# samkoesnadi/fpn-MT-image-captioning

Hardware: AMD Instinct MI355X
Metric: training images/sec (FPN+transformer step) at 1/2/4/8 MI355X; CPU-ref logit Δ (higher is better)
Workload: dtype bf16; 1 GPU; C2: ResNet-50 FPN + 6-layer transformer, 224x224, per-GPU batch 32, T=31, V=10000, full training step (fwd+bwd+clip+AMSGrad), dropout 0.1, hipGraph replay; per_gpu_batch=32, global_batch=32, seq_len=31, parallelism=dp1

## Files before the change

### fpn-mt-image-captioning_amd/csrc/elementwise.hip

```cpp
#include "common.h"
#include <initializer_list>

namespace fpnmt {

template <typename T> struct V16;
template <> struct V16<bf16> { typedef bf16x8 type; static constexpr int n = 8; };
template <> struct V16<float> { typedef f32x4 type; static constexpr int n = 4; };

static inline int grid_for(long long work, int block, int cap = 4096) {
  long long g = (work + block - 1) / block;
  if (g > cap) g = cap;
  if (g < 1) g = 1;
  return (int)g;
}

static inline __host__ __device__ int pow2_floor(int v) {
  int r = 1;
  while (r * 2 <= v) r *= 2;
  return r;
}
template <typename T, bool VEC>
__device__ __forceinline__ void act_bwd_block(int bx, int by, long long rows, int c, int act, float a,
                                              const T* __restrict__ dy, const T* __restrict__ y, T* dz, float* db,
                                              float* __restrict__ ws, int rows_per_chunk, bool write, float dp,
// ... 422 lines not shown
    Ld8<T, VN>::store(dx + (((long long)nn * h + ih) * w + iw) * c + ch, g);
  }
}

template <typename T>
__global__ __launch_bounds__(256) void maxpool3s2_bwd_kernel(int n, int h, int w, int c, int pt, int pl, int ho,
                                                             int wo, const uint8_t* __restrict__ argmax,
                                                             const T* __restrict__ dy, T* __restrict__ dx,
                                                             const T* __restrict__ xact, int act, float alpha) {
  const int cg = c / 8;
  const long long total = (long long)n * ho * wo * cg;
  for (long long i = blockIdx.x * (long long)blockDim.x + threadIdx.x; i < total;
       i += (long long)gridDim.x * blockDim.x) {
    const int ch = (int)(i % cg) * 8;
    long long t = i / cg;
    const int ow = (int)(t % wo);
    t /= wo;
    const int oh = (int)(t % ho);
    const int nn = (int)(t / ho);
    float g[4][8];
#pragma unroll
    for (int q = 0; q < 4; ++q)
#pragma unroll
      for (int j = 0; j < 8; ++j) g[q][j] = 0.f;
#pragma unroll
    for (int dy_ = -1; dy_ <= 0; ++dy_) {
#pragma unroll
      for (int dx_ = -1; dx_ <= 0; ++dx_) {
        const int wy = oh + dy_, wx = ow + dx_;
        if (wy < 0 || wx < 0) continue;
        const long long o = (((long long)nn * ho + wy) * wo + wx) * c + ch;
        const uint2 a = *(const uint2*)(argmax + o);
        int slot[8];
        bool any = false;
#pragma unroll
        for (int j = 0; j < 8; ++j) {
          const int am = (int)(((j < 4 ? a.x : a.y) >> (8 * (j & 3))) & 255);
          const int r = am / 3, q = am - 3 * r;
          const int dr = 2 * dy_ + r, dc = 2 * dx_ + q;
          slot[j] = ((unsigned)dr < 2u && (unsigned)dc < 2u) ? dr * 2 + dc : -1;
          any |= slot[j] >= 0;
        }
        if (!any) continue;
        float d[8];
        Ld8<T, 8>::load(dy + o, d);
#pragma unroll
        for (int j = 0; j < 8; ++j)
#pragma unroll
          for (int q = 0; q < 4; ++q)
            if (slot[j] == q) g[q][j] += d[j];
      }
    }
#pragma unroll
    for (int q = 0; q < 4; ++q) {
      const int ih = 2 * oh - pt + (q >> 1), iw = 2 * ow - pl + (q & 1);
      if (ih < 0 || ih >= h || iw < 0 || iw >= w) continue;
      T* dst = dx + (((long long)nn * h + ih) * w + iw) * c + ch;
      if (xact) {
        float v[8];
        Ld8<T, 8>::load(xact + (dst - dx), v);
#pragma unroll
        for (int j = 0; j < 8; ++j) g[q][j] *= act_mask_from_y(v[j], act, alpha);
      }
      Ld8<T, 8>::store(dst, g[q]);
    }
  }
}

template <typename T>
static void maxpool_launch(bool fwd, int n, int h, int w, int c, int kh, int kw, int sh, int sw, int pt, int pl,
                           int ho, int wo, const void* x, void* y, uint8_t* am, const void* dy, void* dx,
                           hipStream_t s, const void* xact = nullptr, int act = 0, float alpha = 0.f) {
  const bool vec = c % 8 == 0 && (uintptr_t)x % 16 == 0 && (uintptr_t)(fwd ? y : dy) % 16 == 0 &&
                   (uintptr_t)(fwd ? y : dx) % 16 == 0 && (uintptr_t)am % 8 == 0 && (uintptr_t)xact % 16 == 0;
  const long long total = (long long)n * (fwd ? (long long)ho * wo : (long long)h * w) * (vec ? c / 8 : c);
  const int g = grid_for(total, 256, 8192);
  if (fwd) {
    if (vec)
      hipLaunchKernelGGL((maxpool_fwd_kernel<T, 8>), dim3(g), dim3(256), 0, s, n, h, w, c, kh, kw, sh, sw, pt, pl,
                         ho, wo, (const T*)x, (T*)y, am);
    else
      hipLaunchKernelGGL((maxpool_fwd_kernel<T, 1>), dim3(g), dim3(256), 0, s, n, h, w, c, kh, kw, sh, sw, pt, pl,
                         ho, wo, (const T*)x, (T*)y, am);
  } else if (vec && am && kh == 3 && kw == 3 && sh == 2 && sw == 2 && (unsigned)pt < 2u && (unsigned)pl < 2u &&
             2 * ho - pt >= h && 2 * wo - pl >= w) {
    const int g2 = grid_for((long long)n * ho * wo * (c / 8), 256, 8192);
    hipLaunchKernelGGL((maxpool3s2_bwd_kernel<T>), dim3(g2), dim3(256), 0, s, n, h, w, c, pt, pl, ho, wo,
                       (const uint8_t*)am, (const T*)dy, (T*)dx, (const T*)xact, act, alpha);
  } else {
    if (vec)
      hipLaunchKernelGGL((maxpool_bwd_kernel<T, 8>), dim3(g), dim3(256), 0, s, n, h, w, c, kh, kw, sh, sw, pt, pl,
                         ho, wo, (const T*)x, (const uint8_t*)am, (const T*)dy, (T*)dx, (const T*)xact, act, alpha);
    else
      hipLaunchKernelGGL((maxpool_bwd_kernel<T, 1>), dim3(g), dim3(256), 0, s, n, h, w, c, kh, kw, sh, sw, pt, pl,
                         ho, wo, (const T*)x, (const uint8_t*)am, (const T*)dy, (T*)dx, (const T*)xact, act, alpha);
  }
}

__device__ __forceinline__ int nn_src(int d, int in, int out) {
  int s = (int)floorf(((float)d + 0.5f) * ((float)in / (float)out));
  return s < in - 1 ? s : in - 1;
}

template <typename T>
__global__ void fpn_fwd_kernel(int n, int cg, int h5, int w5, int h4, int w4, int h3, int w3,
                               const T* __restrict__ l5, const T* __restrict__ l4,
                               const T* __restrict__ l3, T* __restrict__ p4m,
                               T* __restrict__ p3m) {
  typedef typename V16<T>::type VT;
  constexpr int VN = V16<T>::n;
  const int c = cg * VN;
  const long long tot3 = (long long)n * h3 * w3 * cg, tot4 = (long long)n * h4 * w4 * cg;
  for (long long i = blockIdx.x * (long long)blockDim.x + threadIdx.x; i < tot3 + tot4;
       i += (long long)gridDim.x * blockDim.x) {
    const bool is3 = i < tot3;
    long long j = is3 ? i : i - tot3;
    const int g = (int)(j % cg);
    long long t = j / cg;
    const int W = is3 ? w3 : w4, H = is3 ? h3 : h4;
    const int x = (int)(t % W);
    t /= W;
    const int y = (int)(t % H);
    const int b = (int)(t / H);
    const int y4 = is3 ? nn_src(y, h4, h3) : y, x4 = is3 ? nn_src(x, w4, w3) : x;
    const int y5 = nn_src(y4, h5, h4), x5 = nn_src(x4, w5, w4);
    VT a4 = *(const VT*)(l4 + (((long long)b * h4 + y4) * w4 + x4) * c + g * VN);
    VT a5 = *(const VT*)(l5 + (((long long)b * h5 + y5) * w5 + x5) * c + g * VN);
    VT o;
    if (is3) {
      VT a3 = *(const VT*)(l3 + (((long long)b * h3 + y) * w3 + x) * c + g * VN);
#pragma unroll
      for (int k = 0; k < VN; ++k) {
        const float p4 = to_f32(from_f32<T>(to_f32(a4[k]) + to_f32(a5[k])));
        o[k] = from_f32<T>(to_f32(a3[k]) + p4);
      }
      *(VT*)(p3m + (((long long)b * h3 + y) * w3 + x) * c + g * VN) = o;
    } else {
#pragma unroll
      for (int k = 0; k < VN; ++k) o[k] = from_f32<T>(to_f32(a4[k]) + to_f32(a5[k]));
      *(VT*)(p4m + (((long long)b * h4 + y) * w4 + x) * c + g * VN) = o;
    }
  }
}

__device__ __forceinline__ void nn_children(int s, int in, int out, int& lo, int& hi) {
  int d0 = (int)(((long long)s * out) / in) - 2;
  if (d0 < 0) d0 = 0;
  lo = -1;
  hi = -1;
  for (int d = d0; d < out; ++d) {
    const int src = nn_src(d, in, out);
    if (src == s && lo < 0) lo = d;
    if (src > s) { hi = d; break; }
  }
  if (lo < 0) { lo = 0; hi = 0; return; }
  if (hi < 0) hi = out;
}

template <typename T>
__global__ void fpn_bwd_kernel(int n, int cg, int h5, int w5, int h4, int w4, int h3, int w3,
                               const T* __restrict__ dp4, const T* __restrict__ dp3,
                               T* __restrict__ dl4, T* __restrict__ dl5, int acc5) {
  typedef typename V16<T>::type VT;
  constexpr int VN = V16<T>::n;
  const int c = cg * VN;
  const long long tot4 = (long long)n * h4 * w4 * cg, tot5 = (long long)n * h5 * w5 * cg;
  for (long long i = blockIdx.x * (long long)blockDim.x + threadIdx.x; i < tot4 + tot5;
       i += (long long)gridDim.x * blockDim.x) {
    const bool is4 = i < tot4;
    long long j = is4 ? i : i - tot4;
    const int g = (int)(j % cg);
    long long t = j / cg;
    const int W = is4 ? w4 : w5, H = is4 ? h4 : h5;
    const int x = (int)(t % W);
    t /= W;
    const int y = (int)(t % H);
    const int b = (int)(t / H);
    float acc[VN];
#pragma unroll
    for (int k = 0; k < VN; ++k) acc[k] = 0.f;
    int y4lo, y4hi, x4lo, x4hi;
    if (is4) { y4lo = y; y4hi = y + 1; x4lo = x; x4hi = x + 1; }
    else { nn_children(y, h5, h4, y4lo, y4hi); nn_children(x, w5, w4, x4lo, x4hi); }
    for (int yy = y4lo; yy < y4hi; ++yy)
      for (int xx = x4lo; xx < x4hi; ++xx) {
        VT d4 = *(const VT*)(dp4 + (((long long)b * h4 + yy) * w4 + xx) * c + g * VN);
        float s4[VN];
#pragma unroll
        for (int k = 0; k < VN; ++k) s4[k] = to_f32(d4[k]);
        int y3lo, y3hi, x3lo, x3hi;
        nn_children(yy, h4, h3, y3lo, y3hi);
        nn_children(xx, w4, w3, x3lo, x3hi);
        for (int y3 = y3lo; y3 < y3hi; ++y3)
          for (int x3 = x3lo; x3 < x3hi; ++x3) {
            VT d3 = *(const VT*)(dp3 + (((long long)b * h3 + y3) * w3 + x3) * c + g * VN);
#pragma unroll
            for (int k = 0; k < VN; ++k) s4[k] += to_f32(d3[k]);
          }
        if (is4) {
#pragma unroll
          for (int k = 0; k < VN; ++k) acc[k] = s4[k];
        } else {
#pragma unroll
          for (int k = 0; k < VN; ++k) acc[k] += to_f32(from_f32<T>(s4[k]));
        }
      }
    VT o;
    if (is4) {
#pragma unroll
      for (int k = 0; k < VN; ++k) o[k] = from_f32<T>(acc[k]);
      *(VT*)(dl4 + (((long long)b * h4 + y) * w4 + x) * c + g * VN) = o;
    } else {
      T* dst = dl5 + (((long long)b * h5 + y) * w5 + x) * c + g * VN;
      if (acc5) {
        VT old = *(const VT*)dst;
#pragma unroll
        for (int k = 0; k < VN; ++k) o[k] = from_f32<T>(acc[k] + to_f32(old[k]));
      } else {
#pragma unroll
        for (int k = 0; k < VN; ++k) o[k] = from_f32<T>(acc[k]);
      }
      *(VT*)dst = o;
    }
  }
}

template <typename T>
__global__ __launch_bounds__(256) void ssm_fwd_kernel(int hw, int c, int chunk,
                                                      const T* __restrict__ score,
                                                      const T* __restrict__ hs,
                                                      T* __restrict__ ctx, float* __restrict__ a_out) {
  __shared__ float red[8];
  const int b = blockIdx.x;
  const T* sc = score + (long long)b * hw;
  float m = -INFINITY;
  for (int p = threadIdx.x; p < hw; p += 256) m = fmaxf(m, to_f32(sc[p]));
  m = wave_max(m);
  if ((threadIdx.x & 63) == 0) red[threadIdx.x >> 6] = m;
  __syncthreads();
  m = fmaxf(fmaxf(red[0], red[1]), fmaxf(red[2], red[3]));
  __syncthreads();
  float s = 0.f;
  for (int p = threadIdx.x; p < hw; p += 256) s += expf(to_f32(sc[p]) - m);
  s = wave_sum(s);
  if ((threadIdx.x & 63) == 0) red[threadIdx.x >> 6] = s;
  __syncthreads();
  s = red[0] + red[1] + red[2] + red[3];
  const int p0 = blockIdx.y * chunk, p1 = min(hw, p0 + chunk);
  for (int p = p0 + threadIdx.x; p < p1; p += 256)
    a_out[(long long)b * hw + p] = expf(to_f32(sc[p]) - m) / s;
  const long long e0 = (long long)p0 * c, e1 = (long long)p1 * c;
  const T* h = hs + (long long)b * hw * c;
  T* o = ctx + (long long)b * hw * c;
  for (long long e = e0 + threadIdx.x; e < e1; e += 256) {
    const int p = (int)(e / c);
    const float a = expf(to_f32(sc[p]) - m) / s;
    o[e] = from_f32<T>(a * to_f32(h[e]));
  }
}

template <typename T>
__global__ __launch_bounds__(256) void ssm_bwd1_kernel(long long npos, int c, const float* __restrict__ a,
                                                       const T* __restrict__ hs,
                                                       const T* __restrict__ dctx, T* __restrict__ dhs,
                                                       double* __restrict__ da) {
  const long long wid = (blockIdx.x * 256LL + threadIdx.x) >> 6;
  const int lane = threadIdx.x & 63;
  for (long long p = wid; p < npos; p += (long long)gridDim.x * 4) {
    const float ap = a[p];
    double dot = 0.0;
    for (int ch = lane; ch < c; ch += 64) {
      const long long e = p * c + ch;
      const float g = to_f32(dctx[e]);
      dot += (double)g * (double)to_f32(hs[e]);
      dhs[e] = from_f32<T>(ap * g);
    }
    dot = wave_sum(dot);
    if (lane == 0) da[p] = dot;
  }
}
template <typename T>
__global__ __launch_bounds__(256) void ssm_bwd2_kernel(int hw, const float* __restrict__ a,
                                                       const double* __restrict__ da,
                                                       T* __restrict__ dscore) {
  __shared__ double red[4];
  const long long base = (long long)blockIdx.x * hw;
  double s = 0.0;
  for (int p = threadIdx.x; p < hw; p += 256) s += (double)a[base + p] * da[base + p];
  s = wave_sum(s);
  if ((threadIdx.x & 63) == 0) red[threadIdx.x >> 6] = s;
  __syncthreads();
  s = red[0] + red[1] + red[2] + red[3];
  for (int p = threadIdx.x; p < hw; p += 256)
    dscore[base + p] = from_f32<T>((float)((double)a[base + p] * (da[base + p] - s)));
}

constexpr int LN_MAXE = 16;
template <bool VEC>
__device__ __forceinline__ int ln_col(int lane, int k) {
  if constexpr (VEC) return (lane + 64 * (k >> 3)) * 8 + (k & 7);
  else return lane + 64 * k;
}

template <typename T, bool VEC>
__device__ __forceinline__ void ln_fwd_rows(long long blk, long long nblk, long long rows, int d, float eps,
                                            const T* __restrict__ x, const T* __restrict__ res,
                                            const float* __restrict__ gamma, const float* __restrict__ beta,
                                            const float* __restrict__ pe, int pe_rows, T* __restrict__ y,
                                            float* __restrict__ mean_out, float* __restrict__ rstd_out, float op,
                                            unsigned long long okey) {
  const int lane = threadIdx.x & 63;
  const long long wid = (blk * 256LL + threadIdx.x) >> 6;
  const long long nw = nblk * 4;
  const float osc = op > 0.f ? 1.f / (1.f - op) : 1.f;
  float gm[LN_MAXE], bt[LN_MAXE];
#pragma unroll
  for (int i = 0; i < LN_MAXE; ++i) {
    const int col = ln_col<VEC>(lane, i);
    gm[i] = col < d ? gamma[col] : 0.f;
    bt[i] = col < d ? beta[col] : 0.f;
  }
  for (long long r = wid; r < rows; r += nw) {
    float v[LN_MAXE], pv[LN_MAXE];
    float s = 0.f;
    {
      const long long prow = pe ? (r % pe_rows) : 0;
#pragma unroll
      for (int i = 0; i < LN_MAXE; ++i) {
        const int col = ln_col<VEC>(lane, i);
        pv[i] = pe && col < d ? pe[prow * d + col] : 0.f;
      }
    }
    if constexpr (VEC) {
#pragma unroll
      for (int i = 0; i < LN_MAXE / 8; ++i) {
        const int c0 = (lane + 64 * i) * 8;
        bf16x8 xv = {}, rv = {};
        if (c0 < d) {
          xv = *(const bf16x8*)(x + r * d + c0);
          if (res) rv = *(const bf16x8*)(res + r * d + c0);
        }
#pragma unroll
        for (int e = 0; e < 8; ++e) {
          float t = 0.f;
          if (c0 < d) {
            t = to_f32(xv[e]);
            if (res) t = to_f32(from_f32<T>(t + to_f32(rv[e])));
          }
          v[i * 8 + e] = t;
          s += t;
        }
      }
    } else {
#pragma unroll
      for (int i = 0; i < LN_MAXE; ++i) {
        const int col = lane + 64 * i;
        v[i] = 0.f;
        if (col < d) {
          float t = to_f32(x[r * d + col]);
          if (res) t = to_f32(from_f32<T>(t + to_f32(res[r * d + col])));
          v[i] = t;
          s += t;
        }
      }
    }
    const float mu = wave_sum(s) / (float)d;
    float q = 0.f;
#pragma unroll
    for (int i = 0; i < LN_MAXE; ++i) {
      const int col = ln_col<VEC>(lane, i);
      if (col < d) { const float t = v[i] - mu; q += t * t; }
    }
    const float var = wave_sum(q) / (float)d;
    const float rs = rsqrtf(var + eps);
    if constexpr (VEC) {
#pragma unroll
      for (int i = 0; i < LN_MAXE / 8; ++i) {
        const int c0 = (lane + 64 * i) * 8;
        if (c0 < d) {
          bf16x8 ov;
#pragma unroll
          for (int e = 0; e < 8; ++e) {
            float o = (v[i * 8 + e] - mu) * rs * gm[i * 8 + e] + bt[i * 8 + e];
            if (pe) o += pv[i * 8 + e];
            ov[e] = from_f32<T>(o);
            if (op > 0.f)
              ov[e] = from_f32<T>(uniform01(okey, (uint64_t)r * (uint64_t)d + (uint64_t)(c0 + e)) >= op
                                      ? to_f32(ov[e]) * osc : 0.f);
          }
          *(bf16x8*)(y + r * d + c0) = ov;
        }
      }
    } else {
#pragma unroll
      for (int i = 0; i < LN_MAXE; ++i) {
        const int col = lane + 64 * i;
        if (col < d) {
          float o = (v[i] - mu) * rs * gm[i] + bt[i];
          if (pe) o += pv[i];
          T ot = from_f32<T>(o);
          if (op > 0.f)
            ot = from_f32<T>(uniform01(okey, (uint64_t)r * (uint64_t)d + (uint64_t)col) >= op ? to_f32(ot) * osc
                                                                                                 : 0.f);
          y[r * d + col] = ot;
        }
      }
    }
    if (lane == 0) { mean_out[r] = mu; rstd_out[r] = rs; }
  }
}

template <typename T, bool VEC = false>
__global__ __launch_bounds__(256) void ln_fwd_kernel(long long rows, int d, float eps,
                                                     const T* __restrict__ x, const T* __restrict__ res,
                                                     const float* __restrict__ gamma,
                                                     const float* __restrict__ beta,
                                                     const float* __restrict__ pe, int pe_rows,
                                                     T* __restrict__ y, float* __restrict__ mean_out,
                                                     float* __restrict__ rstd_out) {
  ln_fwd_rows<T, VEC>(blockIdx.x, gridDim.x, rows, d, eps, x, res, gamma, beta, pe, pe_rows, y, mean_out, rstd_out,
                      0.f, 0ull);
}

template <typename T, bool VEC>
__device__ __forceinline__ void ln_bwd_rows(long long blk, long long nblk, long long rows, int d,
                                            const T* __restrict__ x, const T* __restrict__ res,
                                            const float* __restrict__ gamma, const float* __restrict__ mean,
                                            const float* __restrict__ rstd, const T* __restrict__ dy,
                                            T* __restrict__ dx, float* __restrict__ part, float dp,
                                            unsigned long long dkey, T* __restrict__ dz, float ip,
                                            unsigned long long ikey) {
  const int lane = threadIdx.x & 63;
  const float dsc = dz ? 1.f / (1.f - dp) : 1.f;
  const float isc = ip > 0.f ? 1.f / (1.f - ip) : 1.f;
  const long long wid = (blk * 256LL + threadIdx.x) >> 6;
  const long long nw = nblk * 4;
  float pg[LN_MAXE], pb[LN_MAXE];
#pragma unroll
  for (int i = 0; i < LN_MAXE; ++i) pg[i] = pb[i] = 0.f;
  for (long long r = wid; r < rows; r += nw) {
    const float mu = mean[r], rs = rstd[r];
    float xh[LN_MAXE], g[LN_MAXE];
    float s1 = 0.f, s2 = 0.f;
    if constexpr (VEC) {
#pragma unroll
      for (int i = 0; i < LN_MAXE / 8; ++i) {
        const int c0 = (lane + 64 * i) * 8;
        bf16x8 xv = {}, rv = {}, dv = {};
        if (c0 < d) {
          xv = *(const bf16x8*)(x + r * d + c0);
          if (res) rv = *(const bf16x8*)(res + r * d + c0);
          dv = *(const bf16x8*)(dy + r * d + c0);
        }
#pragma unroll
        for (int e = 0; e < 8; ++e) {
          const int k = i * 8 + e;
          xh[k] = 0.f;
          g[k] = 0.f;
          if (c0 < d) {
            float t = to_f32(xv[e]);
            if (res) t = to_f32(from_f32<T>(t + to_f32(rv[e])));
            xh[k] = (t - mu) * rs;
            float dyf = to_f32(dv[e]);
            if (ip > 0.f)
              dyf = to_f32(from_f32<T>(uniform01(ikey, (uint64_t)r * (uint64_t)d + (uint64_t)(c0 + e)) >= ip
                                           ? dyf * isc : 0.f));
            g[k] = dyf * gamma[c0 + e];
            pg[k] += dyf * xh[k];
            pb[k] += dyf;
            s1 += g[k];
            s2 += g[k] * xh[k];
          }
        }
      }
    } else {
#pragma unroll
      for (int i = 0; i < LN_MAXE; ++i) {
        const int col = lane + 64 * i;
        xh[i] = 0.f;
        g[i] = 0.f;
        if (col < d) {
          float t = to_f32(x[r * d + col]);
          if (res) t = to_f32(from_f32<T>(t + to_f32(res[r * d + col])));
          xh[i] = (t - mu) * rs;
          float dyf = to_f32(dy[r * d + col]);
          if (ip > 0.f)
            dyf = to_f32(from_f32<T>(uniform01(ikey, (uint64_t)r * (uint64_t)d + (uint64_t)col) >= ip ? dyf * isc
                                                                                                       : 0.f));
          g[i] = dyf * gamma[col];
          pg[i] += dyf * xh[i];
          pb[i] += dyf;
          s1 += g[i];
          s2 += g[i] * xh[i];
        }
      }
    }
    s1 = wave_sum(s1) / (float)d;
    s2 = wave_sum(s2) / (float)d;
    if constexpr (VEC) {
#pragma unroll
      for (int i = 0; i < LN_MAXE / 8; ++i) {
        const int c0 = (lane + 64 * i) * 8;
        if (c0 < d) {
          bf16x8 ov;
#pragma unroll
          for (int e = 0; e < 8; ++e) ov[e] = from_f32<T>(rs * (g[i * 8 + e] - s1 - xh[i * 8 + e] * s2));
          *(bf16x8*)(dx + r * d + c0) = ov;
          if (dz) {
#pragma unroll
            for (int e = 0; e < 8; ++e) {
              const float t = to_f32(ov[e]);
              ov[e] = from_f32<T>(uniform01(dkey, (uint64_t)r * (uint64_t)d + (uint64_t)(c0 + e)) >= dp ? t * dsc
                                                                                                         : 0.f);
            }
            *(bf16x8*)(dz + r * d + c0) = ov;
          }
        }
      }
    } else {
#pragma unroll
      for (int i = 0; i < LN_MAXE; ++i) {
        const int col = lane + 64 * i;
        if (col < d) {
          const T v = from_f32<T>(rs * (g[i] - s1 - xh[i] * s2));
          dx[r * d + col] = v;
          if (dz) {
            const float t = to_f32(v);
            dz[r * d + col] =
                from_f32<T>(uniform01(dkey, (uint64_t)r * (uint64_t)d + (uint64_t)col) >= dp ? t * dsc : 0.f);
          }
        }
      }
    }
  }
  if (part) {
    __shared__ float red[4][2 * 64 * LN_MAXE];
    const int w = threadIdx.x >> 6;
#pragma unroll
    for (int i = 0; i < LN_MAXE; ++i) {
      const int col = ln_col<VEC>(lane, i);
      if (col < d) {
        red[w][col] = pg[i];
        red[w][d + col] = pb[i];
      }
    }
    __syncthreads();
    float* dst = part + blk * 2 * d;
    for (int e = threadIdx.x; e < 2 * d; e += 256) dst[e] = ((red[0][e] + red[1][e]) + red[2][e]) + red[3][e];
  }
}

__device__ __forceinline__ unsigned long long drop_key_of(unsigned long long seed, const long long* seed_dev) {
  return seed + (seed_dev ? (unsigned long long)(*seed_dev) * 0x9E3779B97F4A7C15ull : 0ull);
}

template <typename T, bool VEC = false>
__global__ __launch_bounds__(256) void ln_bwd_kernel(long long rows, int d, const T* __restrict__ x,
                                                     const T* __restrict__ res,
                                                     const float* __restrict__ gamma,
                                                     const float* __restrict__ mean,
                                                     const float* __restrict__ rstd,
                                                     const T* __restrict__ dy, T* __restrict__ dx,
                                                     float* __restrict__ part, float dp,
                                                     unsigned long long dseed,
                                                     const long long* __restrict__ dseed_dev,
                                                     T* __restrict__ dz) {
  ln_bwd_rows<T, VEC>(blockIdx.x, gridDim.x, rows, d, x, res, gamma, mean, rstd, dy, dx, part, dp,
                      dz ? drop_key_of(dseed, dseed_dev) : 0ull, dz, 0.f, 0ull);
}

struct LnView {
  const void* x;
  void* y;
  const void* dy;
  float* mean;
  float* rstd;
  float* part;
  long long rows;
  unsigned long long seed;
  int blk0, nblk, pe_rows;
};
struct LnViews {
  LnView v[FPNMT_MAX_LN_VIEWS];
  int n;
};

__device__ __forceinline__ int ln_view_of(const LnViews& A, int b) {
  int k = 0;
#pragma unroll
  for (int i = 1; i < FPNMT_MAX_LN_VIEWS; ++i)
    if (i < A.n && b >= A.v[i].blk0) k = i;
  return k;
}

template <typename T, bool VEC>
__global__ __launch_bounds__(256) void ln_views_fwd_kernel(const LnViews A, int d, float eps,
                                                           const float* __restrict__ gamma,
                                                           const float* __restrict__ beta,
                                                           const float* __restrict__ pe, float p,
                                                           const long long* __restrict__ seed_dev) {
  const LnView& a = A.v[ln_view_of(A, blockIdx.x)];
  ln_fwd_rows<T, VEC>(blockIdx.x - a.blk0, a.nblk, a.rows, d, eps, (const T*)a.x, nullptr, gamma, beta, pe, a.pe_rows,
                      (T*)a.y, a.mean, a.rstd, p, p > 0.f ? drop_key_of(a.seed, seed_dev) : 0ull);
}

template <typename T, bool VEC>
__global__ __launch_bounds__(256) void ln_views_bwd_kernel(const LnViews A, int d, const float* __restrict__ gamma,
                                                           float p, const long long* __restrict__ seed_dev) {
  const LnView& a = A.v[ln_view_of(A, blockIdx.x)];
  ln_bwd_rows<T, VEC>(blockIdx.x - a.blk0, a.nblk, a.rows, d, (const T*)a.x, nullptr, gamma, a.mean, a.rstd,
                      (const T*)a.dy, (T*)a.y, a.part, 0.f, 0ull, nullptr, p,
                      p > 0.f ? drop_key_of(a.seed, seed_dev) : 0ull);
}

template <typename T>
__global__ void embed_fwd_kernel(int b, int t, int d, const int32_t* __restrict__ tok,
                                 const float* __restrict__ emb, const float* __restrict__ pe,
                                 T* __restrict__ y, float p, unsigned long long seed,
                                 const long long* __restrict__ seed_dev) {
  const long long total = (long long)b * t * d;
  const float sc = p > 0.f ? 1.f / (1.f - p) : 1.f;
  const unsigned long long key = p > 0.f ? drop_key_of(seed, seed_dev) : 0ull;
  for (long long i = blockIdx.x * (long long)blockDim.x + threadIdx.x; i < total;
       i += (long long)gridDim.x * blockDim.x) {
    const int col = (int)(i % d);
    const long long row = i / d;
    const int pos = (int)(row % t);
    const int id = tok[row];
    T v = from_f32<T>(emb[(long long)id * d + col] + pe[(long long)pos * d + col]);
    if (p > 0.f) v = from_f32<T>(uniform01(key, (uint64_t)i) >= p ? to_f32(v) * sc : 0.f);
    y[i] = v;
  }
}

template <typename T>
__device__ __forceinline__ float drop_grad(T g, float p, float sc, unsigned long long key, long long i) {
  if (p <= 0.f) return to_f32(g);
  return to_f32(from_f32<T>(uniform01(key, (uint64_t)i) >= p ? to_f32(g) * sc : 0.f));
}
template <typename I>
__global__ void decoder_targets_kernel(int b, int t, const I* __restrict__ tok, long long ld,
                                       int32_t* __restrict__ tin, int32_t* __restrict__ tout,
                                       float* __restrict__ mask) {
  const long long total = (long long)b * t * t;
  for (long long e = blockIdx.x * (long long)blockDim.x + threadIdx.x; e < total;
       e += (long long)gridDim.x * blockDim.x) {
    const int j = (int)(e % t);
    const long long bi = e / t;
    const int i = (int)(bi % t);
    const int bb = (int)(bi / t);
    const long long tj = (long long)tok[(long long)bb * ld + j];
    mask[e] = (tj == 0 || j > i) ? 1.f : 0.f;
    if (i == 0) {
      tin[(long long)bb * t + j] = (int32_t)tj;
      tout[(long long)bb * t + j] = (int32_t)tok[(long long)bb * ld + j + 1];
    }
  }
}

constexpr int EMB_CHUNK = 64, EMB_COLS = 512;
template <typename T>
__global__ __launch_bounds__(256) void embed_chunk_kernel(long long rows, int d, const int32_t* __restrict__ tok,
                                                          const T* __restrict__ dy, float* __restrict__ part,
                                                          float p, unsigned long long seed,
                                                          const long long* __restrict__ seed_dev) {
  const float sc = p > 0.f ? 1.f / (1.f - p) : 1.f;
  const unsigned long long key = p > 0.f ? drop_key_of(seed, seed_dev) : 0ull;
  __shared__ int s_tok[EMB_CHUNK], s_lead[EMB_CHUNK];
  __shared__ float acc[EMB_CHUNK][EMB_COLS];
  const int tid = threadIdx.x;
  const long long p0 = (long long)blockIdx.x * EMB_CHUNK;
  const int n = (int)min((long long)EMB_CHUNK, rows - p0);
  if (tid < EMB_CHUNK) s_tok[tid] = tid < n ? tok[p0 + tid] : -1;
  __syncthreads();
  if (tid < n) {
    int l = tid;
    for (int j = 0; j < tid; ++j)
      if (s_tok[j] == s_tok[tid]) { l = j; break; }
    s_lead[tid] = l;
  }
  __syncthreads();
  for (int c0 = 0; c0 < d; c0 += EMB_COLS) {
    const int w = min(EMB_COLS, d - c0);
    for (int e = tid; e < EMB_CHUNK * EMB_COLS; e += 256) (&acc[0][0])[e] = 0.f;
    __syncthreads();
    for (int col = tid; col < w; col += 256) {
#pragma unroll 8
      for (int i = 0; i < n; ++i)
        acc[s_lead[i]][col] += drop_grad(dy[(p0 + i) * d + c0 + col], p, sc, key, (p0 + i) * d + c0 + col);
    }
    __syncthreads();
    for (int i = 0; i < n; ++i) {
      if (s_lead[i] != i) continue;
      for (int col = tid; col < w; col += 256) part[(p0 + i) * d + c0 + col] = acc[i][col];
    }
    __syncthreads();
  }
}

template <typename T>
__global__ __launch_bounds__(64) void embed_leader_kernel(long long rows, int d, const int32_t* __restrict__ tok,
                                                          const T* __restrict__ dy, const float* __restrict__ part,
                                                          float* __restrict__ demb, float* __restrict__ rowsq,
                                                          int tok_in_lds, float dp, unsigned long long seed,
                                                          const long long* __restrict__ seed_dev) {
  const float dsc = dp > 0.f ? 1.f / (1.f - dp) : 1.f;
  const unsigned long long key = dp > 0.f ? drop_key_of(seed, seed_dev) : 0ull;
  extern __shared__ int s_tok[];
  __shared__ int s_lead[EMB_CHUNK];
  const int lane = threadIdx.x;
  const long long p = blockIdx.x;
  if (tok_in_lds) {
    for (long long q = lane; q < rows; q += 64) s_tok[q] = tok[q];
    __syncthreads();
  }
  const int32_t* tk = tok_in_lds ? (const int32_t*)s_tok : tok;
  const int id = tk[p];
  float sq = 0.f;
  for (int col = lane; col < d; col += 64) {
    const float g = drop_grad(dy[p * d + col], dp, dsc, key, p * d + col);
    sq += g * g;
  }
  sq = wave_sum(sq);
  if (lane == 0 && rowsq) rowsq[p] = sq;
  bool seen = false;
  for (long long q = lane; q < p; q += 64) seen |= tk[q] == id;
  if (__any(seen)) return;
  const long long nch = (rows + EMB_CHUNK - 1) / EMB_CHUNK;
  for (int c0 = 0; c0 < d; c0 += 64 * 8) {
    float a[8];
#pragma unroll
    for (int j = 0; j < 8; ++j) a[j] = 0.f;
    for (long long cb = p / EMB_CHUNK; cb < nch; cb += EMB_CHUNK) {
      int nl = 0;
      for (int l = 0; l < EMB_CHUNK && cb + l < nch; ++l) {
        const long long q = (cb + l) * EMB_CHUNK + lane;
        const unsigned long long m = __ballot(q < rows && tk[q] == id);
        if (m) {
          if (lane == 0) s_lead[nl] = (int)((cb + l) * EMB_CHUNK + __ffsll((long long)m) - 1);
          ++nl;
        }
      }
      __syncthreads();
      for (int i = 0; i < nl; i += 4) {
        float v[4][8];
#pragma unroll
        for (int u = 0; u < 4; ++u)
#pragma unroll
          for (int j = 0; j < 8; ++j) {
            const int col = c0 + lane + 64 * j;
            v[u][j] = (i + u < nl && col < d) ? part[(long long)s_lead[i + u] * d + col] : 0.f;
          }
#pragma unroll
        for (int u = 0; u < 4; ++u)
#pragma unroll
          for (int j = 0; j < 8; ++j) a[j] += v[u][j];
      }
      __syncthreads();
    }
#pragma unroll
    for (int j = 0; j < 8; ++j) {
      const int col = c0 + lane + 64 * j;
      if (col < d) demb[(long long)id * d + col] += a[j];
    }
  }
}

__global__ __launch_bounds__(256) void ordered_sum_kernel(long long n, const float* __restrict__ v, float scale,
                                                          float* __restrict__ out, int accumulate) {
  __shared__ float red[4];
  float s = 0.f;
  for (long long i = threadIdx.x; i < n; i += 256) s += v[i];
  s = wave_sum(s);
  if ((threadIdx.x & 63) == 0) red[threadIdx.x >> 6] = s;
  __syncthreads();
  if (threadIdx.x == 0) {
    const float t = ((red[0] + red[1]) + (red[2] + red[3])) * scale;
    out[0] = accumulate ? out[0] + t : t;
  }
}

template <typename T>
__global__ __launch_bounds__(256) void xent_kernel(long long rows, int v, const float* __restrict__ logits,
                                                   long long ld, const int32_t* __restrict__ labels,
                                                   float* __restrict__ loss, T* __restrict__ dlog,
                                                   long long ldd, float gscale) {
  __shared__ float red[4];
  const long long r = blockIdx.x;
  const float* x = logits + r * ld;
  float m = -INFINITY;
  for (int j = threadIdx.x; j < v; j += 256) m = fmaxf(m, x[j]);
  m = wave_max(m);
  if ((threadIdx.x & 63) == 0) red[threadIdx.x >> 6] = m;
  __syncthreads();
  m = fmaxf(fmaxf(red[0], red[1]), fmaxf(red[2], red[3]));
  __syncthreads();
  float s = 0.f;
  for (int j = threadIdx.x; j < v; j += 256) s += expf(x[j] - m);
  s = wave_sum(s);
  if ((threadIdx.x & 63) == 0) red[threadIdx.x >> 6] = s;
  __syncthreads();
  s = red[0] + red[1] + red[2] + red[3];
  const int lab = labels[r];
  const float mask = lab != 0 ? 1.f : 0.f;
  if (threadIdx.x == 0) loss[r] = mask != 0.f ? (m + logf(s)) - x[lab] : 0.f;
  if (dlog) {
    const float coef = mask * gscale / (float)rows;
    T* dr = dlog + r * ldd;
    for (int j = threadIdx.x; j < v; j += 256) {
      float p = expf(x[j] - m) / s;
      if (j == lab) p -= 1.f;
      dr[j] = from_f32<T>(p * coef);
    }
  }
}

}

using namespace fpnmt;

#define DT_DISPATCH(dtype, FN, ...)                                         \
  ((dtype) == FPNMT_BF16 ? FN<bf16>(__VA_ARGS__)                            \
   : (dtype) == FPNMT_F32 ? FN<float>(__VA_ARGS__)                          \
                          : fail(FPNMT_E_ARG, "unknown dtype"))

extern "C" {

long long fpnmt_act_bwd_ws_bytes(int dtype, long long rows, int c) {
  if (rows <= 0 || c <= 0) return 0;
  const ActBwdGrid a = dtype == FPNMT_BF16 ? act_bwd_grid<bf16>(rows, c, true, true)
                                           : act_bwd_grid<float>(rows, c, true, true);
  const ActBwdGrid b = dtype == FPNMT_BF16 ? act_bwd_grid<bf16>(rows, c, false, true)
                                           : act_bwd_grid<float>(rows, c, false, true);
  return (long long)std::max(a.gy, b.gy) * c * (long long)sizeof(float);
}

int fpnmt_act_bwd(int dtype, long long rows, int c, int act, float act_alpha, const void* dy,
                  const void* y, void* dz, float* db, float* ws, float drop_p, unsigned long long drop_seed,
                  const long long* drop_seed_dev, fpnmt_stream_t stream) {
  if (rows <= 0 || c <= 0) return 0;
  if (!dy || !dz || (act != FPNMT_ACT_NONE && !y)) return fail(FPNMT_E_ARG, "act_bwd: null pointer");
  if (drop_p >= 1.f) return fail(FPNMT_E_ARG, "act_bwd: drop_p must be < 1");
  return DT_DISPATCH(dtype, act_bwd_t, rows, c, act, act_alpha, dy, y, dz, db, ws, drop_p, drop_seed,
                     drop_seed_dev, S(stream));
}

int fpnmt_bias_grad(int dtype, long long rows, int c, const void* dy, float* db, fpnmt_stream_t stream) {
  if (rows <= 0 || c <= 0 || !db) return 0;
  if (!dy) return fail(FPNMT_E_ARG, "bias_grad: null pointer");
  if (dtype != FPNMT_BF16 && dtype != FPNMT_F32) return fail(FPNMT_E_ARG, "bias_grad: bad dtype");
  hipStream_t s = S(stream);
  if (!defer_active())
    return dtype == FPNMT_BF16
               ? act_bwd_t<bf16>(rows, c, FPNMT_ACT_NONE, 0.f, dy, nullptr, (void*)dy, db, nullptr, 0.f, 0ull, nullptr, s)
               : act_bwd_t<float>(rows, c, FPNMT_ACT_NONE, 0.f, dy, nullptr, (void*)dy, db, nullptr, 0.f, 0ull, nullptr, s);
  const bool aligned = ((uintptr_t)dy % 16) == 0;
  const ActBwdGrid G = dtype == FPNMT_BF16 ? act_bwd_grid<bf16>(rows, c, aligned, true)
                                           : act_bwd_grid<float>(rows, c, aligned, true);
  DefDirect J{};
  J.dy = dy;
  J.db = db;
  J.rows = rows;
  J.c = c;
  J.rpc = G.rpc;
  J.gt = G.gt;
  J.gx = G.gx;
  J.gy = G.gy;
  J.vec = G.vec ? 1 : 0;
  J.dtype = dtype;
  {
    J.ws = defer_alloc((long long)G.gy * c);
    if (!J.ws)
      return dtype == FPNMT_BF16 ? act_bwd_t<bf16>(rows, c, FPNMT_ACT_NONE, 0.f, dy, nullptr, (void*)dy, db, nullptr,
                                                   0.f, 0ull, nullptr, s)
                                 : act_bwd_t<float>(rows, c, FPNMT_ACT_NONE, 0.f, dy, nullptr, (void*)dy, db, nullptr,
                                                    0.f, 0ull, nullptr, s);
  }
  int st = defer_direct(J, s);
  if (!st) colsum_launch(G.gy, c, J.ws, db, s);
  return st;
}

int fpnmt_cast(int in_dtype, int out_dtype, long long n, const void* in, void* out,
               fpnmt_stream_t stream) {
  if (n <= 0) return 0;
  const int g = grid_for(n, 256);
  hipStream_t s = S(stream);
  if (in_dtype == FPNMT_F32 && out_dtype == FPNMT_BF16)
    hipLaunchKernelGGL((cast_kernel<float, bf16>), dim3(g), dim3(256), 0, s, n, (const float*)in, (bf16*)out);
  else if (in_dtype == FPNMT_BF16 && out_dtype == FPNMT_F32)
    hipLaunchKernelGGL((cast_kernel<bf16, float>), dim3(g), dim3(256), 0, s, n, (const bf16*)in, (float*)out);
  else if (in_dtype == FPNMT_F32 && out_dtype == FPNMT_F32)
    hipLaunchKernelGGL((cast_kernel<float, float>), dim3(g), dim3(256), 0, s, n, (const float*)in, (float*)out);
  else if (in_dtype == FPNMT_BF16 && out_dtype == FPNMT_BF16)
    hipLaunchKernelGGL((cast_kernel<bf16, bf16>), dim3(g), dim3(256), 0, s, n, (const bf16*)in, (bf16*)out);
  else
    return fail(FPNMT_E_ARG, "cast: bad dtype");
  return check_launch("cast");
}

int fpnmt_dropout(int dtype, long long n, float p, unsigned long long seed, const long long* seed_dev,
                  const void* x, void* y, fpnmt_stream_t stream) {
  if (n <= 0) return 0;
  if (!(p >= 0.f && p < 1.f)) return fail(FPNMT_E_ARG, "dropout: p must be in [0,1)");
  const int g = grid_for(n, 256);
  if (dtype == FPNMT_BF16)
    hipLaunchKernelGGL((dropout_kernel<bf16>), dim3(g), dim3(256), 0, S(stream), n, p, seed, seed_dev,
                       (const bf16*)x, (bf16*)y);
  else
    hipLaunchKernelGGL((dropout_kernel<float>), dim3(g), dim3(256), 0, S(stream), n, p, seed, seed_dev,
                       (const float*)x, (float*)y);
  return check_launch("dropout");
}

int fpnmt_add(int dtype, long long n, const void* a, const void* b, void* out, fpnmt_stream_t stream) {
  if (n <= 0) return 0;
  const int g = grid_for(n, 256);
  if (dtype == FPNMT_BF16)
    hipLaunchKernelGGL((add_kernel<bf16>), dim3(g), dim3(256), 0, S(stream), n, (const bf16*)a,
                       (const bf16*)b, (bf16*)out);
  else
    hipLaunchKernelGGL((add_kernel<float>), dim3(g), dim3(256), 0, S(stream), n, (const float*)a,
                       (const float*)b, (float*)out);
  return check_launch("add");
}

int fpnmt_maxpool2d_fwd(int dtype, int n, int h, int w, int c, int kh, int kw, int sh, int sw, int pt,
                        int pl, int ho, int wo, const void* x, void* y, uint8_t* argmax, fpnmt_stream_t stream) {
  const long long total = (long long)n * ho * wo * c;
  if (total <= 0) return 0;
  if (argmax && kh * kw > 255) return fail(FPNMT_E_UNSUPPORTED, "maxpool: argmax needs kh*kw <= 255");
  if (dtype == FPNMT_BF16)
    maxpool_launch<bf16>(true, n, h, w, c, kh, kw, sh, sw, pt, pl, ho, wo, x, y, argmax, nullptr, nullptr, S(stream));
  else
    maxpool_launch<float>(true, n, h, w, c, kh, kw, sh, sw, pt, pl, ho, wo, x, y, argmax, nullptr, nullptr, S(stream));
  return check_launch("maxpool_fwd");
}

int fpnmt_maxpool2d_bwd(int dtype, int n, int h, int w, int c, int kh, int kw, int sh, int sw, int pt,
                        int pl, int ho, int wo, const void* x, const uint8_t* argmax, const void* dy, void* dx,
                        fpnmt_stream_t stream) {
  const long long total = (long long)n * h * w * c;
  if (total <= 0) return 0;
  if (ho <= 0 || wo <= 0) return zero_fill(dx, total * (dtype == FPNMT_BF16 ? 2 : 4), S(stream));
  if (!argmax && !x) return fail(FPNMT_E_ARG, "maxpool_bwd: need x or argmax");
  if (dtype == FPNMT_BF16)
    maxpool_launch<bf16>(false, n, h, w, c, kh, kw, sh, sw, pt, pl, ho, wo, x, nullptr, (uint8_t*)argmax, dy, dx, S(stream));
  else
    maxpool_launch<float>(false, n, h, w, c, kh, kw, sh, sw, pt, pl, ho, wo, x, nullptr, (uint8_t*)argmax, dy, dx, S(stream));
  return check_launch("maxpool_bwd");
}

int fpnmt_maxpool2d_bwd_act(int dtype, int n, int h, int w, int c, int kh, int kw, int sh, int sw, int pt, int pl,
                            int ho, int wo, const uint8_t* argmax, const void* dy, const void* x, int act,
                            float alpha, void* dx, fpnmt_stream_t stream) {
  const long long total = (long long)n * h * w * c;
  if (total <= 0) return 0;
  if (ho <= 0 || wo <= 0) return zero_fill(dx, total * (dtype == FPNMT_BF16 ? 2 : 4), S(stream));
  if (!argmax || !x || !dy || !dx) return fail(FPNMT_E_ARG, "maxpool_bwd_act: null argmax / x / dy / dx");
  if (act != FPNMT_ACT_RELU && act != FPNMT_ACT_RELU6 && act != FPNMT_ACT_LEAKY)
    return fail(FPNMT_E_ARG, "maxpool_bwd_act: act must be relu / relu6 / leaky");
  if (act == FPNMT_ACT_LEAKY && (kh > sh || kw > sw))
    return fail(FPNMT_E_UNSUPPORTED, "maxpool_bwd_act: leaky needs non-overlapping windows");
  if (dtype == FPNMT_BF16)
    maxpool_launch<bf16>(false, n, h, w, c, kh, kw, sh, sw, pt, pl, ho, wo, nullptr, nullptr, (uint8_t*)argmax, dy,
                         dx, S(stream), x, act, alpha);
  else
    maxpool_launch<float>(false, n, h, w, c, kh, kw, sh, sw, pt, pl, ho, wo, nullptr, nullptr, (uint8_t*)argmax, dy,
                          dx, S(stream), x, act, alpha);
  return check_launch("maxpool_bwd_act");
}

int fpnmt_fpn_topdown_fwd(int dtype, int n, int c, int h5, int w5, int h4, int w4, int h3, int w3,
                          const void* lat5, const void* lat4, const void* lat3, void* p4m, void* p3m,
                          fpnmt_stream_t stream) {
  const int vn = dtype == FPNMT_BF16 ? 8 : 4;
  if (c % vn) return fail(FPNMT_E_UNSUPPORTED, "fpn_topdown: channels must be a multiple of 8 (bf16) / 4 (f32)");
  const long long total = (long long)n * (h3 * w3 + h4 * w4) * (c / vn);
  if (total <= 0) return 0;
  const int g = grid_for(total, 256);
  if (dtype == FPNMT_BF16)
    hipLaunchKernelGGL((fpn_fwd_kernel<bf16>), dim3(g), dim3(256), 0, S(stream), n, c / vn, h5, w5, h4, w4,
                       h3, w3, (const bf16*)lat5, (const bf16*)lat4, (const bf16*)lat3, (bf16*)p4m, (bf16*)p3m);
  else
    hipLaunchKernelGGL((fpn_fwd_kernel<float>), dim3(g), dim3(256), 0, S(stream), n, c / vn, h5, w5, h4, w4,
                       h3, w3, (const float*)lat5, (const float*)lat4, (const float*)lat3, (float*)p4m,
                       (float*)p3m);
  return check_launch("fpn_topdown_fwd");
}

int fpnmt_fpn_topdown_bwd(int dtype, int n, int c, int h5, int w5, int h4, int w4, int h3, int w3,
                          const void* d_p4m, const void* d_p3m, void* d_lat4, void* d_lat5,
                          int accumulate_lat5, fpnmt_stream_t stream) {
  const int vn = dtype == FPNMT_BF16 ? 8 : 4;
  if (c % vn) return fail(FPNMT_E_UNSUPPORTED, "fpn_topdown: channels must be a multiple of 8 (bf16) / 4 (f32)");
  const long long total = (long long)n * (h4 * w4 + h5 * w5) * (c / vn);
  if (total <= 0) return 0;
  const int g = grid_for(total, 256);
  if (dtype == FPNMT_BF16)
    hipLaunchKernelGGL((fpn_bwd_kernel<bf16>), dim3(g), dim3(256), 0, S(stream), n, c / vn, h5, w5, h4, w4,
                       h3, w3, (const bf16*)d_p4m, (const bf16*)d_p3m, (bf16*)d_lat4, (bf16*)d_lat5,
                       accumulate_lat5);
  else
    hipLaunchKernelGGL((fpn_bwd_kernel<float>), dim3(g), dim3(256), 0, S(stream), n, c / vn, h5, w5, h4, w4,
                       h3, w3, (const float*)d_p4m, (const float*)d_p3m, (float*)d_lat4, (float*)d_lat5,
                       accumulate_lat5);
  return check_launch("fpn_topdown_bwd");
}

int fpnmt_spatial_softmax_fwd(int dtype, int n, int hw, int c, const void* score, const void* hs,
                              void* ctx, float* a_out, fpnmt_stream_t stream) {
  if (n <= 0 || hw <= 0) return 0;
  int chunks = (int)((long long)hw * c / 8192);
  if (chunks < 1) chunks = 1;
  if (chunks > hw) chunks = hw;
  const int chunk = cdiv(hw, chunks);
  chunks = cdiv(hw, chunk);
  dim3 grid(n, chunks);
  if (dtype == FPNMT_BF16)
    hipLaunchKernelGGL((ssm_fwd_kernel<bf16>), grid, dim3(256), 0, S(stream), hw, c, chunk,
                       (const bf16*)score, (const bf16*)hs, (bf16*)ctx, a_out);
  else
    hipLaunchKernelGGL((ssm_fwd_kernel<float>), grid, dim3(256), 0, S(stream), hw, c, chunk,
                       (const float*)score, (const float*)hs, (float*)ctx, a_out);
  return check_launch("spatial_softmax_fwd");
}

int fpnmt_spatial_softmax_bwd(int dtype, int n, int hw, int c, const float* a, const void* hs,
                              const void* d_ctx, void* d_score, void* d_hs, double* ws,
                              fpnmt_stream_t stream) {
  if (n <= 0 || hw <= 0) return 0;
  const long long npos = (long long)n * hw;
  const int g = grid_for(npos, 4, 8192);
  if (dtype == FPNMT_BF16) {
    hipLaunchKernelGGL((ssm_bwd1_kernel<bf16>), dim3(g), dim3(256), 0, S(stream), npos, c, a,
                       (const bf16*)hs, (const bf16*)d_ctx, (bf16*)d_hs, ws);
    hipLaunchKernelGGL((ssm_bwd2_kernel<bf16>), dim3(n), dim3(256), 0, S(stream), hw, a, ws, (bf16*)d_score);
  } else {
    hipLaunchKernelGGL((ssm_bwd1_kernel<float>), dim3(g), dim3(256), 0, S(stream), npos, c, a,
                       (const float*)hs, (const float*)d_ctx, (float*)d_hs, ws);
    hipLaunchKernelGGL((ssm_bwd2_kernel<float>), dim3(n), dim3(256), 0, S(stream), hw, a, ws, (float*)d_score);
  }
  return check_launch("spatial_softmax_bwd");
}

static bool ln_vec(int d, std::initializer_list<const void*> ptrs) {
  if (d % 8) return false;
  for (const void* p : ptrs)
    if ((uintptr_t)p & 15) return false;
  return true;
}

int fpnmt_layernorm_fwd(int dtype, long long rows, int d, float eps, const void* x, const void* res,
                        const float* gamma, const float* beta, const float* pe, int pe_rows, void* y,
                        float* mean, float* rstd, fpnmt_stream_t stream) {
  if (rows <= 0) return 0;
  if (d > 64 * LN_MAXE) return fail(FPNMT_E_UNSUPPORTED, "layernorm: d > 1024");
  if (pe && pe_rows <= 0) return fail(FPNMT_E_ARG, "layernorm: pe_rows");
  const int g = grid_for(rows, 4, 8192);
  if (dtype == FPNMT_BF16) {
    if (ln_vec(d, {x, res, y}))
      hipLaunchKernelGGL((ln_fwd_kernel<bf16, true>), dim3(g), dim3(256), 0, S(stream), rows, d, eps, (const bf16*)x,
                       (const bf16*)res, gamma, beta, pe, pe_rows, (bf16*)y, mean, rstd);
    else
      hipLaunchKernelGGL((ln_fwd_kernel<bf16>), dim3(g), dim3(256), 0, S(stream), rows, d, eps, (const bf16*)x,
                       (const bf16*)res, gamma, beta, pe, pe_rows, (bf16*)y, mean, rstd);
  } else {
    hipLaunchKernelGGL((ln_fwd_kernel<float>), dim3(g), dim3(256), 0, S(stream), rows, d, eps, (const float*)x,
                       (const float*)res, gamma, beta, pe, pe_rows, (float*)y, mean, rstd);
  }
  return check_launch("layernorm_fwd");
}

static int layernorm_bwd_impl(int dtype, long long rows, int d, const void* x, const void* res, const float* gamma,
                              const float* mean, const float* rstd, const void* dy, void* dx, float* dgamma,
                              float* dbeta, float dp, unsigned long long dseed, const long long* dseed_dev, void* dz,
                              hipStream_t s) {
  if (rows <= 0) return 0;
  if (d > 64 * LN_MAXE) return fail(FPNMT_E_UNSUPPORTED, "layernorm: d > 1024");
  if (dz && !(dp > 0.f && dp < 1.f)) return fail(FPNMT_E_ARG, "layernorm_bwd_drop: drop_p outside (0, 1)");
  const int g = grid_for(rows, 4, 1024);
  float* part = nullptr;
  if (dgamma || dbeta) {
    part = partial_f32((long long)g * 2 * d);
    if (!part) return fail(FPNMT_E_ARG, "layernorm_bwd: dgamma / dbeta need the fpnmt workspace");
  }
  if (dtype == FPNMT_BF16) {
    if (ln_vec(d, {x, res, dy, dx, dz}))
      hipLaunchKernelGGL((ln_bwd_kernel<bf16, true>), dim3(g), dim3(256), 0, s, rows, d, (const bf16*)x,
                         (const bf16*)res, gamma, mean, rstd, (const bf16*)dy, (bf16*)dx, part, dp, dseed, dseed_dev,
                         (bf16*)dz);
    else
      hipLaunchKernelGGL((ln_bwd_kernel<bf16>), dim3(g), dim3(256), 0, s, rows, d, (const bf16*)x,
                         (const bf16*)res, gamma, mean, rstd, (const bf16*)dy, (bf16*)dx, part, dp, dseed, dseed_dev,
                         (bf16*)dz);
  } else {
    hipLaunchKernelGGL((ln_bwd_kernel<float>), dim3(g), dim3(256), 0, s, rows, d, (const float*)x,
                       (const float*)res, gamma, mean, rstd, (const float*)dy, (float*)dx, part, dp, dseed, dseed_dev,
                       (float*)dz);
  }
  if (part) colsum_launch(g, 2 * d, part, dgamma, s, d, dbeta);
  return check_launch("layernorm_bwd");
}

int fpnmt_layernorm_bwd(int dtype, long long rows, int d, const void* x, const void* res,
                        const float* gamma, const float* mean, const float* rstd, const void* dy, void* dx,
                        float* dgamma, float* dbeta, fpnmt_stream_t stream) {
  return layernorm_bwd_impl(dtype, rows, d, x, res, gamma, mean, rstd, dy, dx, dgamma, dbeta, 0.f, 0ull, nullptr,
                            nullptr, S(stream));
}

int fpnmt_layernorm_bwd_drop(int dtype, long long rows, int d, const void* x, const void* res, const float* gamma,
                             const float* mean, const float* rstd, const void* dy, void* dx, float* dgamma,
                             float* dbeta, float drop_p, unsigned long long drop_seed,
                             const long long* drop_seed_dev, void* dz, fpnmt_stream_t stream) {
  if (!dz) return fail(FPNMT_E_ARG, "layernorm_bwd_drop: null dz");
  return layernorm_bwd_impl(dtype, rows, d, x, res, gamma, mean, rstd, dy, dx, dgamma, dbeta, drop_p, drop_seed,
                            drop_seed_dev, dz, S(stream));
}

static bool ln_views_vec(int n, int d, const fpnmt_ln_view* v, bool bwd) {
  for (int i = 0; i < n; ++i)
    if (!(bwd ? ln_vec(d, {v[i].x, v[i].dy, v[i].y}) : ln_vec(d, {v[i].x, v[i].y}))) return false;
  return true;
}

int fpnmt_layernorm_views_fwd(int dtype, int n, int d, float eps, const fpnmt_ln_view* views, const float* gamma,
                              const float* beta, const float* pe, float drop_p, const long long* seed_dev,
                              fpnmt_stream_t stream) {
  if (n < 0 || n > FPNMT_MAX_LN_VIEWS) return fail(FPNMT_E_ARG, "layernorm_views_fwd: 0 <= n <= FPNMT_MAX_LN_VIEWS");
  if (d > 64 * LN_MAXE) return fail(FPNMT_E_UNSUPPORTED, "layernorm: d > 1024");
  if (!(drop_p >= 0.f && drop_p < 1.f)) return fail(FPNMT_E_ARG, "layernorm_views_fwd: drop_p outside [0, 1)");
  LnViews A{};
  int blocks = 0;
  for (int i = 0; i < n; ++i) {
    const fpnmt_ln_view& v = views[i];
    if (v.rows <= 0) continue;
    if (!v.x || !v.y || !v.mean || !v.rstd || (pe && v.pe_rows <= 0))
      return fail(FPNMT_E_ARG, "layernorm_views_fwd: null pointer / pe_rows");
    LnView& a = A.v[A.n++];
    a.x = v.x; a.y = v.y; a.mean = v.mean; a.rstd = v.rstd; a.rows = v.rows; a.seed = v.seed;
    a.pe_rows = pe ? v.pe_rows : 1;
    a.blk0 = blocks;
    a.nblk = grid_for(v.rows, 4, 8192);
    blocks += a.nblk;
  }
  if (!A.n) return 0;
  hipStream_t s = S(stream);
  if (dtype == FPNMT_BF16) {
    if (ln_views_vec(n, d, views, false))
      hipLaunchKernelGGL((ln_views_fwd_kernel<bf16, true>), dim3(blocks), dim3(256), 0, s, A, d, eps, gamma, beta, pe,
                         drop_p, seed_dev);
    else
      hipLaunchKernelGGL((ln_views_fwd_kernel<bf16, false>), dim3(blocks), dim3(256), 0, s, A, d, eps, gamma, beta,
                         pe, drop_p, seed_dev);
  } else {
    hipLaunchKernelGGL((ln_views_fwd_kernel<float, false>), dim3(blocks), dim3(256), 0, s, A, d, eps, gamma, beta, pe,
                       drop_p, seed_dev);
  }
  return check_launch("layernorm_views_fwd");
}

int fpnmt_layernorm_views_bwd(int dtype, int n, int d, const fpnmt_ln_view* views, const float* gamma, float drop_p,
                              const long long* seed_dev, float* dgamma, float* dbeta, fpnmt_stream_t stream) {
  if (n < 0 || n > FPNMT_MAX_LN_VIEWS) return fail(FPNMT_E_ARG, "layernorm_views_bwd: 0 <= n <= FPNMT_MAX_LN_VIEWS");
  if (d > 64 * LN_MAXE) return fail(FPNMT_E_UNSUPPORTED, "layernorm: d > 1024");
  if (!(drop_p >= 0.f && drop_p < 1.f)) return fail(FPNMT_E_ARG, "layernorm_views_bwd: drop_p outside [0, 1)");
  LnViews A{};
  int blocks = 0;
  for (int i = 0; i < n; ++i) {
    const fpnmt_ln_view& v = views[i];
    if (v.rows <= 0) continue;
    if (!v.x || !v.y || !v.dy || !v.mean || !v.rstd) return fail(FPNMT_E_ARG, "layernorm_views_bwd: null pointer");
    LnView& a = A.v[A.n++];
    a.x = v.x; a.y = v.y; a.dy = v.dy; a.mean = v.mean; a.rstd = v.rstd; a.rows = v.rows; a.seed = v.seed;
    a.blk0 = blocks;
    a.nblk = grid_for(v.rows, 4, 1024);
    blocks += a.nblk;
    a.part = nullptr;
  }
  if (!A.n) return 0;
  if (dgamma || dbeta) {
    float* part = partial_f32((long long)blocks * 2 * d);
    if (!part) return fail(FPNMT_E_ARG, "layernorm_views_bwd: dgamma / dbeta need the fpnmt workspace");
    for (int i = 0; i < A.n; ++i) A.v[i].part = part + (long long)A.v[i].blk0 * 2 * d;
  }
  hipStream_t s = S(stream);
  if (dtype == FPNMT_BF16) {
    if (ln_views_vec(n, d, views, true))
      hipLaunchKernelGGL((ln_views_bwd_kernel<bf16, true>), dim3(blocks), dim3(256), 0, s, A, d, gamma, drop_p,
                         seed_dev);
    else
      hipLaunchKernelGGL((ln_views_bwd_kernel<bf16, false>), dim3(blocks), dim3(256), 0, s, A, d, gamma, drop_p,
                         seed_dev);
  } else {
    hipLaunchKernelGGL((ln_views_bwd_kernel<float, false>), dim3(blocks), dim3(256), 0, s, A, d, gamma, drop_p,
                       seed_dev);
  }
  const int st = check_launch("layernorm_views_bwd");
  if (st) return st;
  for (int i = 0; i < A.n; ++i)
    if (A.v[i].part) colsum_launch(A.v[i].nblk, 2 * d, A.v[i].part, dgamma, s, d, dbeta);
  return check_launch("layernorm_views_bwd colsum");
}

static int embed_fwd_impl(int dtype, int b, int t, int d, const int32_t* tok, const float* emb, const float* pe,
                          void* y, float p, unsigned long long seed, const long long* seed_dev, hipStream_t s) {
  const long long total = (long long)b * t * d;
  if (total <= 0) return 0;
  const int g = grid_for(total, 256);
  if (dtype == FPNMT_BF16)
    hipLaunchKernelGGL((embed_fwd_kernel<bf16>), dim3(g), dim3(256), 0, s, b, t, d, tok, emb, pe, (bf16*)y, p, seed,
                       seed_dev);
  else
    hipLaunchKernelGGL((embed_fwd_kernel<float>), dim3(g), dim3(256), 0, s, b, t, d, tok, emb, pe, (float*)y, p,
                       seed, seed_dev);
  return check_launch("embed_fwd");
}

static int embed_bwd_impl(int dtype, int b, int t, int d, const int32_t* tok, const void* dy, float* d_emb,
                          float* sumsq, float p, unsigned long long seed, const long long* seed_dev,
                          hipStream_t s) {
  const long long rows = (long long)b * t;
  if (rows <= 0) return 0;
  if (rows >= (1LL << 31)) return fail(FPNMT_E_UNSUPPORTED, "embed_bwd: too many positions");
  float* part = scratch_f32(rows * d + rows);
  if (!part) return fail(FPNMT_E_ARG, "embed_bwd: needs the fpnmt workspace");
  float* rowsq = sumsq ? part + rows * d : nullptr;
  const unsigned nch = (unsigned)((rows + EMB_CHUNK - 1) / EMB_CHUNK);
  const unsigned lds = rows <= 8192 ? (unsigned)(rows * 4) : 0u;
  if (dtype == FPNMT_BF16) {
    hipLaunchKernelGGL((embed_chunk_kernel<bf16>), dim3(nch), dim3(256), 0, s, rows, d, tok, (const bf16*)dy, part,
                       p, seed, seed_dev);
    hipLaunchKernelGGL((embed_leader_kernel<bf16>), dim3((unsigned)rows), dim3(64), lds, s, rows, d, tok,
                       (const bf16*)dy, (const float*)part, d_emb, rowsq, lds > 0, p, seed, seed_dev);
  } else {
    hipLaunchKernelGGL((embed_chunk_kernel<float>), dim3(nch), dim3(256), 0, s, rows, d, tok, (const float*)dy, part,
                       p, seed, seed_dev);
    hipLaunchKernelGGL((embed_leader_kernel<float>), dim3((unsigned)rows), dim3(64), lds, s, rows, d, tok,
                       (const float*)dy, (const float*)part, d_emb, rowsq, lds > 0, p, seed, seed_dev);
  }
  if (sumsq) hipLaunchKernelGGL(ordered_sum_kernel, dim3(1), dim3(256), 0, s, rows, rowsq, 1.f, sumsq, 1);
  return check_launch("embed_bwd");
}

int fpnmt_embed_posenc_fwd(int dtype, int b, int t, int d, const int32_t* tok, const float* emb,
                           const float* pe, void* y, fpnmt_stream_t stream) {
  return embed_fwd_impl(dtype, b, t, d, tok, emb, pe, y, 0.f, 0ull, nullptr, S(stream));
}

int fpnmt_embed_posenc_bwd(int dtype, int b, int t, int d, const int32_t* tok, const void* dy, float* d_emb,
                           float* sumsq, fpnmt_stream_t stream) {
  return embed_bwd_impl(dtype, b, t, d, tok, dy, d_emb, sumsq, 0.f, 0ull, nullptr, S(stream));
}

int fpnmt_embed_posenc_fwd_drop(int dtype, int b, int t, int d, const int32_t* tok, const float* emb,
                                const float* pe, void* y, float drop_p, unsigned long long seed,
                                const long long* seed_dev, fpnmt_stream_t stream) {
  if (!(drop_p >= 0.f && drop_p < 1.f)) return fail(FPNMT_E_ARG, "embed_posenc_fwd_drop: drop_p outside [0, 1)");
  return embed_fwd_impl(dtype, b, t, d, tok, emb, pe, y, drop_p, seed, seed_dev, S(stream));
}

int fpnmt_embed_posenc_bwd_drop(int dtype, int b, int t, int d, const int32_t* tok, const void* dy, float* d_emb,
                                float* sumsq, float drop_p, unsigned long long seed, const long long* seed_dev,
                                fpnmt_stream_t stream) {
  if (!(drop_p >= 0.f && drop_p < 1.f)) return fail(FPNMT_E_ARG, "embed_posenc_bwd_drop: drop_p outside [0, 1)");
  return embed_bwd_impl(dtype, b, t, d, tok, dy, d_emb, sumsq, drop_p, seed, seed_dev, S(stream));
}
int fpnmt_decoder_targets(int b, int t_full, const void* tok, int tok_bytes, long long ld_tok, int32_t* tar_inp,
                          int32_t* tar_real, float* mask, fpnmt_stream_t stream) {
  const int t = t_full - 1;
  if (b <= 0 || t <= 0) return 0;
  if (!tok || !tar_inp || !tar_real || !mask || ld_tok < t_full || (tok_bytes != 4 && tok_bytes != 8))
    return fail(FPNMT_E_ARG, "decoder_targets: null pointer / ld_tok < t_full / tok_bytes not 4 or 8");
  const long long total = (long long)b * t * t;
  if (tok_bytes == 8)
    hipLaunchKernelGGL(decoder_targets_kernel<long long>, dim3(grid_for(total, 256)), dim3(256), 0, S(stream), b, t,
                       (const long long*)tok, ld_tok, tar_inp, tar_real, mask);
  else
    hipLaunchKernelGGL(decoder_targets_kernel<int32_t>, dim3(grid_for(total, 256)), dim3(256), 0, S(stream), b, t,
                       (const int32_t*)tok, ld_tok, tar_inp, tar_real, mask);
  return check_launch("decoder_targets");
}

int fpnmt_xent_fwd_bwd(int dtype, long long rows, int v, const float* logits, long long ld,
                       const int32_t* labels, float* loss, void* dlogits, long long ldd, float dloss_scale,
                       fpnmt_stream_t stream) {
  if (!loss || !logits || !labels) return fail(FPNMT_E_ARG, "xent: null pointer");
  if (rows <= 0) return zero_fill(loss, sizeof(float), S(stream));
  float* row_loss = scratch_f32(rows);
  if (!row_loss) return fail(FPNMT_E_ARG, "xent: needs the fpnmt workspace");
  if (dtype == FPNMT_BF16)
    hipLaunchKernelGGL((xent_kernel<bf16>), dim3((unsigned)rows), dim3(256), 0, S(stream), rows, v, logits, ld,
                       labels, row_loss, (bf16*)dlogits, ldd, dloss_scale);
  else
    hipLaunchKernelGGL((xent_kernel<float>), dim3((unsigned)rows), dim3(256), 0, S(stream), rows, v, logits, ld,
                       labels, row_loss, (float*)dlogits, ldd, dloss_scale);
  hipLaunchKernelGGL(ordered_sum_kernel, dim3(1), dim3(256), 0, S(stream), rows, (const float*)row_loss,
                     1.f / (float)rows, loss, 0);
  return check_launch("xent");
}

}
```

### fpn-mt-image-captioning_amd/fpnmt/__init__.py

```python
import torch

from . import _lib
from . import ops, layers

_DTYPES = {"bf16": torch.bfloat16, "fp32": torch.float32, "f32": torch.float32,
           torch.bfloat16: torch.bfloat16, torch.float32: torch.float32}


class _Config:
    dtype = torch.bfloat16
    fuse_projections = True
    fuse_conv_chains = True
    fuse_bottleneck = True
    side_wgrad = False
    defer_reductions = True
    defer_conv_wgrads = True
    early_update = False
    early_update_grid = 64
    fuse_residual_grads = True
    fuse_optimizer_prep = True
    fuse_identity_residual = True
    fuse_block_act = True
    fuse_bias_wgrad = True
    fuse_drop_ln = True
    fuse_grad_sums = True
    fuse_view_norms = True
    fuse_ffn_act = True
    fuse_input_act = True
    zero_grad_overlap_grid = 0


config = _Config()


def set_precision(p):
    config.dtype = _DTYPES[p]


def compute_dtype():
    return config.dtype
```

### fpn-mt-image-captioning_amd/fpnmt/_lib.py

```python
from __future__ import annotations

import ctypes as C
import os

import torch

_HERE = os.path.dirname(os.path.abspath(__file__))
IN_TREE_PATH = os.path.join(_HERE, "libfpnmt.so")
LIB_PATH = os.environ.get("FPNMT_LIBRARY") or IN_TREE_PATH


CSRC_DIR = os.path.join(os.path.dirname(_HERE), "csrc")
HEADER_PATH = os.path.join(os.path.dirname(os.path.dirname(_HERE)), "include", "fpnmt.h")


def tree_build_id(csrc_dir: str = CSRC_DIR, header: str = HEADER_PATH) -> str:
    import hashlib
    names = sorted(f for f in os.listdir(csrc_dir) if f.endswith((".hip", ".h")))
    h = hashlib.sha256()
    for p in [os.path.join(csrc_dir, f) for f in names] + [os.path.join(csrc_dir, "Makefile"), header]:
        with open(p, "rb") as fh:
            h.update(fh.read())
    return h.hexdigest()[:16]


def library_build_id() -> str:
    return lib.fpnmt_build_id().decode()


def assert_in_tree():
    if os.path.realpath(LIB_PATH) != os.path.realpath(IN_TREE_PATH):
        raise RuntimeError(f"fpnmt: FPNMT_LIBRARY={LIB_PATH} is not the in-tree build {IN_TREE_PATH}; "
                           "unset it for benchmarks, smoke and tests")
    built, tree = library_build_id(), tree_build_id()
    if built != tree:
        raise RuntimeError(f"fpnmt: {LIB_PATH} was built from other sources (build id {built}) than the "
                           f"tree's csrc/ ({tree}); rebuild it with `make -C fpn-mt-image-captioning_amd/csrc`")
    knobs = sorted(k for k in os.environ if k.startswith(("FPNMT_TUNE_", "FPNMT_DBG_")))
    if knobs:
        raise RuntimeError(f"fpnmt: tuning / debug variables set ({', '.join(knobs)}); "
                           "unset them for benchmarks, smoke and tests")

F32, BF16 = 0, 1
ACT_NONE, ACT_RELU, ACT_LEAKY, ACT_RELU6 = 0, 1, 2, 3


class GemmDesc(C.Structure):
    _fields_ = [
        ("m", C.c_int), ("n", C.c_int), ("k", C.c_int),
        ("batch", C.c_int), ("batch_inner", C.c_int),
        ("dtype", C.c_int), ("a_trans", C.c_int), ("b_trans", C.c_int),
        ("lda", C.c_longlong), ("ldb", C.c_longlong), ("ldc", C.c_longlong), ("ldr", C.c_longlong),
        ("a_so", C.c_longlong), ("a_si", C.c_longlong), ("b_so", C.c_longlong), ("b_si", C.c_longlong),
        ("c_so", C.c_longlong), ("c_si", C.c_longlong), ("r_so", C.c_longlong), ("r_si", C.c_longlong),
        ("alpha", C.c_float), ("act", C.c_int), ("act_alpha", C.c_float),
        ("accumulate", C.c_int), ("c_f32", C.c_int), ("split_k", C.c_int),
        ("drop_p", C.c_float), ("drop_seed", C.c_ulonglong), ("drop_seed_dev", C.c_void_p),
    ]


class ConvDesc(C.Structure):
    _fields_ = [
        ("n", C.c_int), ("h", C.c_int), ("w", C.c_int), ("c", C.c_int),
        ("k", C.c_int), ("r", C.c_int), ("s", C.c_int),
        ("stride_h", C.c_int), ("stride_w", C.c_int),
        ("pad_t", C.c_int), ("pad_b", C.c_int), ("pad_l", C.c_int), ("pad_r", C.c_int),
        ("dtype", C.c_int), ("act", C.c_int), ("act_alpha", C.c_float),
    ]


class ConvLevel(C.Structure):
    _fields_ = [
        ("n", C.c_int), ("h", C.c_int), ("w", C.c_int),
        ("x", C.c_void_p), ("dz", C.c_void_p), ("residual", C.c_void_p), ("y", C.c_void_p),
    ]


class LnView(C.Structure):
    _fields_ = [
        ("x", C.c_void_p), ("y", C.c_void_p), ("dy", C.c_void_p), ("mean", C.c_void_p), ("rstd", C.c_void_p),
        ("rows", C.c_longlong), ("pe_rows", C.c_int), ("seed", C.c_ulonglong),
    ]


class AttnDesc(C.Structure):
    _fields_ = [
        ("b", C.c_int), ("h", C.c_int), ("lq", C.c_int), ("lk", C.c_int), ("d", C.c_int),
        ("dtype", C.c_int),
        ("ldq", C.c_longlong), ("ldk", C.c_longlong), ("ldv", C.c_longlong),
        ("ldo", C.c_longlong), ("ldw", C.c_longlong),
        ("scale", C.c_float),
        ("m_sb", C.c_longlong), ("m_sh", C.c_longlong), ("m_si", C.c_longlong), ("m_sj", C.c_longlong),
    ]


class AdamDesc(C.Structure):
    _fields_ = [
        ("beta1", C.c_float), ("beta2", C.c_float), ("eps", C.c_float), ("clipnorm", C.c_float),
        ("sched_d_model", C.c_float), ("sched_warmup", C.c_float), ("sched_mult", C.c_float),
        ("sched_warm_pow", C.c_float), ("const_lr", C.c_float), ("grad_scale", C.c_float),
    ]


class WPrepItem(C.Structure):
    _fields_ = [
        ("w_hwio", C.c_void_p), ("scale", C.c_void_p), ("w_ohwi", C.c_void_p), ("w_flip", C.c_void_p),
        ("r", C.c_int), ("s", C.c_int), ("c", C.c_int), ("k", C.c_int),
        ("tile_start", C.c_longlong), ("ld_flip", C.c_longlong),
    ]


class SegPrep(C.Structure):
    _fields_ = [
        ("ohwi", C.c_void_p), ("flip", C.c_void_p), ("scale", C.c_void_p),
        ("r", C.c_int), ("s", C.c_int), ("c", C.c_int), ("k", C.c_int),
        ("ld_flip", C.c_longlong), ("c_magic", C.c_uint32), ("c_shift", C.c_uint32),
    ]


P = C.c_void_p
I = C.c_int
LL = C.c_longlong
F = C.c_float
ULL = C.c_ulonglong
PP = C.POINTER(C.c_void_p)

SIGNATURES = {
    "fpnmt_version": [],
    "fpnmt_set_workspace": [P, LL],
    "fpnmt_fill_zero": [P, LL, P],
    "fpnmt_fill_zero_grid": [P, LL, I, P],
    "fpnmt_defer_begin": [P, LL],
    "fpnmt_defer_flush": [P],
    "fpnmt_gemm": [C.POINTER(GemmDesc), P, P, P, P, P, P, P],
    "fpnmt_gemm_act_in": [C.POINTER(GemmDesc), P, P, P, P, I, F, P],
    "fpnmt_gemm_wgrad": [C.POINTER(GemmDesc), P, P, P, P],
    "fpnmt_bottleneck_fwd": [I, I, I, I, I, P, P, P, P, P, P, P, P, P],
    "fpnmt_conv2d_fwd": [C.POINTER(ConvDesc), P, P, P, P, P, P, P],
    "fpnmt_conv2d_bwd_data": [C.POINTER(ConvDesc), P, P, P, I, P],
    "fpnmt_conv2d_bwd_data_act": [C.POINTER(ConvDesc), P, P, P, P, I, P],
    "fpnmt_conv2d_bwd_data_mask": [C.POINTER(ConvDesc), P, P, P, I, P, I, P],
    "fpnmt_conv2d_bwd_data_res": [C.POINTER(ConvDesc), P, P, P, P, P],
    "fpnmt_conv2d_bwd_data_res_act": [C.POINTER(ConvDesc), P, P, P, P, P, I, P],
    "fpnmt_set_defer_conv_wgrads": [I],
    "fpnmt_conv2d_bwd_filter": [C.POINTER(ConvDesc), P, P, P, P, P],
    "fpnmt_conv2d_bwd_filter_bias": [C.POINTER(ConvDesc), P, P, P, P, P, P],
    "fpnmt_conv2d_fwd_grouped": [C.POINTER(ConvDesc), I, C.POINTER(ConvLevel), P, P, P, P],
    "fpnmt_conv2d_bwd_data_grouped": [C.POINTER(ConvDesc), I, C.POINTER(ConvLevel), P, I, P],
    "fpnmt_conv2d_bwd_data_grouped_act": [C.POINTER(ConvDesc), I, C.POINTER(ConvLevel), P, I, P],
    "fpnmt_conv2d_bwd_data_grouped_mask": [C.POINTER(ConvDesc), I, C.POINTER(ConvLevel), P, I, I, P],
    "fpnmt_conv2d_bwd_filter_grouped": [C.POINTER(ConvDesc), I, C.POINTER(ConvLevel), P, P, P],
    "fpnmt_conv2d_bwd_filter_grouped_bias": [C.POINTER(ConvDesc), I, C.POINTER(ConvLevel), P, P, P, P],
    "fpnmt_weight_prep": [P, I, I, I, I, P, I, P, P, LL, P],
    "fpnmt_weight_prep_batched": [P, I, LL, I, P],
    "fpnmt_act_bwd": [I, LL, I, I, F, P, P, P, P, P, F, ULL, P, P],
    "fpnmt_bias_grad": [I, LL, I, P, P, P],
    "fpnmt_cast": [I, I, LL, P, P, P],
    "fpnmt_dropout": [I, LL, F, ULL, P, P, P, P],
    "fpnmt_add": [I, LL, P, P, P, P],
    "fpnmt_maxpool2d_fwd": [I, I, I, I, I, I, I, I, I, I, I, I, I, P, P, P, P],
    "fpnmt_maxpool2d_bwd": [I, I, I, I, I, I, I, I, I, I, I, I, I, P, P, P, P, P],
    "fpnmt_maxpool2d_bwd_act": [I, I, I, I, I, I, I, I, I, I, I, I, I, P, P, P, I, F, P, P],
    "fpnmt_fpn_topdown_fwd": [I, I, I, I, I, I, I, I, I, P, P, P, P, P, P],
    "fpnmt_fpn_topdown_bwd": [I, I, I, I, I, I, I, I, I, P, P, P, P, I, P],
    "fpnmt_spatial_softmax_fwd": [I, I, I, I, P, P, P, P, P],
    "fpnmt_spatial_softmax_bwd": [I, I, I, I, P, P, P, P, P, P, P],
    "fpnmt_attention_fwd": [C.POINTER(AttnDesc), P, P, P, P, P, P, P, P],
    "fpnmt_attention_bwd": [C.POINTER(AttnDesc), P, P, P, P, P, P, P, P, P, P],
    "fpnmt_attention_fwd_views": [I, C.POINTER(AttnDesc), PP, PP, PP, PP, PP, PP, PP, P],
    "fpnmt_attention_bwd_views": [I, C.POINTER(AttnDesc), PP, PP, PP, PP, PP, PP, PP, PP, PP, P],
    "fpnmt_view_proj_fwd": [I, I, I, I, I, P, LL, P, P, P, LL, P, LL, F, ULL, P, P],
    "fpnmt_view_proj_bwd_dz": [I, I, I, I, P, LL, P, P, F, ULL, P, P],
    "fpnmt_layernorm_fwd": [I, LL, I, F, P, P, P, P, P, I, P, P, P, P],
    "fpnmt_layernorm_bwd": [I, LL, I, P, P, P, P, P, P, P, P, P, P],
    "fpnmt_layernorm_bwd_drop": [I, LL, I, P, P, P, P, P, P, P, P, P, F, ULL, P, P, P],
    "fpnmt_decoder_targets": [I, I, P, I, LL, P, P, P, P],
    "fpnmt_layernorm_views_fwd": [I, I, I, F, C.POINTER(LnView), P, P, P, F, P, P],
    "fpnmt_layernorm_views_bwd": [I, I, I, C.POINTER(LnView), P, F, P, P, P, P],
    "fpnmt_embed_posenc_fwd": [I, I, I, I, P, P, P, P, P],
    "fpnmt_embed_posenc_bwd": [I, I, I, I, P, P, P, P, P],
    "fpnmt_embed_posenc_fwd_drop": [I, I, I, I, P, P, P, P, F, ULL, P, P],
    "fpnmt_embed_posenc_bwd_drop": [I, I, I, I, P, P, P, P, F, ULL, P, P],
    "fpnmt_xent_fwd_bwd": [I, LL, I, P, LL, P, P, P, LL, F, P],
    "fpnmt_grad_sumsq": [I, P, P, I, P, P, P, F, P, P],
    "fpnmt_amsgrad_step": [C.POINTER(AdamDesc), I, P, P, I, P, P, P, P, P, P, P, P, P, P, P, P],
    "fpnmt_amsgrad_step_prep": [C.POINTER(AdamDesc), I, P, P, I, P, P, P, P, P, P, P, P, P, P, P, P, P],
    "fpnmt_grad_sumsq_part": [I, I, I, P, P, I, P, P, P, F, P, P],
    "fpnmt_amsgrad_step_part": [C.POINTER(AdamDesc), I, I, I, I, P, P, I, P, P, P, P, P, P, P, P, P, P, P, P, P],
    "fpnmt_decode_attention": [I, I, I, I, I, F, P, LL, P, LL, LL, LL, LL, P, I, I, P, LL, P],
    "fpnmt_beam_step": [I, I, I, P, LL, P, P, P, I, I, P, P, I, I, P, P, I, P, P, P],
    "fpnmt_beam_step_log": [I, I, I, P, LL, P, P, P, P, P, I, I, P, P, I, I, P, P, P],
    "fpnmt_beam_finalize": [I, I, P, I, P, P, P, F, P, I, P, P, P],
    "fpnmt_sample_step": [I, I, P, LL, F, I, F, ULL, P, P, P, P, P, I, I, I, P, P, P],
    "fpnmt_sample_uniform": [I, I, ULL, P, P, P],
    "fpnmt_bn_stats": [I, LL, I, P, P, P, P, P, F, P],
    "fpnmt_bn_apply": [I, LL, I, P, P, P, P, P, F, I, P, P, P],
    "fpnmt_bn_bwd": [I, LL, I, P, P, P, P, F, I, P, P, P, P, P, P],
    "fpnmt_bn_stats_sums": [I, LL, I, P, P, P],
    "fpnmt_bn_stats_finalize": [I, P, P, P, P, P, F, P],
    "fpnmt_bn_bwd_sums": [I, LL, I, P, P, P, F, I, P, P, P, P, P, P],
    "fpnmt_bn_bwd_dx": [I, LL, I, P, P, P, P, F, I, P, P, P, P, P],
    "fpnmt_depthwise_fwd": [I, I, I, I, I, I, I, I, I, I, I, I, P, P, P, P],
    "fpnmt_depthwise_bwd_data": [I, I, I, I, I, I, I, I, I, I, I, I, P, P, P, P],
    "fpnmt_depthwise_bwd_filter": [I, I, I, I, I, I, I, I, I, I, I, I, P, P, P, P],
    "fpnmt_image_resize_normalize": [P, I, P, LL, I, I, I, F, F, I, P, P],
}
SIZE_T_FUNCS = {"fpnmt_attention_ws_bytes": [C.POINTER(AttnDesc)]}
LL_FUNCS = {"fpnmt_act_bwd_ws_bytes": [I, LL, I], "fpnmt_defer_peak_bytes": []}
STR_FUNCS = {"fpnmt_last_error": [], "fpnmt_build_id": []}
ALL_SYMBOLS = sorted(list(SIGNATURES) + list(SIZE_T_FUNCS) + list(LL_FUNCS) + list(STR_FUNCS))


def _load():
    if not os.path.exists(LIB_PATH):
        raise ImportError(
            f"libfpnmt.so not found at {LIB_PATH}; build it with "
            "`make -C fpn-mt-image-captioning_amd/csrc` (or __graft_entry__.build()). "
            "There is no fallback path.")
    lib = C.CDLL(LIB_PATH)
    for name, args in SIGNATURES.items():
        fn = getattr(lib, name)
        fn.argtypes = args
        fn.restype = C.c_int
    for name, args in SIZE_T_FUNCS.items():
        fn = getattr(lib, name)
        fn.argtypes = args
        fn.restype = C.c_size_t
    for name, args in LL_FUNCS.items():
        fn = getattr(lib, name)
        fn.argtypes = args
        fn.restype = C.c_longlong
    for name, args in STR_FUNCS.items():
        fn = getattr(lib, name)
        fn.argtypes = args
        fn.restype = C.c_char_p
    return lib


lib = _load()


E_ARG, E_UNSUPPORTED, E_HIP = -1, -2, -3
SAMPLE_FILTER_MAX_VOCAB = 16384


def check(status: int, what: str = ""):
    if status != 0:
        msg = lib.fpnmt_last_error().decode(errors="replace")
        raise RuntimeError(f"fpnmt {what} failed ({status}): {msg}")


def call(name: str, *args):
    check(getattr(lib, name)(*args), name)


def ptr(t):
    if t is None:
        return None
    return t.data_ptr()


WORKSPACE_BYTES = 256 << 20
_ws = {}
_ws_dev = [None]


def _ensure_workspace():
    dev = torch.cuda.current_device()
    if _ws_dev[0] == dev:
        return
    buf = _ws.get(dev)
    if buf is None:
        buf = torch.zeros(WORKSPACE_BYTES, dtype=torch.uint8, device=f"cuda:{dev}")
        _ws[dev] = buf
    check(lib.fpnmt_set_workspace(buf.data_ptr(), buf.numel()), "fpnmt_set_workspace")
    _ws_dev[0] = dev


_ws_side = {}


class side_workspace:

    def __enter__(self):
        _ensure_workspace()
        dev = torch.cuda.current_device()
        buf = _ws_side.get(dev)
        if buf is None:
            buf = torch.zeros(WORKSPACE_BYTES, dtype=torch.uint8, device=f"cuda:{dev}")
            _ws_side[dev] = buf
        check(lib.fpnmt_set_workspace(buf.data_ptr(), buf.numel()), "fpnmt_set_workspace")
        return self

    def __exit__(self, *exc):
        dev = torch.cuda.current_device()
        buf = _ws[dev]
        check(lib.fpnmt_set_workspace(buf.data_ptr(), buf.numel()), "fpnmt_set_workspace")
        return False


DEFER_BYTES = 3 << 30
_defer = {}


class deferred_reductions:

    def __init__(self, enabled=True):
        self.enabled = enabled

    def __enter__(self):
        self.on = False
        if self.enabled and torch.cuda.is_available():
            dev = torch.cuda.current_device()
            buf = _defer.get(dev)
            if buf is None:
                buf = torch.empty(DEFER_BYTES, dtype=torch.uint8, device=f"cuda:{dev}")
                _defer[dev] = buf
            _ensure_workspace()
            from . import config
            classes = conv_wgrad_classes(config.defer_conv_wgrads)
            check(lib.fpnmt_set_defer_conv_wgrads(classes), "fpnmt_set_defer_conv_wgrads")
            check(lib.fpnmt_defer_begin(buf.data_ptr(), buf.numel()), "fpnmt_defer_begin")
            self.on = True
            _defer_active[0] = True
            _defer_conv[0] = classes != 0
        return self

    def __exit__(self, *exc):
        if self.on:
            _defer_active[0] = False
            check(lib.fpnmt_defer_flush(torch.cuda.current_stream().cuda_stream), "fpnmt_defer_flush")
            _defer_keep.clear()
        return False


_defer_active = [False]
_defer_conv = [False]

CONV_WGRAD_CLASSES_DEFAULT = 0b01111


def conv_wgrad_classes(setting):
    if setting is True:
        return CONV_WGRAD_CLASSES_DEFAULT
    return int(setting or 0)


def defer_conv_wgrads():
    return _defer_active[0] and _defer_conv[0]
_defer_keep = []


def defer_checkpoint():
    if not _defer_active[0]:
        return
    dev = torch.cuda.current_device()
    buf = _defer[dev]
    check(lib.fpnmt_defer_flush(torch.cuda.current_stream().cuda_stream), "fpnmt_defer_flush")
    _defer_keep.clear()
    check(lib.fpnmt_defer_begin(buf.data_ptr(), buf.numel()), "fpnmt_defer_begin")


def defer_keep(t):
    if _defer_active[0]:
        _defer_keep.append(t)


def defer_active():
    return _defer_active[0]


def stream_ptr():
    _ensure_workspace()
    return torch.cuda.current_stream().cuda_stream


def dtype_code(dt: torch.dtype) -> int:
    if dt == torch.bfloat16:
        return BF16
    if dt == torch.float32:
        return F32
    raise TypeError(f"fpnmt kernels run in float32 or bfloat16, got {dt}")


ACT_CODES = {None: ACT_NONE, "linear": ACT_NONE, "relu": ACT_RELU, "leaky_relu": ACT_LEAKY, "relu6": ACT_RELU6}
```

### fpn-mt-image-captioning_amd/fpnmt/layers.py

```python
from __future__ import annotations

import math

import torch
from torch import nn

from . import _lib as L
from . import ops
from ._lib import call, ptr, stream_ptr, dtype_code

_GEN = [0]


def invalidate_weights():
    _GEN[0] += 1


class Init:

    def __init__(self, gen=None):
        self.gen = gen

    def _g(self):
        return self.gen

    def glorot_uniform(self, shape, fan_in, fan_out):
        lim = math.sqrt(6.0 / (fan_in + fan_out))
        return (torch.rand(shape, generator=self._g()) * 2 - 1) * lim

    def he_normal(self, shape, fan_in):
        std = math.sqrt(2.0 / fan_in) / 0.87962566103423978
        t = torch.randn(shape, generator=self._g())
        bad = t.abs() > 2
        while bad.any():
            t[bad] = torch.randn(int(bad.sum()), generator=self._g())
            bad = t.abs() > 2
        return t * std

    def normal(self, shape, std):
        return torch.randn(shape, generator=self._g()) * std

    def uniform(self, shape, lim):
        return (torch.rand(shape, generator=self._g()) * 2 - 1) * lim


DEFAULT_INIT = Init(None)


def _make_kernel(init, kind, shape, fan_in, fan_out, std=0.01):
    if kind == "he_normal":
        return init.he_normal(shape, fan_in)
    if kind == "normal":
        return init.normal(shape, std)
    return init.glorot_uniform(shape, fan_in, fan_out)


class _WeightLayer(nn.Module):

    def _init_copies(self):
        self._copies = {}
        self._gen = -1

    def _rsck(self):
        raise NotImplementedError

    def ensure_copies(self, dt):
        grp = self.__dict__.get("_group")
        if grp is not None and dt not in self._copies:
            grp[0].ensure(dt)
        if dt not in self._copies:
            r, s, c, k = self._rsck()
            dev = self.kernel.device
            self._copies[dt] = (torch.empty(r * s * c * k, dtype=dt, device=dev),
                                torch.empty(r * s * c * k, dtype=dt, device=dev))
        return self._copies[dt]

    def prepare(self, dtype=None):
        dts = [dtype] if dtype is not None else (list(self._copies) or [])
        r, s, c, k = self._rsck()
        for dt in dts:
            wf, wb = self.ensure_copies(dt)
            call("fpnmt_weight_prep", ptr(self.kernel), r, s, c, k, ptr(self.bn_scale), dtype_code(dt),
                 ptr(wf), ptr(wb), self.flip_ld(), stream_ptr())
        self._gen = _GEN[0]

    def flip_ld(self):
        grp = self.__dict__.get("_group")
        if grp is not None:
            return grp[0].n * grp[0].fout
        r, s, c, k = self._rsck()
        return r * s * k

    def compute_weights(self, dtype):
        if dtype not in self._copies or self._gen != _GEN[0]:
            self.prepare(dtype)
            if len(self._copies) > 1:
                self.prepare()
        return self._copies[dtype]


class Conv2D(_WeightLayer):

    def __init__(self, in_channels, filters, kernel_size, strides=1, padding="same", activation=None,
                 use_bias=True, kernel_initializer="glorot_uniform", std=0.01, frozen_bn=False,
                 bn_epsilon=1e-5, act_alpha=0.2, init=None, name=None):
        super().__init__()
        ks = kernel_size if isinstance(kernel_size, (tuple, list)) else (kernel_size, kernel_size)
        st = strides if isinstance(strides, (tuple, list)) else (strides, strides)
        self.kh, self.kw = ks
        self.sh, self.sw = st
        self.in_channels, self.filters = in_channels, filters
        self.padding = padding
        self.activation = activation
        self.act_alpha = act_alpha
        self.lname = name
        init = init or DEFAULT_INIT
        fan_in = self.kh * self.kw * in_channels
        fan_out = self.kh * self.kw * filters
        self.kernel = nn.Parameter(_make_kernel(init, kernel_initializer, (self.kh, self.kw, in_channels, filters),
                                                fan_in, fan_out, std))
        self.bias = nn.Parameter(torch.zeros(filters)) if use_bias else None
        if frozen_bn:
            self.register_buffer("bn_gamma", torch.ones(filters))
            self.register_buffer("bn_beta", torch.zeros(filters))
            self.register_buffer("bn_mean", torch.zeros(filters))
            self.register_buffer("bn_var", torch.ones(filters))
            self.bn_epsilon = bn_epsilon
            self.register_buffer("bn_scale", torch.empty(filters))
            self.register_buffer("bn_shift", torch.empty(filters))
            self.refresh_bn()
        else:
            self.bn_scale = None
            self.bn_shift = None
        self._init_copies()

    def refresh_bn(self):
        with torch.no_grad():
            sc = self.bn_gamma / torch.sqrt(self.bn_var + self.bn_epsilon)
            self.bn_scale.copy_(sc)
            self.bn_shift.copy_(self.bn_beta - self.bn_mean * sc)

    def _rsck(self):
        return self.kh, self.kw, self.in_channels, self.filters

    def pads_for(self, h, w):
        if isinstance(self.padding, (tuple, list)):
            return tuple(self.padding)
        if self.padding == "valid":
            return 0, 0, 0, 0
        ho, wo = -(-h // self.sh), -(-w // self.sw)
        th = max((ho - 1) * self.sh + self.kh - h, 0)
        tw = max((wo - 1) * self.sw + self.kw - w, 0)
        return th // 2, th - th // 2, tw // 2, tw - tw // 2

    def desc(self, n, h, w, c, dtype):
        key = (n, h, w, c, dtype)
        cache = self.__dict__.setdefault("_desc_cache", {})
        d = cache.get(key)
        if d is None:
            d = L.ConvDesc()
            d.n, d.h, d.w, d.c = n, h, w, c
            d.k, d.r, d.s = self.filters, self.kh, self.kw
            d.stride_h, d.stride_w = self.sh, self.sw
            d.pad_t, d.pad_b, d.pad_l, d.pad_r = self.pads_for(h, w)
            d.dtype = dtype_code(dtype)
            d.act = L.ACT_CODES[self.activation]
            d.act_alpha = self.act_alpha
            cache[key] = d
        return d

    def epilogue_bias(self):
        if self.bn_shift is not None:
            if self.bias is not None:
                raise NotImplementedError("conv bias + frozen BN")
            return self.bn_shift
        return self.bias

    def groupable(self, xs):
        return self.sh == 1 and self.sw == 1 and len({self.pads_for(*t.shape[1:3]) for t in xs}) == 1 and \
            len({t.dtype for t in xs}) == 1

    def check_input(self, x):
        if x is not None and x.shape[-1] != self.in_channels:
            raise ValueError(f"Conv2D {self.lname}: expected {self.in_channels} channels, got {x.shape[-1]}")

    def forward(self, x, residual=None):
        if isinstance(x, (list, tuple)):
            for t in x:
                self.check_input(t)
            if residual is None and len(x) > 1 and self.groupable(x):
                return list(ops.ConvGroupedFn.apply(self, *x))
            res = residual if residual is not None else [None] * len(x)
            return [self.forward(t, r) for t, r in zip(x, res)]
        self.check_input(x)
        return ops.Conv2dFn.apply(x, self.kernel, self.bias, residual, self)


class Dense(_WeightLayer):

    def __init__(self, in_features, units, activation=None, use_bias=True, kernel_initializer="glorot_uniform",
                 act_alpha=0.2, out_f32=False, init=None, name=None):
        super().__init__()
        init = init or DEFAULT_INIT
        self.kernel = nn.Parameter(_make_kernel(init, kernel_initializer, (in_features, units), in_features, units))
        self.bias = nn.Parameter(torch.zeros(units)) if use_bias else None
        self.activation = activation
        self.act_alpha = act_alpha
        self.out_f32 = out_f32
        self.bn_scale = None
        self.lname = name
        self._init_copies()

    def _rsck(self):
        fin, fout = self.kernel.shape
        return 1, 1, fin, fout

    def forward(self, x, dropout=0.0, residual=None):
        return ops.LinearFn.apply(x, self.kernel, self.bias, self, float(dropout), residual)


class BatchNormalization(nn.Module):

    def __init__(self, channels, epsilon=1e-3, momentum=0.999):
        super().__init__()
        self.gamma = nn.Parameter(torch.ones(channels))
        self.beta = nn.Parameter(torch.zeros(channels))
        self.register_buffer("moving_mean", torch.zeros(channels))
        self.register_buffer("moving_variance", torch.ones(channels))
        self.epsilon, self.momentum = epsilon, momentum
        self.sync_group = None

    def forward(self, x, training=True, activation=None, residual=None):
        act = L.ACT_CODES[activation]
        if training:
            return ops.BatchNormFn.apply(x, self.gamma, self.beta, self, act, residual)
        return ops.batch_norm_inference(x, self, act, residual)


class DepthwiseConv2D(nn.Module):

    def __init__(self, channels, kernel_size=3, strides=1, pads=(1, 1, 1, 1), init=None, name=None):
        super().__init__()
        init = init or DEFAULT_INIT
        self.kh = self.kw = kernel_size
        self.stride = strides
        self.pads = tuple(pads)
        self.lname = name
        k = kernel_size * kernel_size
        self.kernel = nn.Parameter(init.glorot_uniform((kernel_size, kernel_size, channels, 1), k * channels, k))

    def forward(self, x):
        return ops.DepthwiseConvFn.apply(x, self.kernel, self)


class LayerNormalization(nn.Module):
    def __init__(self, d, epsilon=1e-6):
        super().__init__()
        self.gamma = nn.Parameter(torch.ones(d))
        self.beta = nn.Parameter(torch.zeros(d))
        self.epsilon = epsilon

    def forward(self, x, residual=None, pe=None):
        return ops.LayerNormFn.apply(x, self.gamma, self.beta, residual, pe, self.epsilon, self)


class Embedding(nn.Module):

    def __init__(self, vocab, d, init=None):
        super().__init__()
        init = init or DEFAULT_INIT
        self.embeddings = nn.Parameter(init.uniform((vocab, d), 0.05))
        self.sumsq_slot = None

    def forward(self, tok, pe, dtype, dropout=0.0):
        slot = self.sumsq_slot
        if slot is None:
            slot = torch.zeros(1, dtype=torch.float32, device=self.embeddings.device)
        return ops.EmbedPosencFn.apply(tok, self.embeddings, pe, dtype, self, slot, dropout)


class DenseGroup:

    def __init__(self, layers):
        self.layers = list(layers)
        fin, fout = self.layers[0].kernel.shape
        for m in self.layers:
            if tuple(m.kernel.shape) != (fin, fout) or m.activation not in (None, "linear") or m.out_f32 \
                    or m.bias is None:
                raise ValueError("DenseGroup: members need equal shapes, linear activation, a bias")
        self.fin, self.fout, self.n = fin, fout, len(self.layers)
        for i, m in enumerate(self.layers):
            if m.__dict__.get("_group") is not None or m._copies:
                raise ValueError("DenseGroup: layer already grouped or already holds compute copies")
            m.__dict__["_group"] = (self, i)
        self._stack = {}

    def ensure(self, dt):
        if dt in self._stack:
            return
        n, fin, fout = self.n, self.fin, self.fout
        dev = self.layers[0].kernel.device
        stack = torch.empty(n * fout * fin, dtype=dt, device=dev)
        flip = torch.empty(fin, n * fout, dtype=dt, device=dev)
        self._stack[dt] = (stack, flip)
        for i, m in enumerate(self.layers):
            m._copies[dt] = (stack[i * fout * fin:(i + 1) * fout * fin], flip[:, i * fout:(i + 1) * fout])
            m._gen = -1

    def to_device_moved(self):
        self._stack = {}
        for m in self.layers:
            m._copies = {}

    def stacked(self, dt):
        for m in self.layers:
            m.compute_weights(dt)
        return self._stack[dt]

    def params(self):
        return [m.kernel for m in self.layers] + [m.bias for m in self.layers]

    @staticmethod
    def _contig(ts, per):
        base = ts[0]
        es = base.element_size()
        sp = base.untyped_storage().data_ptr()
        for i, t in enumerate(ts):
            if t is None or t.untyped_storage().data_ptr() != sp or t.data_ptr() != base.data_ptr() + i * per * es:
                return False
        return True

    def bias_cat(self):
        bs = [m.bias for m in self.layers]
        if self._contig(bs, self.fout):
            return bs[0].detach().view(-1).as_strided((self.n * self.fout,), (1,))
        return torch.cat([b.detach() for b in bs])

    def grad_views(self):
        from .ops import _grad_of
        kg = [_grad_of(m.kernel) for m in self.layers]
        bg = [_grad_of(m.bias) for m in self.layers]
        k = kg[0].as_strided((self.n, self.fin, self.fout), (self.fin * self.fout, self.fout, 1)) \
            if self._contig(kg, self.fin * self.fout) else None
        b = bg[0].as_strided((self.n * self.fout,), (1,)) if self._contig(bg, self.fout) else None
        return k, b

    def __call__(self, x):
        return ops.ProjectionGroupFn.apply(x, self, self.layers[0].kernel)


def group_param_order(model, named):
    groups = []
    seen = set()
    for m in model.modules():
        g = m.__dict__.get("_group")
        if g is not None and id(g[0]) not in seen:
            seen.add(id(g[0]))
            groups.append(g[0])
    name_of = {id(p): n for n, p in named}
    first = {}
    for g in groups:
        ps = [p for p in g.params() if id(p) in name_of]
        if len(ps) != len(g.params()):
            continue
        for p in ps:
            first[id(p)] = g
    out, done = [], set()
    for n, p in named:
        if id(p) in done:
            continue
        g = first.get(id(p))
        if g is None:
            out.append((n, p))
            done.add(id(p))
            continue
        for q in g.params():
            if id(q) not in done:
                out.append((name_of[id(q)], q))
                done.add(id(q))
    return out


def weight_layers(model):
    return [m for m in model.modules() if isinstance(m, _WeightLayer)]


class WeightPrepPlan:

    def __init__(self, model, dtypes, skip=()):
        self.layers = [m for m in weight_layers(model) if id(m) not in skip]
        self.tables = []
        for dt in dtypes:
            items = (L.WPrepItem * max(1, len(self.layers)))()
            tiles = 0
            for i, m in enumerate(self.layers):
                r, s, c, k = m._rsck()
                wf, wb = m.ensure_copies(dt)
                it = items[i]
                it.w_hwio = m.kernel.data_ptr()
                it.scale = m.bn_scale.data_ptr() if m.bn_scale is not None else None
                it.w_ohwi, it.w_flip = wf.data_ptr(), wb.data_ptr()
                it.r, it.s, it.c, it.k = r, s, c, k
                it.tile_start = tiles
                it.ld_flip = m.flip_ld()
                tiles += r * s * ((c + 31) // 32) * ((k + 31) // 32)
            raw = torch.frombuffer(bytearray(bytes(items)), dtype=torch.uint8)
            dev = self.layers[0].kernel.device if self.layers else torch.device("cpu")
            self.tables.append((dt, raw.to(dev), len(self.layers), tiles))

    def run(self):
        for dt, table, n, tiles in self.tables:
            call("fpnmt_weight_prep_batched", table.data_ptr(), n, tiles, dtype_code(dt), stream_ptr())
        for m in self.layers:
            m._gen = _GEN[0]


def _fastdiv(d):
    d = max(int(d), 1)
    sh = 0
    while (1 << sh) < d:
        sh += 1
    return (((1 << 32) * ((1 << sh) - d)) // d + 1) & 0xFFFFFFFF, sh


class FusedPrep:

    def __init__(self, model, arena):
        self.layers = set()
        self._mods = []
        n = len(arena.params)
        tab = (L.SegPrep * max(1, n))()
        for m in weight_layers(model):
            seg = arena.index.get(id(m.kernel))
            if seg is None or set(m._copies) != {torch.bfloat16}:
                continue
            r, s, c, k = m._rsck()
            wf, wb = m._copies[torch.bfloat16]
            scale_ok = m.bn_scale is None or m.bn_scale.data_ptr() % 16 == 0
            if (k & (k - 1)) or not 16 <= k <= 4096 or not scale_ok or m.flip_ld() % 4 \
                    or wf.data_ptr() % 8 or wb.data_ptr() % 8:
                continue
            e = tab[seg]
            e.ohwi, e.flip = wf.data_ptr(), wb.data_ptr()
            e.scale = m.bn_scale.data_ptr() if m.bn_scale is not None else None
            e.r, e.s, e.c, e.k = r, s, c, k
            e.ld_flip = m.flip_ld()
            e.c_magic, e.c_shift = _fastdiv(c)
            self.layers.add(id(m))
            self._mods.append(m)
        raw = torch.frombuffer(bytearray(bytes(tab)), dtype=torch.uint8)
        self.table = raw.to(arena.flat.device) if self.layers else None

    def mark_fresh(self):
        for m in self._mods:
            m._gen = _GEN[0]


def fused_prep(model, arena):
    import fpnmt
    if not fpnmt.config.fuse_optimizer_prep or not arena.flat.is_cuda:
        return None
    wl = weight_layers(model)
    key = (arena.flat.data_ptr(), tuple((tuple(sorted(str(d) for d in m._copies)),
                                         tuple(t.data_ptr() for c in m._copies.values() for t in c)) for m in wl))
    tabs = model.__dict__.setdefault("_fpnmt_fused_preps", {})
    if key not in tabs:
        tabs[key] = FusedPrep(model, arena)
    return tabs[key]


def prepare_all(model, dtype=None, skip=()):
    dts = set()
    wl = [m for m in weight_layers(model) if id(m) not in skip]
    for m in wl:
        dts.update(m._copies.keys())
    if dtype is not None:
        dts.add(dtype)
    ptrs = tuple((m.kernel.data_ptr(), m.bn_scale.data_ptr() if m.bn_scale is not None else 0) for m in wl)
    key = (tuple(sorted(str(d) for d in dts)), ptrs)
    plans = model.__dict__.setdefault("_fpnmt_wprep_plans", {})
    if key not in plans:
        plans[key] = WeightPrepPlan(model, sorted(dts, key=str), skip)
    plans[key].run()
```

### fpn-mt-image-captioning_amd/fpnmt/ops.py

```python
from __future__ import annotations

import math

import torch

from . import _lib as L
from ._lib import call, ptr, stream_ptr, dtype_code

class Runtime:
    seed_tensor = None
    base_seed = 0x5EED
    site = 0
    on_transformer_grads = None

    def reset_sites(self):
        self.site = 0

    def next_seed(self):
        self.site += 1
        return (self.base_seed * 1000003 + self.site) & 0xFFFFFFFFFFFF


runtime = Runtime()

# ... 1231 lines not shown


class MultiViewAttnProjFn(torch.autograd.Function):

    @staticmethod
    def forward(ctx, baseline, group, drop_p, num_heads, scale, mask, *qkv):
        nseg, fin, fout = group.n, group.fin, group.fout
        if len(qkv) != 3 * nseg:
            raise ValueError("MultiViewAttnProjFn: one (q, k, v) per view")
        B, Lq, HD = qkv[0].shape
        if HD != fin or baseline.shape[-1] != fout:
            raise ValueError("MultiViewAttnProjFn: view width / output width mismatch")
        rows = B * Lq
        cdt = baseline.dtype
        dt = dtype_code(cdt)
        dev = baseline.device
        O = _empty((rows, nseg * fin), cdt, dev)
        outs = [O[:, i * fin:(i + 1) * fin].view(B, Lq, fin) for i in range(nseg)]
        states = _attn_fwd_views([qkv[3 * i:3 * i + 3] for i in range(nseg)], mask, num_heads, scale, outs)
        stack, _ = group.stacked(cdt)
        bias = group.bias_cat()
        seed, st_dev = 0, None
        if drop_p > 0.0:
            seed = runtime.next_seed()
            st_dev = runtime.seed_tensor
        res = baseline.contiguous()
        ctx.rsink_res = _sink_for_res(baseline)
        y = _empty(tuple(baseline.shape), cdt, dev)
        call("fpnmt_view_proj_fwd", dt, rows, fout, fin, nseg, ptr(O), nseg * fin, ptr(stack), ptr(bias), ptr(res),
             fout, ptr(y), fout, float(drop_p), seed, ptr(st_dev), stream_ptr())
        ctx.group, ctx.drop = group, (float(drop_p), seed, st_dev)
        ctx.descs = [st[0] for st in states]
        ctx.slots = [st[6] for st in states]
        ctx.mask_keep = [st[5] for st in states]
        ctx.view_shape = (B, Lq, fin)
        ctx.set_materialize_grads(False)
        ctx.save_for_backward(O, *[t for st in states for t in (st[1], st[2], st[3], st[4])])
        return y

    @staticmethod
    def backward(ctx, dy):
        O, *saved = ctx.saved_tensors
        group = ctx.group
        nseg, fin, fout = group.n, group.fin, group.fout
        if dy is None:
            return (None,) * (6 + 3 * nseg)
        cdt = O.dtype
        dt = dtype_code(cdt)
        s = stream_ptr()
        rows = O.shape[0]
        dy = dy.contiguous()
        if dy.dtype != cdt:
            dyc = torch.empty(dy.shape, dtype=cdt, device=dy.device)
            call("fpnmt_cast", dtype_code(dy.dtype), dt, dy.numel(), ptr(dy), ptr(dyc), s)
            dy = dyc
        p, seed, st_dev = ctx.drop
        kg, bg = group.grad_views()
        dz = _empty((rows, nseg * fout), cdt, O.device)
        tmp = None
        if bg is None:
            tmp = torch.zeros(nseg * fout, dtype=torch.float32, device=O.device)
        call("fpnmt_view_proj_bwd_dz", dt, rows, fout, nseg, ptr(dy), fout, ptr(dz),
             (bg if bg is not None else tmp).data_ptr(), p, seed, ptr(st_dev), s)
        if tmp is not None:
            for i, m in enumerate(group.layers):
                _grad_of(m.bias).add_(tmp[i * fout:(i + 1) * fout])
        _, flip = group.stacked(cdt)
        dO = _empty((rows, nseg * fin), cdt, O.device)
        g = _gemm_desc(rows, fin, fout, dt, nseg * fout, nseg * fout, nseg * fin)
        g.batch = nseg
        g.a_so, g.b_so, g.c_so = fout, fout, fin
        call("fpnmt_gemm", g, ptr(dz), ptr(flip), ptr(dO), None, None, None, s)
        if kg is not None:
            g = _gemm_desc(fin, fout, rows, dt, nseg * fin, nseg * fout, fout, a_trans=1, b_trans=1,
                           accumulate=2, c_f32=1)
            g.batch = nseg
            g.a_so, g.b_so, g.c_so = fin, fout, fin * fout
            _wgrad(lambda: call("fpnmt_gemm_wgrad", g, ptr(O), ptr(dz), ptr(kg), stream_ptr()), O, dz)
        else:
            for i, m in enumerate(group.layers):
                g = _gemm_desc(fin, fout, rows, dt, nseg * fin, nseg * fout, fout, a_trans=1, b_trans=1,
                               accumulate=2, c_f32=1)
                gk = _grad_of(m.kernel)
                _wgrad(lambda g=g, i=i, gk=gk: call("fpnmt_gemm_wgrad", g, O[:, i * fin:].data_ptr(),
                                                    dz[:, i * fout:].data_ptr(), ptr(gk),
                                                    stream_ptr()), O, dz)
        B, Lq, _ = ctx.view_shape
        grads = _attn_bwd_views([(ctx.descs[i], *saved[4 * i:4 * i + 4], ctx.slots[i]) for i in range(nseg)],
                                [dO[:, i * fin:(i + 1) * fin].view(B, Lq, fin) for i in range(nseg)])
        dres = _sink_put(ctx.rsink_res, dy)
        return (dres, None, None, None, None, None, *grads)


class _GradSlot:

    def __init__(self, rows, cols, dtype, device):
        self.rows, self.cols, self.dtype, self.device = rows, cols, dtype, device
        self.buf = None
        self.claimed = set()

    def claim(self, off):
        if off in self.claimed:
            return False
        self.claimed.add(off)
        return True

    def get(self):
        if self.buf is None:
            self.buf = torch.empty((self.rows, self.cols), dtype=self.dtype, device=self.device)
        return self.buf

    def view(self, off, shape):
        w = shape[-1]
        return self.get()[:, off:off + w].view(shape)


def _slot_of(t):
    s = t.__dict__.get("_fpnmt_gslot") if hasattr(t, "__dict__") else None
    return s


class ProjectionGroupFn(torch.autograd.Function):

    @staticmethod
    def forward(ctx, x, group, _anchor):
        fin, fout, n = group.fin, group.fout, group.n
        ctx.rsink_gemm = _sink_for_gemm(x)
        if x.stride(-1) != 1 or not x.is_contiguous():
            x = x.contiguous()
        lead = x.shape[:-1]
        rows = x.numel() // fin if fin else 0
        x2 = x.view(rows, fin)
        cdt = x.dtype
        dt = dtype_code(cdt)
        y = _empty((rows, n * fout), cdt, x.device)
        stack, _ = group.stacked(cdt)
        bias = group.bias_cat()
        g = _gemm_desc(rows, n * fout, fin, dt, fin, fin, n * fout)
        call("fpnmt_gemm", g, ptr(x2), ptr(stack), ptr(y), None, ptr(bias), None, stream_ptr())
        slot = _GradSlot(rows, n * fout, cdt, x.device)
        outs = []
        for i in range(n):
            o = y[:, i * fout:(i + 1) * fout].view(*lead, fout)
            o.__dict__["_fpnmt_gslot"] = (slot, i * fout)
            outs.append(o)
        ctx.group, ctx.slot, ctx.rows = group, slot, rows
        ctx.in_shape = x.shape
        ctx.set_materialize_grads(False)
        ctx.save_for_backward(x2)
        return tuple(outs)

    @staticmethod
    def backward(ctx, *gs):
        (x2,) = ctx.saved_tensors
        group, slot, rows = ctx.group, ctx.slot, ctx.rows
        fin, fout, n = group.fin, group.fout, group.n
        cdt = x2.dtype
        dt = dtype_code(cdt)
        s = stream_ptr()
        buf = slot.get()
        for i, gi in enumerate(gs):
            dst = buf[:, i * fout:(i + 1) * fout]
            if gi is None:
                dst.zero_()
            elif not (gi.data_ptr() == dst.data_ptr() and gi.dim() >= 2 and gi.stride(-1) == 1 and
                      (rows <= 1 or gi.reshape(-1, fout).stride(0) == n * fout)):
                dst.copy_(gi.reshape(rows, fout))
        kg, bg = group.grad_views()
        if bg is not None:
            bias_grad(dt, rows, n * fout, buf, bg.data_ptr(), s)
        else:
            tmp = torch.zeros(n * fout, dtype=torch.float32, device=buf.device)
            act_bwd(dt, rows, n * fout, L.ACT_NONE, 0.0, buf, None, buf, tmp.data_ptr(), s)
            for i, m in enumerate(group.layers):
                _grad_of(m.bias).add_(tmp[i * fout:(i + 1) * fout])
        dx = None
        if ctx.needs_input_grad[0]:
            _, flip = group.stacked(cdt)
            dx = _empty((rows, fin), cdt, buf.device)
            g = _gemm_desc(rows, fin, n * fout, dt, n * fout, n * fout, fin)
            r = _sink_take(ctx.rsink_gemm)
            if r is not None and (r.dtype != cdt or r.numel() != dx.numel()):
                r = r.to(cdt).reshape(dx.shape).contiguous()
            call("fpnmt_gemm", g, ptr(buf), ptr(flip), ptr(dx), None, None, ptr(r), s)
            dx = dx.view(ctx.in_shape)
        if rows > 0:
            if kg is not None:
                g = _gemm_desc(fin, fout, rows, dt, fin, n * fout, fout, a_trans=1, b_trans=1,
                               accumulate=2, c_f32=1)
                g.batch = n
                g.a_so, g.b_so, g.c_so = 0, fout, fin * fout
                _wgrad(lambda: call("fpnmt_gemm_wgrad", g, ptr(x2), ptr(buf), ptr(kg), stream_ptr()),
                       x2, buf)
            else:
                for i, m in enumerate(group.layers):
                    g = _gemm_desc(fin, fout, rows, dt, fin, n * fout, fout, a_trans=1, b_trans=1,
                                   accumulate=2, c_f32=1)
                    gk = _grad_of(m.kernel)
                    _wgrad(lambda g=g, i=i, gk=gk: call("fpnmt_gemm_wgrad", g, ptr(x2), buf[:, i * fout:].data_ptr(),
                                                        ptr(gk), stream_ptr()), x2, buf)
        return dx, None, None


class LayerNormFn(torch.autograd.Function):

    @staticmethod
    def forward(ctx, x, gamma, beta, res, pe, eps, layer):
        ctx.rsink_res = _sink_for_res(res) if res is not x else None
        ctx.drop_tok = _drop_tok_claim(x)
        x = x.contiguous()
        d = x.shape[-1]
        rows = x.numel() // d if d else 0
        if res is not None:
            res = res.contiguous()
        y = torch.empty_like(x)
        mean = _empty((max(rows, 1),), torch.float32, x.device)
        rstd = _empty((max(rows, 1),), torch.float32, x.device)
        pe_rows = 0
        if pe is not None:
            pe_rows = x.shape[-2]
        call("fpnmt_layernorm_fwd", dtype_code(x.dtype), rows, d, eps, ptr(x), ptr(res), ptr(gamma),
             ptr(beta), ptr(pe), pe_rows, ptr(y), ptr(mean), ptr(rstd), stream_ptr())
        ctx.layer = layer
        ctx.has_res = res is not None
        ctx.save_for_backward(x, res if res is not None else x, mean, rstd)
        return y

    @staticmethod
    def backward(ctx, dy):
        x, res, mean, rstd = ctx.saved_tensors
        layer = ctx.layer
        d = x.shape[-1]
        rows = x.numel() // d if d else 0
        dx = torch.empty_like(x)
        tok = ctx.drop_tok
        if tok is None:
            call("fpnmt_layernorm_bwd", dtype_code(x.dtype), rows, d, ptr(x), ptr(res) if ctx.has_res else None,
                 ptr(layer.gamma), ptr(mean), ptr(rstd), ptr(dy.contiguous()), ptr(dx),
                 ptr(_grad_of(layer.gamma)), ptr(_grad_of(layer.beta)), stream_ptr())
        else:
            p, seed, st = tok.drop
            dz = torch.empty_like(x)
            call("fpnmt_layernorm_bwd_drop", dtype_code(x.dtype), rows, d, ptr(x),
                 ptr(res) if ctx.has_res else None, ptr(layer.gamma), ptr(mean), ptr(rstd), ptr(dy.contiguous()),
                 ptr(dx), ptr(_grad_of(layer.gamma)), ptr(_grad_of(layer.beta)), p, seed, ptr(st), ptr(dz),
                 stream_ptr())
            tok.dz = dz
            dx.__dict__["_fpnmt_dropdz"] = (tok, dx._version)
        return dx, None, None, (_sink_put(ctx.rsink_res, dx) if ctx.has_res else None), None, None, None


class LayerNormViewsFn(torch.autograd.Function):

    @staticmethod
    def forward(ctx, layer, pe, drop_p, *xs):
        xs = [x.contiguous() for x in xs]
        n, d = len(xs), xs[0].shape[-1]
        tab = (L.LnView * n)()
        ys, stats, seeds = [], [], []
        for i, x in enumerate(xs):
            rows = x.numel() // d if d else 0
            y = torch.empty_like(x)
            mean = _empty((max(rows, 1),), torch.float32, x.device)
            rstd = _empty((max(rows, 1),), torch.float32, x.device)
            seed = runtime.next_seed() if drop_p > 0.0 and rows > 0 else 0
            tab[i].x, tab[i].y, tab[i].mean, tab[i].rstd = ptr(x), ptr(y), ptr(mean), ptr(rstd)
            tab[i].rows, tab[i].pe_rows, tab[i].seed = rows, (x.shape[-2] if pe is not None else 0), seed
            ys.append(y)
            stats += [mean, rstd]
            seeds.append(seed)
        st = runtime.seed_tensor if drop_p > 0.0 else None
        call("fpnmt_layernorm_views_fwd", dtype_code(xs[0].dtype), n, d, float(layer.epsilon), tab, ptr(layer.gamma),
             ptr(layer.beta), ptr(pe), float(drop_p), ptr(st), stream_ptr())
        ctx.layer, ctx.p, ctx.st, ctx.seeds, ctx.n = layer, float(drop_p), st, seeds, n
        ctx.set_materialize_grads(False)
        ctx.save_for_backward(*xs, *stats)
        return tuple(ys)

    @staticmethod
    def backward(ctx, *dys):
        n = ctx.n
        saved = ctx.saved_tensors
        xs, stats = saved[:n], saved[n:]
        layer = ctx.layer
        d = xs[0].shape[-1]
        tab = (L.LnView * n)()
        dxs, keep = [], []
        for i, (x, dy) in enumerate(zip(xs, dys)):
            if dy is None or x.numel() == 0:
                dxs.append(None)
                continue
            dy = dy.contiguous()
            dx = torch.empty_like(x)
            tab[i].x, tab[i].y, tab[i].dy = ptr(x), ptr(dx), ptr(dy)
            tab[i].mean, tab[i].rstd = ptr(stats[2 * i]), ptr(stats[2 * i + 1])
            tab[i].rows, tab[i].seed = x.numel() // d, ctx.seeds[i]
            dxs.append(dx)
            keep.append(dy)
        call("fpnmt_layernorm_views_bwd", dtype_code(xs[0].dtype), n, d, tab, ptr(layer.gamma), ctx.p, ptr(ctx.st),
             ptr(_grad_of(layer.gamma)), ptr(_grad_of(layer.beta)), stream_ptr())
        return (None, None, None, *dxs)


class EmbedPosencFn(torch.autograd.Function):
    @staticmethod
    def forward(ctx, tok, emb, pe, dtype, layer, sumsq_slot, drop_p=0.0):
        tok = tok.to(torch.int32).contiguous()
        b, t = tok.shape
        d = emb.shape[1]
        y = _empty((b, t, d), dtype, emb.device)
        ctx.drop = None
        if drop_p > 0.0 and y.numel() > 0:
            ctx.drop = (float(drop_p), runtime.next_seed(), runtime.seed_tensor)
            p, seed, st = ctx.drop
            call("fpnmt_embed_posenc_fwd_drop", dtype_code(dtype), b, t, d, ptr(tok), ptr(emb), ptr(pe), ptr(y), p,
                 seed, ptr(st), stream_ptr())
        else:
            call("fpnmt_embed_posenc_fwd", dtype_code(dtype), b, t, d, ptr(tok), ptr(emb), ptr(pe), ptr(y),
                 stream_ptr())
        ctx.save_for_backward(tok)
        ctx.layer = layer
        ctx.sumsq = sumsq_slot
        ctx.dt = dtype
        return y

    @staticmethod
    def backward(ctx, dy):
        (tok,) = ctx.saved_tensors
        b, t = tok.shape
        emb = ctx.layer.embeddings
        if ctx.drop is not None:
            p, seed, st = ctx.drop
            call("fpnmt_embed_posenc_bwd_drop", dtype_code(ctx.dt), b, t, emb.shape[1], ptr(tok),
                 ptr(dy.contiguous()), ptr(_grad_of(emb)), ptr(ctx.sumsq), p, seed, ptr(st), stream_ptr())
        else:
            call("fpnmt_embed_posenc_bwd", dtype_code(ctx.dt), b, t, emb.shape[1], ptr(tok), ptr(dy.contiguous()),
                 ptr(_grad_of(emb)), ptr(ctx.sumsq), stream_ptr())
        return None, None, None, None, None, None, None


def decoder_targets(tok):
    if tok.dtype not in (torch.int64, torch.int32) or tok.dim() != 2 or tok.stride(1) != 1 or not tok.is_cuda:
        tin, tout = tok[:, :-1], tok[:, 1:]
        t = tin.shape[1]
        la = 1.0 - torch.tril(torch.ones((t, t), device=tok.device))
        return tin, tout, torch.maximum((tin == 0).to(torch.float32)[:, None, None, :], la)
    b, T = tok.shape
    t = T - 1
    tin = _empty((b, t), torch.int32, tok.device)
    tout = _empty((b, t), torch.int32, tok.device)
    mask = _empty((b, 1, t, t), torch.float32, tok.device)
    call("fpnmt_decoder_targets", b, T, ptr(tok), tok.element_size(), tok.stride(0), ptr(tin), ptr(tout), ptr(mask),
         stream_ptr())
    return tin, tout, mask


class MaskedXentFn(torch.autograd.Function):

    @staticmethod
    def forward(ctx, logits, labels):
        v = logits.shape[-1]
        lg = logits.reshape(-1, v)
        if lg.dtype != torch.float32:
            raise TypeError("MaskedXentFn expects fp32 logits")
        lg = lg.contiguous()
        lab = labels.reshape(-1).to(torch.int32).contiguous()
        rows = lg.shape[0]
        loss = torch.empty((1,), dtype=torch.float32, device=lg.device)
        dlog = torch.empty_like(lg)
        call("fpnmt_xent_fwd_bwd", L.F32, rows, v, ptr(lg), v, ptr(lab), ptr(loss), ptr(dlog), v, 1.0,
             stream_ptr())
        ctx.save_for_backward(dlog)
        ctx.shape = logits.shape
        return loss.reshape(())

    @staticmethod
    def backward(ctx, g):
        (dlog,) = ctx.saved_tensors
        return dlog.reshape(ctx.shape), None


class DropoutFn(torch.autograd.Function):
    @staticmethod
    def forward(ctx, x, p):
        x = x.contiguous()
        seed = runtime.next_seed()
        y = torch.empty_like(x)
        st = runtime.seed_tensor
        call("fpnmt_dropout", dtype_code(x.dtype), x.numel(), float(p), seed, ptr(st), ptr(x), ptr(y), stream_ptr())
        ctx.seed = seed
        ctx.p = p
        ctx.st = st
        return y

    @staticmethod
    def backward(ctx, dy):
        dy = dy.contiguous()
        dx = torch.empty_like(dy)
        call("fpnmt_dropout", dtype_code(dy.dtype), dy.numel(), float(ctx.p), ctx.seed, ptr(ctx.st), ptr(dy),
             ptr(dx), stream_ptr())
        return dx, None


def dropout(x, p, training):
    if not training or p <= 0.0 or x.numel() == 0:
        return x
    return DropoutFn.apply(x, p)


class AddFn(torch.autograd.Function):
    @staticmethod
    def forward(ctx, a, b):
        a, b = a.contiguous(), b.contiguous()
        out = torch.empty_like(a)
        call("fpnmt_add", dtype_code(a.dtype), a.numel(), ptr(a), ptr(b), ptr(out), stream_ptr())
        return out

    @staticmethod
    def backward(ctx, g):
        return g, g


def add(a, b):
    return AddFn.apply(a, b)


def cast(x, dtype):
    if x.dtype == dtype:
        return x
    x = x.contiguous()
    y = torch.empty(x.shape, dtype=dtype, device=x.device)
    call("fpnmt_cast", dtype_code(x.dtype), dtype_code(dtype), x.numel(), ptr(x), ptr(y), stream_ptr())
    return y
```

### fpn-mt-image-captioning_amd/models/transformer.py

```python
import math

import numpy as np
import torch
from torch import nn

from common.common_definitions import (ACTIVATION, BASELINE_INDEX, KERNEL_INITIALIZER, LEAKY_ALPHA, NUM_OF_PYRAMIDS,
                                       RETINANET_WEIGHT_PATH, BACKBONE, d_model as D_MODEL)
import fpnmt
from fpnmt import ops
from fpnmt.layers import Dense, DenseGroup, Embedding, LayerNormalization
from . import retinanet


def get_angles(pos, i, d_model):
    angle_rates = 1 / np.power(10000, (2 * (i // 2)) / np.float32(d_model))
    return pos * angle_rates


def raw_positional_encoding(position, d_model):
    angle_rads = get_angles(np.arange(position)[:, np.newaxis], np.arange(d_model)[np.newaxis, :], d_model)
    angle_rads[:, 0::2] = np.sin(angle_rads[:, 0::2])
    angle_rads[:, 1::2] = np.cos(angle_rads[:, 1::2])
    return torch.from_numpy(angle_rads.astype(np.float32))


def positional_encoding(position, d_model):
    return raw_positional_encoding(position, d_model)[None, ...]


def create_padding_mask(seq):
    return (seq == 0).to(torch.float32)[:, None, None, :]


def create_look_ahead_mask(size, device=None):
    return 1.0 - torch.tril(torch.ones((size, size), device=device))


def create_masks(tar):
    look_ahead_mask = create_look_ahead_mask(tar.shape[1], device=tar.device)
    dec_target_padding_mask = create_padding_mask(tar)
    return torch.maximum(dec_target_padding_mask, look_ahead_mask)


def scaled_dot_product_attention(q, k, v, mask):
    lead = q.shape[:-2]
    Lq, dk = q.shape[-2], q.shape[-1]
    Lk = k.shape[-2]
    bsz = int(np.prod(lead)) if len(lead) else 1
    q3 = q.reshape(bsz, Lq, dk)
    k3 = k.reshape(bsz, Lk, dk)
    v3 = v.reshape(bsz, Lk, v.shape[-1])
    m = None
    if mask is not None:
        m = torch.broadcast_to(mask.to(torch.float32), (*lead, Lq, Lk)).reshape(bsz, 1, Lq, Lk)
    out, w = ops.AttentionFn.apply(q3, k3, v3, m, 1, 1.0 / math.sqrt(dk))
    return out.reshape(*lead, Lq, v.shape[-1]), w.reshape(*lead, Lq, Lk)


class MultiHeadAttention(nn.Module):

    def __init__(self, d_model, num_heads, init=None):
        super().__init__()
        self.num_heads = num_heads
        self.d_model = d_model
        assert d_model % self.num_heads == 0
        self.depth = d_model // self.num_heads
        self.wq = Dense(d_model, d_model, kernel_initializer=KERNEL_INITIALIZER, init=init)
        self.wk = Dense(d_model, d_model, kernel_initializer=KERNEL_INITIALIZER, init=init)
        self.wv = Dense(d_model, d_model, kernel_initializer=KERNEL_INITIALIZER, init=init)
        self.dense = Dense(d_model, d_model, kernel_initializer=KERNEL_INITIALIZER, init=init)

    def split_heads(self, x, batch_size):
        return x.reshape(batch_size, -1, self.num_heads, self.depth).permute(0, 2, 1, 3)

    def forward(self, v, k, q, mask, dropout=0.0, residual=None):
        return self.attend(self.wq(q), self.wk(k), self.wv(v), mask, dropout, residual)

    def attend(self, q, k, v, mask, dropout=0.0, residual=None):
        scaled_attention, attention_weights = ops.AttentionFn.apply(
            q, k, v, mask, self.num_heads, 1.0 / math.sqrt(float(self.depth)))
        output = self.dense(scaled_attention, dropout=dropout, residual=residual)
        return output, attention_weights

    call = forward


class EncoderLayer(nn.Module):

    def __init__(self, d_model, num_heads, dff, rate=0.1, init=None):
        super().__init__()
        self.mhas = nn.ModuleList([MultiHeadAttention(d_model, num_heads, init=init)
                                   for _ in range(NUM_OF_PYRAMIDS - 1)])
        self.ffn1 = Dense(d_model, dff, activation=ACTIVATION, act_alpha=LEAKY_ALPHA,
                          kernel_initializer=KERNEL_INITIALIZER, init=init)
        self.ffn2 = Dense(dff, d_model, kernel_initializer=KERNEL_INITIALIZER, init=init)
        self.ffn1.act_into_next = True
        self.layernorm1 = LayerNormalization(d_model, epsilon=1e-6)
        self.layernorm2 = LayerNormalization(d_model, epsilon=1e-6)
        self.rate = rate
        self.q_group = DenseGroup([m.wq for m in self.mhas])
        self.o_group = DenseGroup([m.dense for m in self.mhas])

    def forward(self, x, training, mask, kv=None):
        baseline = x[NUM_OF_PYRAMIDS - 1]
        out = baseline
        fused = kv is not None and fpnmt.config.fuse_projections
        drop = self.rate if training else 0.0
        if fused:
            qs = self.q_group(baseline)
            qkv = [t for i in range(NUM_OF_PYRAMIDS - 1) for t in (qs[i], kv[i][0], kv[i][1])]
            m0 = self.mhas[0]
            out = ops.MultiViewAttnProjFn.apply(baseline, self.o_group, drop, m0.num_heads,
                                                1.0 / math.sqrt(float(m0.depth)), mask, *qkv)
        else:
            for i in range(NUM_OF_PYRAMIDS - 1):
                out, _ = self.mhas[i](x[i], x[i], baseline, mask, dropout=drop, residual=out)
        out1 = self.layernorm1(out)
        ffn_output = self.ffn2(self.ffn1(out1), dropout=drop)
        return self.layernorm2(ffn_output, residual=out1)

    call = forward


class DecoderLayer(nn.Module):

    def __init__(self, d_model, num_heads, dff, rate=0.1, init=None):
        super().__init__()
        self.mha1 = MultiHeadAttention(d_model, num_heads, init=init)
        self.mha2 = MultiHeadAttention(d_model, num_heads, init=init)
        self.ffn1 = Dense(d_model, dff, activation=ACTIVATION, act_alpha=LEAKY_ALPHA,
                          kernel_initializer=KERNEL_INITIALIZER, init=init)
        self.ffn2 = Dense(dff, d_model, kernel_initializer=KERNEL_INITIALIZER, init=init)
        self.ffn1.act_into_next = True
        self.layernorm1 = LayerNormalization(d_model, epsilon=1e-6)
        self.layernorm2 = LayerNormalization(d_model, epsilon=1e-6)
        self.layernorm3 = LayerNormalization(d_model, epsilon=1e-6)
        self.rate = rate
        self.qkv_group = DenseGroup([self.mha1.wq, self.mha1.wk, self.mha1.wv])

    def forward(self, x, enc_output, training, look_ahead_mask, padding_mask, kv2=None):
        fused = fpnmt.config.fuse_projections
        drop = self.rate if training else 0.0
        if fused:
            q, k, v = self.qkv_group(x)
            attn1, attn_weights_block1 = self.mha1.attend(q, k, v, look_ahead_mask, dropout=drop)
        else:
            attn1, attn_weights_block1 = self.mha1(x, x, x, look_ahead_mask, dropout=drop)
        out1 = self.layernorm1(attn1, residual=x)
        if fused and kv2 is not None:
            attn2, attn_weights_block2 = self.mha2.attend(self.mha2.wq(out1), kv2[0], kv2[1], padding_mask,
                                                          dropout=drop)
        else:
            attn2, attn_weights_block2 = self.mha2(enc_output, enc_output, out1, padding_mask, dropout=drop)
        out2 = self.layernorm2(attn2, residual=out1)
        ffn_output = self.ffn2(self.ffn1(out2), dropout=drop)
        out3 = self.layernorm3(ffn_output, residual=out2)
        return out3, attn_weights_block1, attn_weights_block2

    call = forward


class Encoder(nn.Module):

    def __init__(self, num_layers, d_model, num_heads, dff, input_vocab_size, rate=0.1, backbone=None, init=None):
        super().__init__()
        self.d_model = d_model
        self.num_layers = num_layers
        self.x_order = [i for i in range(NUM_OF_PYRAMIDS) if i != BASELINE_INDEX] + [BASELINE_INDEX]
        self.register_buffer("pos_encoding", positional_encoding(input_vocab_size, self.d_model)[0].contiguous())
        self.enc_layers = nn.ModuleList([EncoderLayer(d_model, num_heads, dff, rate, init=init)
                                         for _ in range(num_layers)])
        self.feature_extractor = retinanet.FeatureExtractor(RETINANET_WEIGHT_PATH, backbone=backbone or BACKBONE,
                                                            init=init)
        self.layernorm1 = LayerNormalization(d_model, epsilon=1e-6)
        self.rate = rate
        self.kv_groups = [DenseGroup([w for l in self.enc_layers for w in (l.mhas[i].wk, l.mhas[i].wv)])
                          for i in range(NUM_OF_PYRAMIDS - 1)] if num_layers > 0 else []

    def forward(self, x, training, mask):
        return self.from_features(self.feature_extractor(x, training=training), training, mask)

    def from_features(self, x, training, mask):
        x = ops.transformer_grads_barrier(list(x))
        x = [x[i] for i in self.x_order]
        for i_x in range(NUM_OF_PYRAMIDS):
            b, h, w, c = x[i_x].shape
            if h * w > self.pos_encoding.shape[0]:
                raise ValueError(f"view of length {h * w} exceeds the positional table "
                                 f"({self.pos_encoding.shape[0]}); raise input_vocab_size")
            x[i_x] = x[i_x].reshape(b, h * w, c)
        if fpnmt.config.fuse_view_norms:
            x = list(ops.LayerNormViewsFn.apply(self.layernorm1, self.pos_encoding,
                                                self.rate if training else 0.0, *x))
        else:
            for i_x in range(NUM_OF_PYRAMIDS):
                _x = self.layernorm1(x[i_x], pe=self.pos_encoding)
                x[i_x] = ops.dropout(_x, self.rate, training)
        kvs = [g(x[i]) for i, g in enumerate(self.kv_groups)] if fpnmt.config.fuse_projections else None
        for i in range(self.num_layers):
            kv = [(kvs[j][2 * i], kvs[j][2 * i + 1]) for j in range(NUM_OF_PYRAMIDS - 1)] if kvs else None
            x[NUM_OF_PYRAMIDS - 1] = self.enc_layers[i](x, training, mask, kv=kv)
        return x[NUM_OF_PYRAMIDS - 1]

    call = forward


class Decoder(nn.Module):

    def __init__(self, num_layers, d_model, num_heads, dff, target_vocab_size, rate=0.1, max_position=0,
                 max_seq_len=12, init=None):
        super().__init__()
        self.d_model = d_model
        self.num_layers = num_layers
        self.embedding = Embedding(target_vocab_size, d_model, init=init)
        self.register_buffer("pos_encoding", raw_positional_encoding(max_seq_len + max_position, d_model).contiguous())
        self.dec_layers = nn.ModuleList([DecoderLayer(d_model, num_heads, dff, rate, init=init)
                                         for _ in range(num_layers)])
        self.rate = rate
        self.cross_kv_group = DenseGroup([w for l in self.dec_layers for w in (l.mha2.wk, l.mha2.wv)]) \
            if num_layers > 0 else None

    def forward(self, x, enc_output, training, look_ahead_mask, padding_mask):
        seq_len = x.shape[1]
        if seq_len > self.pos_encoding.shape[0]:
            raise ValueError(f"target length {seq_len} exceeds max_seq_len {self.pos_encoding.shape[0]}")
        attention_weights = {}
        if fpnmt.config.fuse_view_norms:
            x = self.embedding(x, self.pos_encoding, enc_output.dtype, dropout=self.rate if training else 0.0)
        else:
            x = self.embedding(x, self.pos_encoding, enc_output.dtype)
            x = ops.dropout(x, self.rate, training)
        kv = self.cross_kv_group(enc_output) if (fpnmt.config.fuse_projections and self.cross_kv_group) else None
        for i in range(self.num_layers):
            kv2 = (kv[2 * i], kv[2 * i + 1]) if kv is not None else None
            x, block1, block2 = self.dec_layers[i](x, enc_output, training, look_ahead_mask, padding_mask, kv2=kv2)
            attention_weights["decoder_layer{}_block1".format(i + 1)] = block1
            attention_weights["decoder_layer{}_block2".format(i + 1)] = block2
        return x, attention_weights

    call = forward


class Transformer(nn.Module):

    def __init__(self, num_layers, d_model, num_heads, dff, input_vocab_size, target_vocab_size, rate=0.1,
                 max_position=0, max_seq_len=12, backbone=None, init=None):
        super().__init__()
        self.encoder = Encoder(num_layers, d_model, num_heads, dff, input_vocab_size, rate, backbone=backbone,
                               init=init)
        self.decoder = Decoder(num_layers, d_model, num_heads, dff, target_vocab_size, rate, max_position,
                               max_seq_len, init=init)
        self.final_layer = Dense(d_model, target_vocab_size, out_f32=True, init=init)

    def forward(self, inp, tar, training, look_ahead_mask):
        if training:
            enc_output = self.encoder(inp, training, None)
        else:
            enc_output = inp
        dec_output, attention_weights = self.decoder(tar, enc_output, training, look_ahead_mask, None)
        final_output = self.final_layer(dec_output)
        return final_output, attention_weights

    call = forward

    @property
    def trainable_variables(self):
        return [p for p in self.parameters() if p.requires_grad]

    def save_weights(self, filepath):
        from safetensors.torch import save_file
        import os
        sd = {k: (v.detach().float() if v.is_floating_point() else v.detach()).contiguous().cpu()
              for k, v in self.state_dict().items()}
        d = os.path.dirname(os.path.abspath(filepath))
        os.makedirs(d, exist_ok=True)
        save_file(sd, filepath, metadata={"format": "fpnmt-weights-v1"})

    def load_weights(self, filepath):
        from safetensors.torch import load_file
        from fpnmt import layers as flayers
        sd = load_file(filepath)
        own = self.state_dict()
        missing = [k for k in own if k not in sd]
        if missing:
            raise ValueError(f"load_weights: {filepath} lacks {missing[:4]}")
        unexpected = [k for k in sd if k not in own]
        if unexpected:
            raise ValueError(f"load_weights: {filepath} holds tensors this model does not have: {unexpected[:4]}")
        bad = [k for k, v in own.items() if tuple(sd[k].shape) != tuple(v.shape)]
        if bad:
            raise ValueError(f"load_weights: shape mismatch for {bad[:4]}: "
                             f"{[(tuple(sd[k].shape), tuple(own[k].shape)) for k in bad[:4]]}")
        with torch.no_grad():
            for k, v in own.items():
                v.copy_(sd[k].to(v.dtype))
        flayers.invalidate_weights()
```

### include/fpnmt.h

```cpp
#ifndef FPNMT_H
#define FPNMT_H

#include <stddef.h>
#include <stdint.h>

#ifdef __cplusplus
extern "C" {
#endif

typedef void* fpnmt_stream_t;

enum { FPNMT_F32 = 0, FPNMT_BF16 = 1 };
enum { FPNMT_ACT_NONE = 0, FPNMT_ACT_RELU = 1, FPNMT_ACT_LEAKY = 2, FPNMT_ACT_RELU6 = 3 };
enum {
  FPNMT_OK = 0,
  FPNMT_E_ARG = -1,
  FPNMT_E_UNSUPPORTED = -2,
  FPNMT_E_HIP = -3
};

const char* fpnmt_last_error(void);
int fpnmt_version(void);
const char* fpnmt_build_id(void);
int fpnmt_fill_zero(void* p, long long bytes, fpnmt_stream_t stream);
int fpnmt_fill_zero_grid(void* p, long long bytes, int max_blocks, fpnmt_stream_t stream);

int fpnmt_set_workspace(void* ws, long long bytes);

int fpnmt_defer_begin(void* arena, long long bytes);
int fpnmt_defer_flush(fpnmt_stream_t stream);
long long fpnmt_defer_peak_bytes(void);
int fpnmt_set_defer_conv_wgrads(int classes);

typedef struct fpnmt_gemm_desc {
  int m, n, k;
  int batch, batch_inner;
  int dtype;
  int a_trans, b_trans;
  long long lda, ldb, ldc, ldr;
  long long a_so, a_si, b_so, b_si, c_so, c_si, r_so, r_si;
  float alpha;
  int act;
  float act_alpha;
  int accumulate;
  int c_f32;
  int split_k;
  float drop_p;
  unsigned long long drop_seed;
  const long long* drop_seed_dev;
} fpnmt_gemm_desc;

int fpnmt_gemm(const fpnmt_gemm_desc* d, const void* A, const void* B, void* C,
               const float* col_scale, const float* bias, const void* R,
               fpnmt_stream_t stream);
int fpnmt_gemm_wgrad(const fpnmt_gemm_desc* d, const void* A, const void* B, void* C, fpnmt_stream_t stream);
int fpnmt_gemm_act_in(const fpnmt_gemm_desc* d, const void* A, const void* B, void* C, const void* y_in,
                      int act_in, float act_alpha, fpnmt_stream_t stream);

int fpnmt_bottleneck_fwd(int n, int h, int w, int c, int cm, const void* x, const void* wa, const float* ba,
                         const void* w3, const float* b3, const void* wc, const float* bc, void* y,
                         fpnmt_stream_t stream);

typedef struct fpnmt_conv_desc {
  int n, h, w, c;
  int k, r, s;
  int stride_h, stride_w;
  int pad_t, pad_b, pad_l, pad_r;
  int dtype;
  int act;
  float act_alpha;
} fpnmt_conv_desc;

int fpnmt_conv2d_fwd(const fpnmt_conv_desc* d, const void* x, const void* w_ohwi,
                     const float* scale, const float* bias, const void* residual,
                     void* y, fpnmt_stream_t stream);
int fpnmt_conv2d_bwd_data(const fpnmt_conv_desc* d, const void* dz, const void* w_flip,
                          void* dx, int accumulate, fpnmt_stream_t stream);
int fpnmt_conv2d_bwd_filter(const fpnmt_conv_desc* d, const void* x, const void* dz,
                            const float* col_scale, float* dw_hwio, fpnmt_stream_t stream);
int fpnmt_conv2d_bwd_filter_bias(const fpnmt_conv_desc* d, const void* x, const void* dz,
                                 const float* col_scale, float* dw_hwio, float* db,
                                 fpnmt_stream_t stream);
int fpnmt_conv2d_bwd_data_act(const fpnmt_conv_desc* d, const void* dz, const void* w_flip,
                              void* dx, const void* y_in, int act_in, fpnmt_stream_t stream);
int fpnmt_conv2d_bwd_data_mask(const fpnmt_conv_desc* d, const void* dz, const void* w_flip,
                               void* dx, int accumulate, const void* y, int act,
                               fpnmt_stream_t stream);
int fpnmt_conv2d_bwd_data_res(const fpnmt_conv_desc* d, const void* dz, const void* w_flip,
                              void* dx, const void* res, fpnmt_stream_t stream);
int fpnmt_conv2d_bwd_data_res_act(const fpnmt_conv_desc* d, const void* dz, const void* w_flip,
                                  void* dx, const void* res, const void* y_in, int act_in,
                                  fpnmt_stream_t stream);

typedef struct fpnmt_conv_level {
  int n, h, w;
  const void* x;
  const void* dz;
  const void* residual;
  void* y;
} fpnmt_conv_level;
int fpnmt_conv2d_fwd_grouped(const fpnmt_conv_desc* d, int n_levels, const fpnmt_conv_level* lv,
                             const void* w_ohwi, const float* scale, const float* bias,
                             fpnmt_stream_t stream);
int fpnmt_conv2d_bwd_data_grouped(const fpnmt_conv_desc* d, int n_levels, const fpnmt_conv_level* lv,
                                  const void* w_flip, int accumulate, fpnmt_stream_t stream);
int fpnmt_conv2d_bwd_filter_grouped(const fpnmt_conv_desc* d, int n_levels, const fpnmt_conv_level* lv,
                                    const float* col_scale, float* dw_hwio, fpnmt_stream_t stream);
int fpnmt_conv2d_bwd_filter_grouped_bias(const fpnmt_conv_desc* d, int n_levels, const fpnmt_conv_level* lv,
                                         const float* col_scale, float* dw_hwio, float* db,
                                         fpnmt_stream_t stream);
int fpnmt_conv2d_bwd_data_grouped_act(const fpnmt_conv_desc* d, int n_levels, const fpnmt_conv_level* lv,
                                      const void* w_flip, int act_in, fpnmt_stream_t stream);
int fpnmt_conv2d_bwd_data_grouped_mask(const fpnmt_conv_desc* d, int n_levels, const fpnmt_conv_level* lv,
                                       const void* w_flip, int accumulate, int act, fpnmt_stream_t stream);

int fpnmt_weight_prep(const float* w_hwio, int r, int s, int c, int k, const float* scale,
                      int dtype, void* w_ohwi, void* w_flip, long long ld_flip, fpnmt_stream_t stream);
typedef struct fpnmt_wprep_item {
  const float* w_hwio;
  const float* scale;
  void* w_ohwi;
  void* w_flip;
  int r, s, c, k;
  long long tile_start;
  long long ld_flip;
} fpnmt_wprep_item;
int fpnmt_weight_prep_batched(const fpnmt_wprep_item* items_dev, int n_items, long long total_tiles,
                              int dtype, fpnmt_stream_t stream);

long long fpnmt_act_bwd_ws_bytes(int dtype, long long rows, int c);
int fpnmt_act_bwd(int dtype, long long rows, int c, int act, float act_alpha,
                  const void* dy, const void* y, void* dz, float* db, float* ws,
                  float drop_p, unsigned long long drop_seed, const long long* drop_seed_dev,
                  fpnmt_stream_t stream);
int fpnmt_bias_grad(int dtype, long long rows, int c, const void* dy, float* db, fpnmt_stream_t stream);
int fpnmt_cast(int in_dtype, int out_dtype, long long n, const void* in, void* out,
               fpnmt_stream_t stream);
int fpnmt_dropout(int dtype, long long n, float p, unsigned long long seed,
                  const long long* seed_dev, const void* x, void* y, fpnmt_stream_t stream);
int fpnmt_add(int dtype, long long n, const void* a, const void* b, void* out,
              fpnmt_stream_t stream);

int fpnmt_maxpool2d_fwd(int dtype, int n, int h, int w, int c, int kh, int kw, int sh, int sw,
                        int pt, int pl, int ho, int wo, const void* x, void* y,
                        uint8_t* argmax, fpnmt_stream_t stream);
int fpnmt_maxpool2d_bwd(int dtype, int n, int h, int w, int c, int kh, int kw, int sh, int sw,
                        int pt, int pl, int ho, int wo, const void* x, const uint8_t* argmax,
                        const void* dy, void* dx, fpnmt_stream_t stream);
int fpnmt_maxpool2d_bwd_act(int dtype, int n, int h, int w, int c, int kh, int kw, int sh, int sw,
                            int pt, int pl, int ho, int wo, const uint8_t* argmax, const void* dy,
                            const void* x, int act, float alpha, void* dx, fpnmt_stream_t stream);

int fpnmt_fpn_topdown_fwd(int dtype, int n, int c, int h5, int w5, int h4, int w4, int h3,
                          int w3, const void* lat5, const void* lat4, const void* lat3,
                          void* p4m, void* p3m, fpnmt_stream_t stream);
int fpnmt_fpn_topdown_bwd(int dtype, int n, int c, int h5, int w5, int h4, int w4, int h3,
                          int w3, const void* d_p4m, const void* d_p3m, void* d_lat4,
                          void* d_lat5, int accumulate_lat5, fpnmt_stream_t stream);

int fpnmt_spatial_softmax_fwd(int dtype, int n, int hw, int c, const void* score, const void* hs,
                              void* ctx, float* a_out, fpnmt_stream_t stream);
int fpnmt_spatial_softmax_bwd(int dtype, int n, int hw, int c, const float* a, const void* hs,
                              const void* d_ctx, void* d_score, void* d_hs, double* ws,
                              fpnmt_stream_t stream);

typedef struct fpnmt_attn_desc {
  int b, h, lq, lk, d;
  int dtype;
  long long ldq, ldk, ldv, ldo, ldw;
  float scale;
  long long m_sb, m_sh, m_si, m_sj;
} fpnmt_attn_desc;
size_t fpnmt_attention_ws_bytes(const fpnmt_attn_desc* d);
int fpnmt_attention_fwd(const fpnmt_attn_desc* d, const void* q, const void* k, const void* v,
                        const float* mask, void* out, void* weights, void* ws,
                        fpnmt_stream_t stream);
int fpnmt_attention_bwd(const fpnmt_attn_desc* d, const void* q, const void* k, const void* v,
                        const void* weights, const void* d_out, void* dq, void* dk, void* dv,
                        void* ws, fpnmt_stream_t stream);
#define FPNMT_MAX_VIEWS 4
int fpnmt_attention_fwd_views(int n, const fpnmt_attn_desc* d, const void* const* q, const void* const* k,
                              const void* const* v, const float* const* mask, void* const* out,
                              void* const* weights, void* const* ws, fpnmt_stream_t stream);
int fpnmt_attention_bwd_views(int n, const fpnmt_attn_desc* d, const void* const* q, const void* const* k,
                              const void* const* v, const void* const* weights, const void* const* d_out,
                              void* const* dq, void* const* dk, void* const* dv, void* const* ws,
                              fpnmt_stream_t stream);

int fpnmt_view_proj_fwd(int dtype, int m, int n, int k, int nseg, const void* A, long long lda, const void* W,
                        const float* bias, const void* R, long long ldr, void* out, long long ldo, float drop_p,
                        unsigned long long seed, const long long* seed_dev, fpnmt_stream_t stream);
int fpnmt_view_proj_bwd_dz(int dtype, int m, int n, int nseg, const void* dy, long long lddy, void* dz, float* db,
                           float drop_p, unsigned long long seed, const long long* seed_dev,
                           fpnmt_stream_t stream);

int fpnmt_layernorm_fwd(int dtype, long long rows, int d, float eps, const void* x,
                        const void* res, const float* gamma, const float* beta, const float* pe,
                        int pe_rows, void* y, float* mean, float* rstd, fpnmt_stream_t stream);
int fpnmt_layernorm_bwd(int dtype, long long rows, int d, const void* x, const void* res,
                        const float* gamma, const float* mean, const float* rstd, const void* dy,
                        void* dx, float* dgamma, float* dbeta, fpnmt_stream_t stream);
#define FPNMT_MAX_LN_VIEWS 8
typedef struct fpnmt_ln_view {
  const void* x;
  void* y;
  const void* dy;
  float* mean;
  float* rstd;
  long long rows;
  int pe_rows;
  unsigned long long seed;
} fpnmt_ln_view;
int fpnmt_layernorm_views_fwd(int dtype, int n, int d, float eps, const fpnmt_ln_view* views,
                              const float* gamma, const float* beta, const float* pe, float drop_p,
                              const long long* seed_dev, fpnmt_stream_t stream);
int fpnmt_layernorm_views_bwd(int dtype, int n, int d, const fpnmt_ln_view* views, const float* gamma,
                              float drop_p, const long long* seed_dev, float* dgamma, float* dbeta,
                              fpnmt_stream_t stream);
int fpnmt_layernorm_bwd_drop(int dtype, long long rows, int d, const void* x, const void* res,
                             const float* gamma, const float* mean, const float* rstd, const void* dy,
                             void* dx, float* dgamma, float* dbeta, float drop_p,
                             unsigned long long drop_seed, const long long* drop_seed_dev, void* dz,
                             fpnmt_stream_t stream);

int fpnmt_embed_posenc_fwd(int dtype, int b, int t, int d, const int32_t* tok, const float* emb,
                           const float* pe, void* y, fpnmt_stream_t stream);
int fpnmt_embed_posenc_bwd(int dtype, int b, int t, int d, const int32_t* tok, const void* dy,
                           float* d_emb, float* sumsq, fpnmt_stream_t stream);
int fpnmt_embed_posenc_fwd_drop(int dtype, int b, int t, int d, const int32_t* tok, const float* emb,
                                const float* pe, void* y, float drop_p, unsigned long long seed,
                                const long long* seed_dev, fpnmt_stream_t stream);
int fpnmt_embed_posenc_bwd_drop(int dtype, int b, int t, int d, const int32_t* tok, const void* dy,
                                float* d_emb, float* sumsq, float drop_p, unsigned long long seed,
                                const long long* seed_dev, fpnmt_stream_t stream);

int fpnmt_decoder_targets(int b, int t_full, const void* tok, int tok_bytes, long long ld_tok, int32_t* tar_inp,
                          int32_t* tar_real, float* mask, fpnmt_stream_t stream);

int fpnmt_xent_fwd_bwd(int dtype, long long rows, int v, const float* logits, long long ld,
                       const int32_t* labels, float* loss, void* dlogits, long long ldd,
                       float dloss_scale, fpnmt_stream_t stream);

int fpnmt_grad_sumsq(int nblocks, const int32_t* blk_seg, const long long* blk_start,
                     int block_elems, const long long* off, const int32_t* seg_flags,
                     const float* g, float grad_scale, float* blk_part, fpnmt_stream_t stream);
typedef struct fpnmt_adam_desc {
  float beta1, beta2, eps, clipnorm;
  float sched_d_model, sched_warmup, sched_mult, sched_warm_pow;
  float const_lr;
  float grad_scale;
} fpnmt_adam_desc;
int fpnmt_amsgrad_step(const fpnmt_adam_desc* d, int nblocks, const int32_t* blk_seg,
                       const long long* blk_start, int block_elems, const long long* off,
                       const int32_t* seg_flags, float* param, const float* grad, float* m,
                       float* v, float* vhat, const float* sumsq, const float* blk_part,
                       const int32_t* seg_blk0, long long* step, fpnmt_stream_t stream);
typedef struct fpnmt_seg_prep {
  void* ohwi;
  void* flip;
  const float* scale;
  int r, s, c, k;
  long long ld_flip;
  uint32_t c_magic, c_shift;
} fpnmt_seg_prep;
int fpnmt_amsgrad_step_prep(const fpnmt_adam_desc* d, int nblocks, const int32_t* blk_seg,
                            const long long* blk_start, int block_elems, const long long* off,
                            const int32_t* seg_flags, float* param, const float* grad, float* m,
                            float* v, float* vhat, const float* sumsq, const float* blk_part,
                            const int32_t* seg_blk0, long long* step, const fpnmt_seg_prep* preps,
                            fpnmt_stream_t stream);
int fpnmt_grad_sumsq_part(int blk_first, int nblocks, int max_grid, const int32_t* blk_seg,
                          const long long* blk_start, int block_elems, const long long* off,
                          const int32_t* seg_flags, const float* g, float grad_scale, float* blk_part,
                          fpnmt_stream_t stream);
int fpnmt_amsgrad_step_part(const fpnmt_adam_desc* d, int blk_first, int nblocks, int inc_step, int max_grid,
                            const int32_t* blk_seg, const long long* blk_start, int block_elems,
                            const long long* off, const int32_t* seg_flags, float* param,
                            const float* grad, float* m, float* v, float* vhat, const float* sumsq,
                            const float* blk_part, const int32_t* seg_blk0, long long* step,
                            const fpnmt_seg_prep* preps, fpnmt_stream_t stream);

int fpnmt_decode_attention(int dtype, int rows, int heads, int depth, int lk, float scale, const void* q,
                           long long ldq, const void* kv, long long row_stride, long long pos_stride,
                           long long k_off, long long v_off, const int32_t* src, int src_ld, int row_div,
                           void* out, long long ldo, fpnmt_stream_t stream);
int fpnmt_beam_step(int n_images, int beam_n, int vocab, const float* logits, long long ldl, float* beam_prob,
                    const int32_t* hist_in, int32_t* hist_out, int hist_ld, int t, const int32_t* src_in,
                    int32_t* src_out, int src_ld, int end_token, int32_t* tok_out, int32_t* result, int result_ld,
                    int32_t* result_len, int32_t* status, fpnmt_stream_t stream);
int fpnmt_beam_step_log(int n_images, int beam_n, int vocab, const float* logits, long long ldl, float* beam_score,
                        int32_t* beam_len, int32_t* beam_fin, const int32_t* hist_in, int32_t* hist_out,
                        int hist_ld, int t, const int32_t* src_in, int32_t* src_out, int src_ld, int end_token,
                        int32_t* tok_out, int32_t* status, fpnmt_stream_t stream);
int fpnmt_beam_finalize(int n_images, int beam_n, const int32_t* hist, int hist_ld, const float* beam_score,
                        const int32_t* beam_len, const int32_t* beam_fin, float alpha, int32_t* nbest_tok,
                        int tok_ld, int32_t* nbest_len, float* nbest_score, fpnmt_stream_t stream);

#define FPNMT_SAMPLE_FILTER_MAX_VOCAB 16384
int fpnmt_sample_step(int rows, int vocab, const float* logits, long long ldl, float temperature, int top_k,
                      float top_p, unsigned long long seed, const long long* seed_dev, float* score, int32_t* slen,
                      int32_t* fin, int32_t* hist, int hist_ld, int t, int end_token, int32_t* tok_out,
                      int32_t* kept_out , fpnmt_stream_t stream);
int fpnmt_sample_uniform(int rows, int t, unsigned long long seed, const long long* seed_dev, float* u_out,
                         fpnmt_stream_t stream);

int fpnmt_bn_stats(int dtype, long long rows, int c, const void* x, float* mean, float* var,
                   float* moving_mean, float* moving_var, float momentum, fpnmt_stream_t stream);
int fpnmt_bn_apply(int dtype, long long rows, int c, const void* x, const float* mean, const float* var,
                   const float* gamma, const float* beta, float eps, int act, const void* residual, void* y,
                   fpnmt_stream_t stream);
int fpnmt_bn_bwd(int dtype, long long rows, int c, const void* x, const float* mean, const float* var,
                 const float* gamma, float eps, int act, const void* y, const void* dy, void* dx,
                 float* dgamma, float* dbeta, fpnmt_stream_t stream);
int fpnmt_bn_stats_sums(int dtype, long long rows, int c, const void* x, double* sums, fpnmt_stream_t stream);
int fpnmt_bn_stats_finalize(int c, const double* sums, float* mean, float* var, float* moving_mean,
                            float* moving_var, float momentum, fpnmt_stream_t stream);
int fpnmt_bn_bwd_sums(int dtype, long long rows, int c, const void* x, const float* mean, const float* var,
                      float eps, int act, const void* y, const void* dy, double* sums, float* dgamma,
                      float* dbeta, fpnmt_stream_t stream);
int fpnmt_bn_bwd_dx(int dtype, long long rows, int c, const void* x, const float* mean, const float* var,
                    const float* gamma, float eps, int act, const void* y, const void* dy, const double* sums,
                    void* dx, fpnmt_stream_t stream);
int fpnmt_depthwise_fwd(int dtype, int n, int h, int w, int c, int kh, int kw, int stride, int pad_t,
                        int pad_b, int pad_l, int pad_r, const void* x, const float* w_hwc, void* y,
                        fpnmt_stream_t stream);
int fpnmt_depthwise_bwd_data(int dtype, int n, int h, int w, int c, int kh, int kw, int stride, int pad_t,
                             int pad_b, int pad_l, int pad_r, const void* dy, const float* w_hwc, void* dx,
                             fpnmt_stream_t stream);
int fpnmt_depthwise_bwd_filter(int dtype, int n, int h, int w, int c, int kh, int kw, int stride, int pad_t,
                               int pad_b, int pad_l, int pad_r, const void* x, const void* dy, float* dw_hwc,
                               fpnmt_stream_t stream);

typedef struct fpnmt_image_item {
  long long offset;
  int h, w;
} fpnmt_image_item;
int fpnmt_image_resize_normalize(const fpnmt_image_item* items_dev, int n, const uint8_t* pixels,
                                 long long pixel_bytes, int max_w, int out_h, int out_w, float div, float sub,
                                 int dtype, void* out, fpnmt_stream_t stream);

#ifdef __cplusplus
}
#endif
#endif
```

Baseline: 3371 images/s.

## Collapse single-key cross-attention into a broadcast row fused into LayerNorm

When the encoder output has a single position and no padding mask, cross-attention softmax is identically one, so each decoder layer's cross-attention reduces to projecting V once per batch row and broadcasting it over T. New LayerNorm forward and backward kernels synthesize that broadcast term, with bias and dropout, inside the residual LayerNorm. A grouped row-sum kernel reduces the gradients back to per-batch vectors. This removes the per-layer query projection, attention matmuls and the full-size output projection. The cost is extra code paths, and attention weights are replaced by a cached ones tensor. The fast path depends on config flags and the encoder output shape.

```diff
diff --git a/fpn-mt-image-captioning_amd/csrc/elementwise.hip b/fpn-mt-image-captioning_amd/csrc/elementwise.hip
--- a/fpn-mt-image-captioning_amd/csrc/elementwise.hip
+++ b/fpn-mt-image-captioning_amd/csrc/elementwise.hip
@@ -748,14 +748,33 @@
   else return lane + 64 * k;
 }
 
-template <typename T, bool VEC>
+struct LnSynth {
+  const float* c;
+  const float* cbias;
+  int t;
+  float p;
+  unsigned long long key;
+};
+template <typename T>
+__device__ __forceinline__ float ln_synth(const LnSynth& sy, float sc, long long r, long long crow, int d, int col) {
+#pragma clang fp contract(off)
+  float a = sy.c[crow * d + col];
+  if (sy.cbias) a += sy.cbias[col];
+  if (sy.p > 0.f) a = uniform01(sy.key, (uint64_t)r * (uint64_t)d + (uint64_t)col) >= sy.p ? a * sc : 0.f;
+  return to_f32(from_f32<T>(a));
+}
+
+template <typename T, bool VEC, bool SYN = false>
 __device__ __forceinline__ void ln_fwd_rows(long long blk, long long nblk, long long rows, int d, float eps,
                                             const T* __restrict__ x, const T* __restrict__ res,
                                             const float* __restrict__ gamma, const float* __restrict__ beta,
                                             const float* __restrict__ pe, int pe_rows, T* __restrict__ y,
                                             float* __restrict__ mean_out, float* __restrict__ rstd_out, float op,
-                                            unsigned long long okey) {
+                                            unsigned long long okey, const LnSynth sy = LnSynth{},
+                                            T* __restrict__ x_out = nullptr) {
+#pragma clang fp contract(off)
   const int lane = threadIdx.x & 63;
+  const float ssc = SYN && sy.p > 0.f ? 1.f / (1.f - sy.p) : 1.f;
   const long long wid = (blk * 256LL + threadIdx.x) >> 6;
   const long long nw = nblk * 4;
   const float osc = op > 0.f ? 1.f / (1.f - op) : 1.f;
@@ -783,19 +802,26 @@
         const int c0 = (lane + 64 * i) * 8;
         bf16x8 xv = {}, rv = {};
         if (c0 < d) {
-          xv = *(const bf16x8*)(x + r * d + c0);
+          if constexpr (!SYN) xv = *(const bf16x8*)(x + r * d + c0);
           if (res) rv = *(const bf16x8*)(res + r * d + c0);
         }
 #pragma unroll
         for (int e = 0; e < 8; ++e) {
           float t = 0.f;
           if (c0 < d) {
-            t = to_f32(xv[e]);
+            if constexpr (SYN) {
+              t = ln_synth<T>(sy, ssc, r, r / sy.t, d, c0 + e);
+              xv[e] = from_f32<T>(t);
+            } else {
+              t = to_f32(xv[e]);
+            }
             if (res) t = to_f32(from_f32<T>(t + to_f32(rv[e])));
           }
           v[i * 8 + e] = t;
           s += t;
         }
+        if constexpr (SYN)
+          if (x_out && c0 < d) *(bf16x8*)(x_out + r * d + c0) = xv;
       }
     } else {
 #pragma unroll
@@ -803,7 +829,13 @@
         const int col = lane + 64 * i;
         v[i] = 0.f;
         if (col < d) {
-          float t = to_f32(x[r * d + col]);
+          float t;
+          if constexpr (SYN) {
+            t = ln_synth<T>(sy, ssc, r, r / sy.t, d, col);
+            if (x_out) x_out[r * d + col] = from_f32<T>(t);
+          } else {
+            t = to_f32(x[r * d + col]);
+          }
           if (res) t = to_f32(from_f32<T>(t + to_f32(res[r * d + col])));
           v[i] = t;
           s += t;
@@ -815,7 +847,7 @@
 #pragma unroll
     for (int i = 0; i < LN_MAXE; ++i) {
       const int col = ln_col<VEC>(lane, i);
-      if (col < d) { const float t = v[i] - mu; q += t * t; }
+      if (col < d) { const float t = v[i] - mu; q = __builtin_fmaf(t, t, q); }
     }
     const float var = wave_sum(q) / (float)d;
     const float rs = rsqrtf(var + eps);
@@ -827,7 +859,7 @@
           bf16x8 ov;
 #pragma unroll
           for (int e = 0; e < 8; ++e) {
-            float o = (v[i * 8 + e] - mu) * rs * gm[i * 8 + e] + bt[i * 8 + e];
+            float o = __builtin_fmaf((v[i * 8 + e] - mu) * rs, gm[i * 8 + e], bt[i * 8 + e]);
             if (pe) o += pv[i * 8 + e];
             ov[e] = from_f32<T>(o);
             if (op > 0.f)
@@ -842,7 +874,7 @@
       for (int i = 0; i < LN_MAXE; ++i) {
         const int col = lane + 64 * i;
         if (col < d) {
-          float o = (v[i] - mu) * rs * gm[i] + bt[i];
+          float o = __builtin_fmaf((v[i] - mu) * rs, gm[i], bt[i]);
           if (pe) o += pv[i];
           T ot = from_f32<T>(o);
           if (op > 0.f)
@@ -868,15 +900,17 @@
                       0.f, 0ull);
 }
 
-template <typename T, bool VEC>
+template <typename T, bool VEC, bool SYN = false>
 __device__ __forceinline__ void ln_bwd_rows(long long blk, long long nblk, long long rows, int d,
                                             const T* __restrict__ x, const T* __restrict__ res,
                                             const float* __restrict__ gamma, const float* __restrict__ mean,
                                             const float* __restrict__ rstd, const T* __restrict__ dy,
                                             T* __restrict__ dx, float* __restrict__ part, float dp,
                                             unsigned long long dkey, T* __restrict__ dz, float ip,
-                                            unsigned long long ikey) {
+                                            unsigned long long ikey, const LnSynth sy = LnSynth{}) {
+#pragma clang fp contract(off)
   const int lane = threadIdx.x & 63;
+  const float ssc = SYN && sy.p > 0.f ? 1.f / (1.f - sy.p) : 1.f;
   const float dsc = dz ? 1.f / (1.f - dp) : 1.f;
   const float isc = ip > 0.f ? 1.f / (1.f - ip) : 1.f;
   const long long wid = (blk * 256LL + threadIdx.x) >> 6;
@@ -894,7 +928,7 @@
         const int c0 = (lane + 64 * i) * 8;
         bf16x8 xv = {}, rv = {}, dv = {};
         if (c0 < d) {
-          xv = *(const bf16x8*)(x + r * d + c0);
+          if constexpr (!SYN) xv = *(const bf16x8*)(x + r * d + c0);
           if (res) rv = *(const bf16x8*)(res + r * d + c0);
           dv = *(const bf16x8*)(dy + r * d + c0);
         }
@@ -904,7 +938,9 @@
           xh[k] = 0.f;
           g[k] = 0.f;
           if (c0 < d) {
-            float t = to_f32(xv[e]);
+            float t;
+            if constexpr (SYN) t = ln_synth<T>(sy, ssc, r, r / sy.t, d, c0 + e);
+            else t = to_f32(xv[e]);
             if (res) t = to_f32(from_f32<T>(t + to_f32(rv[e])));
             xh[k] = (t - mu) * rs;
             float dyf = to_f32(dv[e]);
@@ -926,7 +962,9 @@
         xh[i] = 0.f;
         g[i] = 0.f;
         if (col < d) {
-          float t = to_f32(x[r * d + col]);
+          float t;
+          if constexpr (SYN) t = ln_synth<T>(sy, ssc, r, r / sy.t, d, col);
+          else t = to_f32(x[r * d + col]);
           if (res) t = to_f32(from_f32<T>(t + to_f32(res[r * d + col])));
           xh[i] = (t - mu) * rs;
           float dyf = to_f32(dy[r * d + col]);
@@ -950,7 +988,8 @@
         if (c0 < d) {
           bf16x8 ov;
 #pragma unroll
-          for (int e = 0; e < 8; ++e) ov[e] = from_f32<T>(rs * (g[i * 8 + e] - s1 - xh[i * 8 + e] * s2));
+          for (int e = 0; e < 8; ++e)
+            ov[e] = from_f32<T>(rs * __builtin_fmaf(-xh[i * 8 + e], s2, g[i * 8 + e] - s1));
           *(bf16x8*)(dx + r * d + c0) = ov;
           if (dz) {
 #pragma unroll
@@ -968,7 +1007,7 @@
       for (int i = 0; i < LN_MAXE; ++i) {
         const int col = lane + 64 * i;
         if (col < d) {
-          const T v = from_f32<T>(rs * (g[i] - s1 - xh[i] * s2));
+          const T v = from_f32<T>(rs * __builtin_fmaf(-xh[i], s2, g[i] - s1));
           dx[r * d + col] = v;
           if (dz) {
             const float t = to_f32(v);
@@ -1013,6 +1052,57 @@
                                                      T* __restrict__ dz) {
   ln_bwd_rows<T, VEC>(blockIdx.x, gridDim.x, rows, d, x, res, gamma, mean, rstd, dy, dx, part, dp,
                       dz ? drop_key_of(dseed, dseed_dev) : 0ull, dz, 0.f, 0ull);
+}
+
+template <typename T, bool VEC = false>
+__global__ __launch_bounds__(256) void ln_bcast_fwd_kernel(long long rows, int d, float eps, const LnSynth sy,
+                                                           unsigned long long seed,
+                                                           const long long* __restrict__ seed_dev,
+                                                           const T* __restrict__ res,
+                                                           const float* __restrict__ gamma,
+                                                           const float* __restrict__ beta, T* __restrict__ y,
+                                                           float* __restrict__ mean_out,
+                                                           float* __restrict__ rstd_out, T* __restrict__ x_out) {
+  LnSynth q = sy;
+  q.key = sy.p > 0.f ? drop_key_of(seed, seed_dev) : 0ull;
+  ln_fwd_rows<T, VEC, true>(blockIdx.x, gridDim.x, rows, d, eps, nullptr, res, gamma, beta, nullptr, 1, y, mean_out,
+                            rstd_out, 0.f, 0ull, q, x_out);
+}
+
+template <typename T, bool VEC = false>
+__global__ __launch_bounds__(256) void ln_bcast_bwd_kernel(long long rows, int d, const LnSynth sy,
+                                                           unsigned long long seed,
+                                                           const long long* __restrict__ seed_dev,
+                                                           const T* __restrict__ res,
+                                                           const float* __restrict__ gamma,
+                                                           const float* __restrict__ mean,
+                                                           const float* __restrict__ rstd,
+                                                           const T* __restrict__ dy, T* __restrict__ dx,
+                                                           float* __restrict__ part, T* __restrict__ dz) {
+  LnSynth q = sy;
+  q.key = sy.p > 0.f ? drop_key_of(seed, seed_dev) : 0ull;
+  ln_bwd_rows<T, VEC, true>(blockIdx.x, gridDim.x, rows, d, nullptr, res, gamma, mean, rstd, dy, dx, part, sy.p, q.key,
+                            dz, 0.f, 0ull, q);
+}
+
+struct RowsumGroups {
+  const void* dz[FPNMT_MAX_ROWSUM_GROUPS];
+};
+template <typename T>
+__global__ __launch_bounds__(256) void rowsum_groups_kernel(const RowsumGroups G, int b, int t, int d,
+                                                            float* __restrict__ dc, T* __restrict__ dc_lp,
+                                                            T* __restrict__ zero, long long zero_ld,
+                                                            long long zero_so) {
+  const int col = blockIdx.x * 256 + threadIdx.x;
+  const int i = blockIdx.y, l = blockIdx.z;
+  if (col >= d) return;
+  if (zero) zero[l * zero_so + i * zero_ld + col] = from_f32<T>(0.f);
+  const T* src = (const T*)G.dz[l] + (long long)i * t * d + col;
+  float s = 0.f;
+  for (int j = 0; j < t; ++j) s += to_f32(src[(long long)j * d]);
+  const long long o = ((long long)l * b + i) * d + col;
+  dc[o] = s;
+  if (dc_lp) dc_lp[o] = from_f32<T>(s);
 }
 
 struct LnView {
@@ -1565,6 +1655,108 @@
                             drop_seed_dev, dz, S(stream));
 }
 
+static void log_bcast(const char* op, int dtype, long long rows, int d, int t, float p, bool vec) {
+  if (FILE* f = gemm_log()) {
+    std::fprintf(f, "ln_bcast op=%s dtype=%s rows=%lld d=%d t=%d p=%g vec=%d\n", op, dtype == FPNMT_BF16 ? "bf16" : "f32",
+                 rows, d, t, (double)p, vec ? 1 : 0);
+    std::fflush(f);
+  }
+}
+
+static int ln_bcast_args(long long rows, int d, int t, const float* c, float drop_p) {
+  if (d > 64 * LN_MAXE) return fail(FPNMT_E_UNSUPPORTED, "layernorm: d > 1024");
+  if (!c || t <= 0 || rows % t) return fail(FPNMT_E_ARG, "layernorm_bcast: null c / rows not a multiple of t");
+  if (!(drop_p >= 0.f && drop_p < 1.f)) return fail(FPNMT_E_ARG, "layernorm_bcast: drop_p outside [0, 1)");
+  return 0;
+}
+
+int fpnmt_layernorm_bcast_fwd(int dtype, long long rows, int d, int t, float eps, const float* c, const float* cbias,
+                              float drop_p, unsigned long long drop_seed, const long long* drop_seed_dev,
+                              const void* res, const float* gamma, const float* beta, void* y, float* mean,
+                              float* rstd, void* x_out, fpnmt_stream_t stream) {
+  if (rows <= 0) return 0;
+  if (const int st = ln_bcast_args(rows, d, t, c, drop_p)) return st;
+  if (dtype != FPNMT_BF16 && dtype != FPNMT_F32) return fail(FPNMT_E_ARG, "layernorm_bcast_fwd: bad dtype");
+  const LnSynth sy{c, cbias, t, drop_p, 0ull};
+  const int g = grid_for(rows, 4, 8192);
+  const bool vec = dtype == FPNMT_BF16 && ln_vec(d, {res, y, x_out});
+  log_bcast("fwd", dtype, rows, d, t, drop_p, vec);
+  if (dtype == FPNMT_BF16) {
+    if (vec)
+      hipLaunchKernelGGL((ln_bcast_fwd_kernel<bf16, true>), dim3(g), dim3(256), 0, S(stream), rows, d, eps, sy,
+                         drop_seed, drop_seed_dev, (const bf16*)res, gamma, beta, (bf16*)y, mean, rstd, (bf16*)x_out);
+    else
+      hipLaunchKernelGGL((ln_bcast_fwd_kernel<bf16>), dim3(g), dim3(256), 0, S(stream), rows, d, eps, sy, drop_seed,
+                         drop_seed_dev, (const bf16*)res, gamma, beta, (bf16*)y, mean, rstd, (bf16*)x_out);
+  } else {
+    hipLaunchKernelGGL((ln_bcast_fwd_kernel<float>), dim3(g), dim3(256), 0, S(stream), rows, d, eps, sy, drop_seed,
+                       drop_seed_dev, (const float*)res, gamma, beta, (float*)y, mean, rstd, (float*)x_out);
+  }
+  return check_launch("layernorm_bcast_fwd");
+}
+
+int fpnmt_layernorm_bcast_bwd(int dtype, long long rows, int d, int t, const float* c, const float* cbias,
+                              float drop_p, unsigned long long drop_seed, const long long* drop_seed_dev,
+                              const void* res, const float* gamma, const float* mean, const float* rstd,
+                              const void* dy, void* dx, float* dgamma, float* dbeta, void* dz,
+                              fpnmt_stream_t stream) {
+  if (rows <= 0) return 0;
+  if (const int st = ln_bcast_args(rows, d, t, c, drop_p)) return st;
+  if (dtype != FPNMT_BF16 && dtype != FPNMT_F32) return fail(FPNMT_E_ARG, "layernorm_bcast_bwd: bad dtype");
+  if (!dz && drop_p > 0.f) return fail(FPNMT_E_ARG, "layernorm_bcast_bwd: null dz with drop_p > 0");
+  if (drop_p <= 0.f) dz = nullptr;
+  hipStream_t s = S(stream);
+  const LnSynth sy{c, cbias, t, drop_p, 0ull};
+  const int g = grid_for(rows, 4, 1024);
+  float* part = nullptr;
+  if (dgamma || dbeta) {
+    part = partial_f32((long long)g * 2 * d);
+    if (!part) return fail(FPNMT_E_ARG, "layernorm_bcast_bwd: dgamma / dbeta need the fpnmt workspace");
+  }
+  const bool vec = dtype == FPNMT_BF16 && ln_vec(d, {res, dy, dx, dz});
+  log_bcast("bwd", dtype, rows, d, t, drop_p, vec);
+  if (dtype == FPNMT_BF16) {
+    if (vec)
+      hipLaunchKernelGGL((ln_bcast_bwd_kernel<bf16, true>), dim3(g), dim3(256), 0, s, rows, d, sy, drop_seed,
+                         drop_seed_dev, (const bf16*)res, gamma, mean, rstd, (const bf16*)dy, (bf16*)dx, part,
+                         (bf16*)dz);
+    else
+      hipLaunchKernelGGL((ln_bcast_bwd_kernel<bf16>), dim3(g), dim3(256), 0, s, rows, d, sy, drop_seed, drop_seed_dev,
+                         (const bf16*)res, gamma, mean, rstd, (const bf16*)dy, (bf16*)dx, part, (bf16*)dz);
+  } else {
+    hipLaunchKernelGGL((ln_bcast_bwd_kernel<float>), dim3(g), dim3(256), 0, s, rows, d, sy, drop_seed, drop_seed_dev,
+                       (const float*)res, gamma, mean, rstd, (const float*)dy, (float*)dx, part, (float*)dz);
+  }
+  if (part) colsum_launch(g, 2 * d, part, dgamma, s, d, dbeta);
+  return check_launch("layernorm_bcast_bwd");
+}
+
+int fpnmt_rowsum_groups(int dtype, int n, int b, int t, int d, const void* const* dz, float* dc, void* dc_lp,
+                        void* zero, long long zero_ld, long long zero_so, fpnmt_stream_t stream) {
+  if (n < 0 || n > FPNMT_MAX_ROWSUM_GROUPS) return fail(FPNMT_E_ARG, "rowsum_groups: 0 <= n <= FPNMT_MAX_ROWSUM_GROUPS");
+  if (n == 0 || b <= 0 || d <= 0) return 0;
+  if (t < 0 || b > 65535 || !dz || !dc) return fail(FPNMT_E_ARG, "rowsum_groups: bad shape / null pointer");
+  if (dtype != FPNMT_BF16 && dtype != FPNMT_F32) return fail(FPNMT_E_ARG, "rowsum_groups: bad dtype");
+  if (zero && (zero_ld < d || zero_so < 0)) return fail(FPNMT_E_ARG, "rowsum_groups: zero_ld < d / zero_so < 0");
+  RowsumGroups G{};
+  for (int l = 0; l < n; ++l) {
+    if (!dz[l] && t > 0) return fail(FPNMT_E_ARG, "rowsum_groups: null dz");
+    G.dz[l] = dz[l];
+  }
+  if (FILE* f = gemm_log()) {
+    std::fprintf(f, "rowsum_groups dtype=%s n=%d b=%d t=%d d=%d\n", dtype == FPNMT_BF16 ? "bf16" : "f32", n, b, t, d);
+    std::fflush(f);
+  }
+  const dim3 grid(cdiv(d, 256), b, n);
+  if (dtype == FPNMT_BF16)
+    hipLaunchKernelGGL((rowsum_groups_kernel<bf16>), grid, dim3(256), 0, S(stream), G, b, t, d, dc, (bf16*)dc_lp,
+                       (bf16*)zero, zero_ld, zero_so);
+  else
+    hipLaunchKernelGGL((rowsum_groups_kernel<float>), grid, dim3(256), 0, S(stream), G, b, t, d, dc, (float*)dc_lp,
+                       (float*)zero, zero_ld, zero_so);
+  return check_launch("rowsum_groups");
+}
+
 static bool ln_views_vec(int n, int d, const fpnmt_ln_view* v, bool bwd) {
   for (int i = 0; i < n; ++i)
     if (!(bwd ? ln_vec(d, {v[i].x, v[i].dy, v[i].y}) : ln_vec(d, {v[i].x, v[i].y}))) return false;
diff --git a/fpn-mt-image-captioning_amd/fpnmt/__init__.py b/fpn-mt-image-captioning_amd/fpnmt/__init__.py
--- a/fpn-mt-image-captioning_amd/fpnmt/__init__.py
+++ b/fpn-mt-image-captioning_amd/fpnmt/__init__.py
@@ -28,6 +28,8 @@
     fuse_ffn_act = True
     fuse_input_act = True
     zero_grad_overlap_grid = 0
+    cross_one_key = True
+    cross_one_key_store_x = True
 
 
 config = _Config()
diff --git a/fpn-mt-image-captioning_amd/fpnmt/_lib.py b/fpn-mt-image-captioning_amd/fpnmt/_lib.py
--- a/fpn-mt-image-captioning_amd/fpnmt/_lib.py
+++ b/fpn-mt-image-captioning_amd/fpnmt/_lib.py
@@ -42,6 +42,7 @@
                            "unset them for benchmarks, smoke and tests")
 
 F32, BF16 = 0, 1
+MAX_ROWSUM_GROUPS = 16
 ACT_NONE, ACT_RELU, ACT_LEAKY, ACT_RELU6 = 0, 1, 2, 3
 
 
@@ -174,6 +175,9 @@
     "fpnmt_layernorm_fwd": [I, LL, I, F, P, P, P, P, P, I, P, P, P, P],
     "fpnmt_layernorm_bwd": [I, LL, I, P, P, P, P, P, P, P, P, P, P],
     "fpnmt_layernorm_bwd_drop": [I, LL, I, P, P, P, P, P, P, P, P, P, F, ULL, P, P, P],
+    "fpnmt_layernorm_bcast_fwd": [I, LL, I, I, F, P, P, F, ULL, P, P, P, P, P, P, P, P, P],
+    "fpnmt_layernorm_bcast_bwd": [I, LL, I, I, P, P, F, ULL, P, P, P, P, P, P, P, P, P, P, P],
+    "fpnmt_rowsum_groups": [I, I, I, I, I, C.POINTER(C.c_void_p), P, P, P, LL, LL, P],
     "fpnmt_decoder_targets": [I, I, P, I, LL, P, P, P, P],
     "fpnmt_layernorm_views_fwd": [I, I, I, F, C.POINTER(LnView), P, P, P, F, P, P],
     "fpnmt_layernorm_views_bwd": [I, I, I, C.POINTER(LnView), P, F, P, P, P, P],
diff --git a/fpn-mt-image-captioning_amd/fpnmt/layers.py b/fpn-mt-image-captioning_amd/fpnmt/layers.py
--- a/fpn-mt-image-captioning_amd/fpnmt/layers.py
+++ b/fpn-mt-image-captioning_amd/fpnmt/layers.py
@@ -281,8 +281,9 @@
 
 class DenseGroup:
 
-    def __init__(self, layers):
+    def __init__(self, layers, reorder=True):
         self.layers = list(layers)
+        self.reorder = reorder
         fin, fout = self.layers[0].kernel.shape
         for m in self.layers:
             if tuple(m.kernel.shape) != (fin, fout) or m.activation not in (None, "linear") or m.out_f32 \
@@ -354,7 +355,7 @@
     seen = set()
     for m in model.modules():
         g = m.__dict__.get("_group")
-        if g is not None and id(g[0]) not in seen:
+        if g is not None and id(g[0]) not in seen and g[0].reorder:
             seen.add(id(g[0]))
             groups.append(g[0])
     name_of = {id(p): n for n, p in named}
diff --git a/fpn-mt-image-captioning_amd/fpnmt/ops.py b/fpn-mt-image-captioning_amd/fpnmt/ops.py
--- a/fpn-mt-image-captioning_amd/fpnmt/ops.py
+++ b/fpn-mt-image-captioning_amd/fpnmt/ops.py
@@ -1557,6 +1557,184 @@
         return (None, None, None, *dxs)
 
 
+class _OneKeyBox:
+    __slots__ = ("dzs",)
+
+    def __init__(self, n):
+        self.dzs = [None] * n
+
+
+def _uniform_stride(ts):
+    es = ts[0].element_size()
+    base = ts[0].data_ptr()
+    if len(ts) == 1:
+        return 0
+    step = ts[1].data_ptr() - base
+    if step <= 0 or step % es:
+        return None
+    for i, t in enumerate(ts):
+        if t.data_ptr() != base + i * step or t.untyped_storage().data_ptr() != ts[0].untyped_storage().data_ptr():
+            return None
+    return step // es
+
+
+class CrossOneKeyFn(torch.autograd.Function):
+
+    @staticmethod
+    def forward(ctx, o_group, box, *kv):
+        n, fin, fout = o_group.n, o_group.fin, o_group.fout
+        if len(kv) != 2 * n:
+            raise ValueError("CrossOneKeyFn: one (k, v) per layer")
+        ks, vs = kv[:n], kv[n:]
+        B = vs[0].shape[0]
+        if any(tuple(t.shape) != (B, 1, fin) for t in kv) or fin != fout:
+            raise ValueError("CrossOneKeyFn: (B, 1, d) keys / values and a square output Dense")
+        slots = [_slot_of(t) for t in kv]
+        slots = [sl if sl is not None and sl[0].claim(sl[1]) else None for sl in slots]
+        cdt = vs[0].dtype
+        dt = dtype_code(cdt)
+        vs = [_rows_view(v) for v in vs]
+        a_so = _uniform_stride(vs)
+        if a_so is None or len({_row_ld(v) for v in vs}) != 1:
+            vs = list(torch.stack([v.reshape(B, fin) for v in vs]).unbind(0))
+            vs = [v.view(B, 1, fin) for v in vs]
+            a_so = B * fin
+        lda = _row_ld(vs[0])
+        stack, _ = o_group.stacked(cdt)
+        c = _empty((n, B, fout), torch.float32, vs[0].device)
+        g = _gemm_desc(B, fout, fin, dt, lda, fin, fout, c_f32=1 if cdt != torch.float32 else 0)
+        g.batch = n
+        g.a_so, g.b_so, g.c_so = a_so, fout * fin, B * fout
+        call("fpnmt_gemm", g, ptr(vs[0]), ptr(stack), ptr(c), None, None, None, stream_ptr())
+        ctx.o_group, ctx.box, ctx.slots, ctx.B = o_group, box, slots, B
+        ctx.a_so, ctx.lda = a_so, lda
+        ctx.set_materialize_grads(False)
+        ctx.save_for_backward(*vs)
+        return tuple(c[i] for i in range(n))
+
+    @staticmethod
+    def backward(ctx, *_gc):
+        vs = ctx.saved_tensors
+        group, box, B = ctx.o_group, ctx.box, ctx.B
+        n, fin, fout = group.n, group.fin, group.fout
+        dzs, box.dzs = box.dzs, [None] * n
+        if all(z is None for z in dzs):
+            return (None,) * (2 + 2 * n)
+        if any(z is None for z in dzs):
+            raise RuntimeError("CrossOneKeyFn: some decoder layers were not back-propagated")
+        cdt = vs[0].dtype
+        dt = dtype_code(cdt)
+        dev = vs[0].device
+        s = stream_ptr()
+        T = dzs[0].numel() // (B * fout)
+        slots = ctx.slots
+        same = all(sl is not None and sl[0] is slots[0][0] for sl in slots)
+        if same:
+            slot = slots[0][0]
+            grads = [slot.view(sl[1], (B, 1, fin)) for sl in slots]
+        else:
+            buf = _empty((B, 2 * n * fin), cdt, dev)
+            grads = [buf[:, i * fin:(i + 1) * fin].view(B, 1, fin) for i in range(2 * n)]
+        dks, dvs = grads[:n], grads[n:]
+        k_so, v_so = _uniform_stride(dks), _uniform_stride(dvs)
+        if k_so is None or v_so is None or n > L.MAX_ROWSUM_GROUPS:
+            raise RuntimeError("CrossOneKeyFn: the layers' key / value gradients must sit at a constant stride")
+        dc = _empty((n, B, fout), torch.float32, dev)
+        dcl = dc if cdt == torch.float32 else _empty((n, B, fout), cdt, dev)
+        import ctypes
+        tab = (ctypes.c_void_p * n)(*[z.data_ptr() for z in dzs])
+        call("fpnmt_rowsum_groups", dt, n, B, T, fout, tab, ptr(dc), ptr(dcl) if dcl is not dc else None,
+             ptr(dks[0]), _row_ld(dks[0]), k_so, s)
+        _, flip = group.stacked(cdt)
+        g = _gemm_desc(B, fin, fout, dt, fout, n * fout, _row_ld(dvs[0]))
+        g.batch = n
+        g.a_so, g.b_so, g.c_so = B * fout, fout, v_so
+        call("fpnmt_gemm", g, ptr(dcl), ptr(flip), ptr(dvs[0]), None, None, None, s)
+        kg, bg = group.grad_views()
+        for i, m in enumerate(group.layers):
+            if m.bias.requires_grad:
+                bias_grad(L.F32, B, fout, dc[i], _grad_of(m.bias).data_ptr(), s)
+        if kg is not None:
+            g = _gemm_desc(fin, fout, B, dt, ctx.lda, fout, fout, a_trans=1, b_trans=1, accumulate=2, c_f32=1)
+            g.batch = n
+            g.a_so, g.b_so, g.c_so = ctx.a_so, B * fout, fin * fout
+            _wgrad(lambda: call("fpnmt_gemm_wgrad", g, ptr(vs[0]), ptr(dcl), ptr(kg), stream_ptr()), *vs, dcl)
+        else:
+            for i, m in enumerate(group.layers):
+                g = _gemm_desc(fin, fout, B, dt, ctx.lda, fout, fout, a_trans=1, b_trans=1, accumulate=2, c_f32=1)
+                gk = _grad_of(m.kernel)
+                _wgrad(lambda g=g, i=i, gk=gk: call("fpnmt_gemm_wgrad", g, ptr(vs[i]), dcl[i].data_ptr(), ptr(gk),
+                                                    stream_ptr()), vs[i], dcl)
+        return (None, None, *dks, *dvs)
+
+
+class LayerNormBcastFn(torch.autograd.Function):
+
+    @staticmethod
+    def forward(ctx, res, c, layer, dense, drop_p, box, idx):
+        ctx.rsink_res = _sink_for_res(res)
+        res = res.contiguous()
+        d = res.shape[-1]
+        t = res.shape[-2]
+        rows = res.numel() // d if d else 0
+        if c.dtype != torch.float32 or not c.is_contiguous() or c.numel() * t != res.numel():
+            raise ValueError("LayerNormBcastFn: c must be a contiguous fp32 (B, d) for res (B, T, d)")
+        seed, st = 0, None
+        if drop_p > 0.0:
+            seed, st = runtime.next_seed(), runtime.seed_tensor
+        y = torch.empty_like(res)
+        mean = _empty((max(rows, 1),), torch.float32, res.device)
+        rstd = _empty((max(rows, 1),), torch.float32, res.device)
+        import fpnmt
+        x = torch.empty_like(res) if fpnmt.config.cross_one_key_store_x and any(ctx.needs_input_grad) else None
+        call("fpnmt_layernorm_bcast_fwd", dtype_code(res.dtype), rows, d, t, layer.epsilon, ptr(c), ptr(dense.bias),
+             float(drop_p), seed, ptr(st), ptr(res), ptr(layer.gamma), ptr(layer.beta), ptr(y), ptr(mean), ptr(rstd),
+             ptr(x), stream_ptr())
+        ctx.layer, ctx.dense, ctx.drop, ctx.box, ctx.idx = layer, dense, (float(drop_p), seed, st), box, idx
+        ctx.fuse_drop = bool(fpnmt.config.fuse_drop_ln)
+        ctx.save_for_backward(res, c, mean, rstd, x)
+        return y
+
+    @staticmethod
+    def backward(ctx, dy):
+        res, c, mean, rstd, x = ctx.saved_tensors
+        layer = ctx.layer
+        d, t = res.shape[-1], res.shape[-2]
+        rows = res.numel() // d if d else 0
+        p, seed, st = ctx.drop
+        dt = dtype_code(res.dtype)
+        dx = torch.empty_like(res)
+        dz = torch.empty_like(res) if p > 0.0 else None
+        dy = dy.contiguous()
+        dg, db = ptr(_grad_of(layer.gamma)), ptr(_grad_of(layer.beta))
+        if x is None:
+            call("fpnmt_layernorm_bcast_bwd", dt, rows, d, t, ptr(c), ptr(ctx.dense.bias), p, seed, ptr(st), ptr(res),
+                 ptr(layer.gamma), ptr(mean), ptr(rstd), ptr(dy), ptr(dx), dg, db, ptr(dz), stream_ptr())
+        elif dz is not None and ctx.fuse_drop:
+            call("fpnmt_layernorm_bwd_drop", dt, rows, d, ptr(x), ptr(res), ptr(layer.gamma), ptr(mean), ptr(rstd),
+                 ptr(dy), ptr(dx), dg, db, p, seed, ptr(st), ptr(dz), stream_ptr())
+        else:
+            call("fpnmt_layernorm_bwd", dt, rows, d, ptr(x), ptr(res), ptr(layer.gamma), ptr(mean), ptr(rstd), ptr(dy),
+                 ptr(dx), dg, db, stream_ptr())
+            if dz is not None:
+                act_bwd(dt, rows, d, L.ACT_NONE, 0.0, dx, None, dz, None, stream_ptr(), drop=ctx.drop)
+        ctx.box.dzs[ctx.idx] = dz if dz is not None else dx
+        return _sink_put(ctx.rsink_res, dx), None, None, None, None, None, None
+
+
+_ONES_CACHE = {}
+
+
+def cached_ones(shape, dtype, device):
+    key = (tuple(shape), dtype, str(device))
+    t = _ONES_CACHE.get(key)
+    if t is None:
+        t = torch.ones(shape, dtype=dtype, device=device)
+        if not (t.is_cuda and torch.cuda.is_current_stream_capturing()):
+            _ONES_CACHE[key] = t
+    return t
+
+
 class EmbedPosencFn(torch.autograd.Function):
     @staticmethod
     def forward(ctx, tok, emb, pe, dtype, layer, sumsq_slot, drop_p=0.0):
diff --git a/fpn-mt-image-captioning_amd/models/transformer.py b/fpn-mt-image-captioning_amd/models/transformer.py
--- a/fpn-mt-image-captioning_amd/models/transformer.py
+++ b/fpn-mt-image-captioning_amd/models/transformer.py
@@ -138,7 +138,7 @@
         self.rate = rate
         self.qkv_group = DenseGroup([self.mha1.wq, self.mha1.wk, self.mha1.wv])
 
-    def forward(self, x, enc_output, training, look_ahead_mask, padding_mask, kv2=None):
+    def forward(self, x, enc_output, training, look_ahead_mask, padding_mask, kv2=None, one_key=None):
         fused = fpnmt.config.fuse_projections
         drop = self.rate if training else 0.0
         if fused:
@@ -147,6 +147,14 @@
         else:
             attn1, attn_weights_block1 = self.mha1(x, x, x, look_ahead_mask, dropout=drop)
         out1 = self.layernorm1(attn1, residual=x)
+        if one_key is not None:
+            c, box, idx = one_key
+            out2 = ops.LayerNormBcastFn.apply(out1, c, self.layernorm2, self.mha2.dense, drop, box, idx)
+            attn_weights_block2 = ops.cached_ones((out1.shape[0], self.mha2.num_heads, out1.shape[1], 1),
+                                                  out1.dtype, out1.device)
+            ffn_output = self.ffn2(self.ffn1(out2), dropout=drop)
+            out3 = self.layernorm3(ffn_output, residual=out2)
+            return out3, attn_weights_block1, attn_weights_block2
         if fused and kv2 is not None:
             attn2, attn_weights_block2 = self.mha2.attend(self.mha2.wq(out1), kv2[0], kv2[1], padding_mask,
                                                           dropout=drop)
@@ -219,6 +227,13 @@
         self.rate = rate
         self.cross_kv_group = DenseGroup([w for l in self.dec_layers for w in (l.mha2.wk, l.mha2.wv)]) \
             if num_layers > 0 else None
+        self.cross_o_group = DenseGroup([l.mha2.dense for l in self.dec_layers], reorder=False) \
+            if num_layers > 0 else None
+
+    def one_key(self, enc_output, padding_mask, kv):
+        return (fpnmt.config.cross_one_key and kv is not None and enc_output.dim() == 3
+                and enc_output.shape[1] == 1 and padding_mask is None
+                and self.num_layers <= fpnmt._lib.MAX_ROWSUM_GROUPS)
 
     def forward(self, x, enc_output, training, look_ahead_mask, padding_mask):
         seq_len = x.shape[1]
@@ -231,9 +246,14 @@
             x = self.embedding(x, self.pos_encoding, enc_output.dtype)
             x = ops.dropout(x, self.rate, training)
         kv = self.cross_kv_group(enc_output) if (fpnmt.config.fuse_projections and self.cross_kv_group) else None
+        cs = box = None
+        if self.one_key(enc_output, padding_mask, kv):
+            box = ops._OneKeyBox(self.num_layers)
+            cs = ops.CrossOneKeyFn.apply(self.cross_o_group, box, *kv[0::2], *kv[1::2])
         for i in range(self.num_layers):
             kv2 = (kv[2 * i], kv[2 * i + 1]) if kv is not None else None
-            x, block1, block2 = self.dec_layers[i](x, enc_output, training, look_ahead_mask, padding_mask, kv2=kv2)
+            x, block1, block2 = self.dec_layers[i](x, enc_output, training, look_ahead_mask, padding_mask, kv2=kv2,
+                                                   one_key=(cs[i], box, i) if cs is not None else None)
             attention_weights["decoder_layer{}_block1".format(i + 1)] = block1
             attention_weights["decoder_layer{}_block2".format(i + 1)] = block2
         return x, attention_weights
diff --git a/include/fpnmt.h b/include/fpnmt.h
--- a/include/fpnmt.h
+++ b/include/fpnmt.h
@@ -222,6 +222,20 @@
                              void* dx, float* dgamma, float* dbeta, float drop_p,
                              unsigned long long drop_seed, const long long* drop_seed_dev, void* dz,
                              fpnmt_stream_t stream);
+
+int fpnmt_layernorm_bcast_fwd(int dtype, long long rows, int d, int t, float eps, const float* c,
+                              const float* cbias, float drop_p, unsigned long long drop_seed,
+                              const long long* drop_seed_dev, const void* res, const float* gamma,
+                              const float* beta, void* y, float* mean, float* rstd, void* x_out,
+                              fpnmt_stream_t stream);
+int fpnmt_layernorm_bcast_bwd(int dtype, long long rows, int d, int t, const float* c, const float* cbias,
+                              float drop_p, unsigned long long drop_seed, const long long* drop_seed_dev,
+                              const void* res, const float* gamma, const float* mean, const float* rstd,
+                              const void* dy, void* dx, float* dgamma, float* dbeta, void* dz,
+                              fpnmt_stream_t stream);
+#define FPNMT_MAX_ROWSUM_GROUPS 16
+int fpnmt_rowsum_groups(int dtype, int n, int b, int t, int d, const void* const* dz, float* dc, void* dc_lp,
+                        void* zero, long long zero_ld, long long zero_so, fpnmt_stream_t stream);
 
 int fpnmt_embed_posenc_fwd(int dtype, int b, int t, int d, const int32_t* tok, const float* emb,
                            const float* pe, void* y, fpnmt_stream_t stream);
```

Result: faster. 3465 images/s (median of 6 runs) (+2.8%).
